# invesalius/invesalius3

Measured on AMD Instinct MI355X. Metric: Mvoxel/s segmentation + Mtriangles/s marching-cubes, 512^3 int16, 1/2/4/8 GPU, higher is better.
Workload: dtype i16; 1 GPU; configs[1]: 512x512x512 int16 per GPU, threshold(226..3071) + 26-neighbour region-grow + marching-cubes(mask@127); global_voxels=134217728, parallelism=z-slab x1, collectives=none, overlap=none

## Files before the change

include/ivx.h:

```cpp
#ifndef IVX_H
#define IVX_H
#include <stddef.h>
#include <stdint.h>

#ifdef __cplusplus
extern "C" {
#endif

#define IVX_OK 0
#define IVX_EINVAL (-1)
#define IVX_ERANGE (-2)
#define IVX_ENOMEM (-3)
#define IVX_EDOM (-4)
#define IVX_EHIP (-5)
#define IVX_ESTALE (-6)
#define IVX_EINTERNAL (-7)

#define IVX_U8 0
#define IVX_I16 1
#define IVX_F64 2
#define IVX_U16 3
#define IVX_F32 4
#define IVX_I32 5
#define IVX_I64 6
// ... 25 lines not shown
int ivx_stream_destroy(void *stream);
int ivx_stream_synchronize(void *stream);
int ivx_event_create(void **event);
int ivx_event_create_sync(void **event);
int ivx_event_destroy(void *event);
int ivx_event_record(void *event, void *stream);
int ivx_stream_wait_event(void *stream, void *event);
int ivx_event_elapsed_ms(void *start, void *stop, float *ms);
int ivx_release_workspace(void);

int ivx_host_register(const void *base, size_t nbytes, uint64_t *handle);
int ivx_host_touch(uint64_t handle);
int ivx_host_touch_range(uint64_t handle, size_t offset, size_t nbytes);
int ivx_host_release(uint64_t handle);
int ivx_host_stats(uint64_t handle, uint64_t out[8]);
int ivx_host_count(uint64_t *count);
int ivx_host_set_check(int on);
int ivx_transfer_stats(uint64_t out[4]);
int ivx_upload_strided(void *dst, const void *src, const int64_t shape[3], const int64_t strides[3], size_t itemsize);
int ivx_download_strided(void *dst, const int64_t shape[3], const int64_t strides[3], const void *src, size_t itemsize);

int ivx_dev_threshold_i16(const int16_t *img, int64_t dz, int64_t dy, int64_t dx, int lo, int hi,
                          int preserve, const uint8_t *skip_flags, uint8_t *mask, void *stream);
int ivx_dev_threshold_i16_bits(const int16_t *img, int64_t dz, int64_t dy, int64_t dx, int lo, int hi, uint8_t *mask,
                               uint64_t *bits, void *stream);
#define IVX_RANGES_BUILD 0
#define IVX_RANGES_USE 1
int ivx_image_ranges_bytes(int64_t dz, int64_t dy, int64_t dx, size_t *nbytes);
int ivx_dev_image_ranges_i16(const int16_t *img, int64_t dz, int64_t dy, int64_t dx, uint32_t *ranges, void *stream);
int ivx_dev_threshold_i16_bits_ranges(const int16_t *img, int64_t dz, int64_t dy, int64_t dx, int lo, int hi,
                                      uint8_t *mask, uint64_t *bits, uint32_t *ranges, int mode, void *stream);
int ivx_dev_threshold_i16_plane(const int16_t *img, int64_t dz, int64_t dy, int64_t dx, int lo, int hi, uint64_t *bits,
                                void *stream);
int ivx_dev_threshold_i16_plane_ranges(const int16_t *img, int64_t dz, int64_t dy, int64_t dx, int lo, int hi, uint64_t *bits,
                                       uint32_t *ranges, int mode, void *stream);
int ivx_threshold_all_slices(const int16_t *img, const int64_t shape[3], const int64_t img_strides[3],
                             int lo, int hi, int preserve, int honour_flags, uint8_t *mask,
                             const int64_t mask_strides[3]);

int ivx_dev_mip_reduce(int dtype, const void *vol, int64_t dz, int64_t dy, int64_t dx, int axis, int op,
                       void *out, void *stream);
int ivx_mip_reduce(int dtype, const void *vol, const int64_t shape[3], const int64_t strides[3], int axis,
                   int op, void *out, const int64_t out_strides[2]);
int ivx_dev_replicate_i16(const int16_t *src, int64_t h, int64_t w, int factor, int16_t *dst, void *stream);

int ivx_dev_minmax_f32(int dtype, const void *vol, int64_t n, float *minmax2, void *stream);
int ivx_dev_mida(int dtype, const void *vol, int64_t dz, int64_t dy, int64_t dx, int axis, float wl, float ww,
                 const float *minmax2 , int out_dtype, void *out,
                 int *status , void *stream);
int ivx_dev_lmip(int dtype, const void *vol, int64_t dz, int64_t dy, int64_t dx, int axis, double tmin,
                 double tmax, void *out, void *stream);
int ivx_dev_rays_z_slab(int kind, int dtype, const void *vol, int64_t dz, int64_t dy, int64_t dx, double p0, double p1,
                        const float *minmax2, const double *state_in, double *state_out, int out_dtype, void *out,
                        int *status, void *stream);
int ivx_powf_variant(void);
int ivx_dev_powf(const float *x, const float *y, float *out, int64_t n, int variant, void *stream);
int ivx_dev_fcm_bounds(const int32_t *d, const uint32_t *other, float n, float *lo, float *hi, int64_t count, void *stream);
int ivx_dev_fcm_volume(int dtype, const void *vol, int64_t dz, int64_t dy, int64_t dx, float n, int axis,
                       void *tmp , int *status, void *stream);
int ivx_dev_fcm_maxip(int dtype, const void *vol, int64_t dz, int64_t dy, int64_t dx, float n, int axis, void *out,
                      int *status, void *stream);
int ivx_mida(int dtype, const void *img, const int64_t shape[3], const int64_t strides[3], int axis,
             double wl, double ww, int out_dtype, void *out, const int64_t out_strides[2]);
int ivx_lmip(int dtype, const void *img, const int64_t shape[3], const int64_t strides[3], int axis,
             double tmin, double tmax, void *out, const int64_t out_strides[2]);
int ivx_fast_countour_mip(int dtype, const void *img, const int64_t shape[3], const int64_t strides[3],
                          float n, int axis, double wl, double ww, int tmip, void *out,
                          const int64_t out_strides[2]);

typedef struct ivx_mc_params {
    int32_t dtype;
    int32_t pad_xy;
    int32_t pad_bottom;
    int32_t pad_top;
    int32_t vtk_pz;
    int32_t niso;
    int64_t nz, ny, nx;
    int64_t roi_start;
    double pad_value;
    double spacing[3];
    double iso[2];
} ivx_mc_params;
int ivx_dev_mc_scratch_bytes(const ivx_mc_params *p, size_t *nbytes);
int ivx_mc_split_word_ids(const ivx_mc_params *p, const uint32_t *wid, size_t n, uint32_t *k, uint32_t *j, uint32_t *w);
int ivx_dev_mc_count(const ivx_mc_params *p, const void *a, void *scratch, int64_t *ntris, void *stream);
int ivx_dev_mc_count_async(const ivx_mc_params *p, const void *a, void *scratch, void *stream);
int ivx_dev_mc_count_bits_async(const ivx_mc_params *p, const uint64_t *inside_bits, void *scratch, void *stream);
int ivx_dev_mc_total(const ivx_mc_params *p, void *scratch, int64_t *ntris, void *stream);
int ivx_dev_mc_total_early(const ivx_mc_params *p, void *scratch, int64_t *ntris, void *stream);
int ivx_dev_mc_count_bits(const ivx_mc_params *p, const uint64_t *inside_bits, void *scratch, int64_t *ntris,
                          void *stream);
int ivx_dev_mc_emit(const ivx_mc_params *p, const void *a, const void *scratch, float *tris, int64_t max_tris,
                    void *stream);
int ivx_dev_mc_emit_levels(const ivx_mc_params *p, const void *scratch, const uint64_t *sel_bits, double v_out, double v_in,
                           double v_sel, float *tris, int64_t max_tris, void *stream);
int ivx_dev_mc_list(const ivx_mc_params *p, const void *scratch, int64_t max_tris, void *stream);
int ivx_marching_cubes_begin(const ivx_mc_params *p, const void *a, const int64_t strides[3], int64_t *ntris);
int ivx_marching_cubes_fetch(float *tris, int64_t ntris);
int ivx_marching_cubes(const ivx_mc_params *p, const void *a, const int64_t strides[3], float *tris,
                       int64_t max_tris, int64_t *ntris);

int ivx_dev_mc_stitch_sig_bytes(const ivx_mc_params *p, size_t *nbytes);
int ivx_dev_mc_stitch_top_sig(const ivx_mc_params *p, const void *scratch, void *sig, void *stream);
int ivx_dev_mc_stitch_match(const ivx_mc_params *p, const void *scratch, const void *nbr_sig, int64_t nverts, uint32_t *vd,
                            void *stream);
int ivx_dev_mc_stitch_apply(const ivx_mc_params *p, const void *scratch, const void *nbr_sig, const uint32_t *vd_all, int rank,
                            const float *verts, int64_t nverts, int32_t *faces, int64_t ntris, float *verts_out, void *stream);
int ivx_dev_mc_indexed_count(const ivx_mc_params *p, const void *a, const void *scratch, int64_t *nverts, void *stream);
int ivx_dev_mc_indexed_emit(const ivx_mc_params *p, const void *a, const void *scratch, float *verts, int64_t max_verts,
                            int32_t *faces, int64_t max_tris, void *stream);
int ivx_dev_mc_indexed_count_levels(const ivx_mc_params *p, const void *scratch, int64_t *nverts, void *stream);
int ivx_dev_mc_indexed_emit_levels(const ivx_mc_params *p, const void *scratch, const uint64_t *sel_bits, double v_out,
                                   double v_in, double v_sel, float *verts, int64_t max_verts, int32_t *faces,
                                   int64_t max_tris, void *stream);
int ivx_marching_cubes_indexed(const ivx_mc_params *p, const void *a, const int64_t strides[3], float *verts,
                               int64_t max_verts, int32_t *faces, int64_t max_tris, int64_t *nverts, int64_t *ntris);

int ivx_dev_mesh_keep_largest(const float *verts, int64_t nverts, const int32_t *faces, int64_t ntris, float *out_verts,
                              int64_t max_verts, int32_t *out_faces, int64_t max_tris, int64_t *out_nverts,
                              int64_t *out_ntris, int64_t *nregions, void *stream);
int ivx_dev_mesh_mass_properties(const float *verts, const int32_t *faces, int64_t ntris, double *out8, void *stream);
int ivx_mesh_keep_largest(const float *verts, int64_t nverts, const int32_t *faces, int64_t ntris, float *out_verts,
                          int32_t *out_faces, int64_t *out_nverts, int64_t *out_ntris, int64_t *nregions);
int ivx_mesh_mass_properties(const float *verts, int64_t nverts, const int32_t *faces, int64_t ntris, double *out8);
int ivx_mesh_fill_holes(const float *verts, int64_t nverts, const int32_t *faces, int64_t ntris, double hole_size,
                        float *new_verts, int32_t *new_faces, int64_t *n_new_verts, int64_t *n_new_tris);
int ivx_mesh_point_normals(const float *verts, int64_t nverts, const int32_t *faces, int64_t ntris, double cos_feature_angle,
                           int splitting, int auto_orient, float *out_verts, int32_t *out_faces, float *point_normals,
                           float *cell_normals , int64_t *out_nverts);
typedef struct ivx_mesh_view {
    double eye[3], right[3], up[3], fwd[3];
    double znear, zfar;
    double tan_half, aspect;
    int32_t width, height;
} ivx_mesh_view;
#define IVX_RASTER_CLEAR 1
#define IVX_RASTER_SMALL 2
#define IVX_RASTER_BIG 4
#define IVX_RASTER_ALL 7
#define IVX_RASTER_SMALL_BOX 64
int ivx_dev_mesh_bounds(const float *verts, int64_t nverts, float *bounds6, void *stream);
int ivx_dev_mesh_depth_raster(const float *verts, int64_t nverts, const int32_t *faces, int64_t ntris,
                              const ivx_mesh_view *view , int stages, float *depth, void *stream);
int ivx_dev_mesh_visible_points(const float *verts, int64_t nverts, const int32_t *faces, int64_t ntris,
                                const ivx_mesh_view *views , int nviews, uint8_t *flags, void *stream);
int ivx_dev_mesh_select_points(const float *verts, int64_t nverts, const int32_t *faces, int64_t ntris, const uint8_t *flags,
                               int invert, float *out_verts, int64_t max_verts, int32_t *out_faces, int64_t max_tris,
                               int64_t *out_nverts, int64_t *out_ntris, void *stream);
int ivx_mesh_bounds(const float *verts, int64_t nverts, float *bounds6);
int ivx_mesh_depth_raster(const float *verts, int64_t nverts, const int32_t *faces, int64_t ntris, const ivx_mesh_view *view,
                          float *depth);
int ivx_mesh_visible_points(const float *verts, int64_t nverts, const int32_t *faces, int64_t ntris,
                            const ivx_mesh_view *views, int nviews, uint8_t *flags);
int ivx_mesh_select_points(const float *verts, int64_t nverts, const int32_t *faces, int64_t ntris, const uint8_t *flags,
                           int invert, float *out_verts, int32_t *out_faces, int64_t *out_nverts, int64_t *out_ntris);
int ivx_mesh_remove_nonvisible(const float *verts, int64_t nverts, const int32_t *faces, int64_t ntris,
                               const ivx_mesh_view *views, int nviews, int remove_visible, float *out_verts,
                               int32_t *out_faces, int64_t *out_nverts, int64_t *out_ntris);

typedef struct ivx_surface_camera {
    double focal[3], right[3], up[3], dir[3];
    double parallel_scale;
    int32_t width, height;
} ivx_surface_camera;
typedef struct ivx_surface_layer {
    const float *verts;
// ... 121 lines not shown
int ivx_dev_mask_snapshot_restore(uint8_t *dst, int64_t n, const void *header, const void *pool, int64_t literal_blocks,
                                  int64_t plane_bytes, uint8_t *plane_flags, void *stream);
int ivx_mask_snapshot(const uint8_t *matrix, size_t nbytes, void **header, void **pool, int64_t *literal_blocks);
int ivx_mask_snapshot_restore(uint8_t *matrix, size_t nbytes, const void *header, const void *pool, int64_t literal_blocks,
                              size_t plane_bytes, int64_t *planes_written);

int ivx_dev_mask_boolean(int op, const uint8_t *m1, const uint8_t *m2, uint8_t *out, int64_t n, void *stream);
int ivx_dev_masked_density_i16(const int16_t *img, const uint8_t *mask, int64_t n, void *acc5, void *stream);
int ivx_mask_boolean(int op, const uint8_t *m1, const int64_t st1[3], const uint8_t *m2, const int64_t st2[3], uint8_t *out,
                     const int64_t sto[3], const int64_t shape[3]);
int ivx_masked_density_i16(const int16_t *img, const int64_t img_strides[3], const uint8_t *mask,
                           const int64_t mask_strides[3], const int64_t shape[3], double *out5);

int ivx_dev_convolve_non_zero(const double *volume, int64_t sz, int64_t sy, int64_t sx, const double *kernel, int64_t skz,
                              int64_t sky, int64_t skx, int cval, double *out, void *stream);
int ivx_mask_area_scratch_bytes(int64_t sz, int64_t sy, int64_t sx, size_t *nbytes);
int ivx_dev_mask_area_u8(const uint8_t *mask, int64_t sz, int64_t sy, int64_t sx, const double *kernel27_dev,
                         double *scratch, double *area_dev, void *stream);
int ivx_convolve_non_zero(const double *volume, const int64_t shape[3], const int64_t vol_strides[3], const double *kernel,
                          const int64_t kshape[3], int cval, double *out);
int ivx_mask_area(const uint8_t *mask, const int64_t shape[3], const int64_t mask_strides[3], const double spacing_xyz[3],
                  double *area);

typedef struct ivx_flood_plan {
    int64_t dz, dy, dx;
    int64_t wx;
    uint32_t strct_bits;
} ivx_flood_plan;
int ivx_flood_bits_bytes(const ivx_flood_plan *p, size_t *nbytes);
int ivx_flood_scratch_bytes(const ivx_flood_plan *p, size_t *nbytes);
int ivx_flood_strct_bits(const uint8_t *strct, const int64_t sshape[3], uint32_t *bits);
int ivx_dev_flood_clear(const ivx_flood_plan *p, uint64_t *reached, void *scratch, void *stream);
int ivx_dev_flood_candidates(const ivx_flood_plan *p, int dtype, const void *data, double t0, double t1,
                             const uint8_t *barrier, int barrier_mode, double fill, uint64_t *cand, void *stream);
int ivx_dev_flood_candidates_ranges(const ivx_flood_plan *p, const int16_t *data, double t0, double t1,
                                    const uint8_t *barrier, int barrier_mode, double fill, const uint32_t *ranges,
                                    uint64_t *cand, void *stream);
int ivx_dev_flood_seed(const ivx_flood_plan *p, int dtype, const void *data, double t0, double t1,
                       const int64_t *seeds_xyz, int64_t nseeds, uint64_t *cand, uint64_t *reached,
                       void *scratch, void *stream);
int ivx_dev_flood_run(const ivx_flood_plan *p, const uint64_t *cand, uint64_t *reached, void *scratch,
                      int *rounds, void *stream);
int ivx_dev_flood_grow(const ivx_flood_plan *p, int dtype, const void *data, double t0, double t1,
                       const int64_t *seeds_xyz, int64_t nseeds, uint64_t *cand, uint64_t *reached, void *scratch,
                       int *rounds, void *stream);
int ivx_dev_flood_visits(const ivx_flood_plan *p, const void *scratch, uint32_t out[2], void *stream);
int ivx_flood_describe(const ivx_flood_plan *p, int64_t nseeds, int32_t out[8]);
int ivx_dev_flood_arm_gate(const void *scratch, uint32_t *word, uint32_t value, uint32_t below_tiles);
int ivx_dev_flood_disarm_gate(const void *scratch);
int ivx_dev_gate_wait(const uint32_t *word, uint32_t value, uint32_t timeout_us, void *stream);
int ivx_dev_gate_open(uint32_t *word, uint32_t value, void *stream);
int ivx_dev_flood_mark_slab(const ivx_flood_plan *p, void *scratch, int64_t z0, int64_t z1, void *stream);
int ivx_dev_bits_combine(uint64_t *dst, const uint64_t *src, int64_t nwords, int op, void *stream);
int ivx_dev_flood_or_plane(const ivx_flood_plan *p, const uint64_t *cand, uint64_t *reached, int64_t z,
                           const uint64_t *plane, void *scratch, int *changed, void *stream);
int ivx_dev_flood_or_planes(const ivx_flood_plan *p, const uint64_t *cand, uint64_t *reached, int64_t z_a,
                            const uint64_t *plane_a, int64_t z_b, const uint64_t *plane_b, void *scratch, int *changed,
                            void *stream);
int ivx_dev_flood_or_planes_dev(const ivx_flood_plan *p, const uint64_t *cand, uint64_t *reached, int64_t z_a,
                                const uint64_t *plane_a, int64_t z_b, const uint64_t *plane_b, void *scratch,
                                uint32_t *changed_dev, void *stream);
int ivx_dev_flood_or_planes_acc(const ivx_flood_plan *p, const uint64_t *cand, uint64_t *reached, int64_t z_a,
                                const uint64_t *plane_a, int64_t z_b, const uint64_t *plane_b, void *scratch,
                                uint32_t *changed_dev, void *stream);
int ivx_dev_flood_apply(const ivx_flood_plan *p, const uint64_t *reached, int dtype, void *target,
                        double fill, void *stream);
int ivx_dev_flood_apply_levels(const ivx_flood_plan *p, const uint64_t *reached, const uint64_t *inside_bits, uint8_t *mask,
                               int v_in, int v_sel, void *stream);
int ivx_dev_mask_from_planes(const ivx_flood_plan *p, const uint64_t *inside_bits, const uint64_t *reached, uint8_t *mask,
                             int v_in, int v_sel, void *stream);
enum { IVX_FLOOD_WRITE_NONE = 0, IVX_FLOOD_WRITE_MASK_FROM_PLANES = 1, IVX_FLOOD_WRITE_APPLY_LEVELS = 2, IVX_FLOOD_WRITE_APPLY_U8 = 3 };
typedef struct ivx_flood_write {
    int32_t kind, v_in, v_sel, reserved;
    const uint64_t *inside_bits;
    uint8_t *mask;
} ivx_flood_write;
int ivx_dev_flood_grow_select(const ivx_flood_plan *p, int dtype, const void *data, double t0, double t1,
                              const int64_t *seeds_xyz, int64_t nseeds, uint64_t *cand, uint64_t *reached, void *scratch,
                              int *rounds, const ivx_flood_write *write, int look_ahead, void *stream);
int ivx_dev_flood_grow_select_count(const ivx_flood_plan *p, int dtype, const void *data, double t0, double t1,
                                    const int64_t *seeds_xyz, int64_t nseeds, uint64_t *cand, uint64_t *reached, void *scratch,
                                    int *rounds, const ivx_flood_write *write, int look_ahead, const ivx_mc_params *mc,
                                    void *mc_scratch, int *counted, void *stream);
int ivx_flood_look_ahead(int64_t n_list, int32_t *look_ahead);
int ivx_dev_flood_apply2(const ivx_flood_plan *p, const uint64_t *reached, uint8_t *out, int fill, uint8_t *mask,
                         int select, void *stream);
int ivx_dev_flood_count(const ivx_flood_plan *p, const uint64_t *reached, int64_t *count, void *stream);
int ivx_flood_edges_bytes(const ivx_flood_plan *p, size_t *nbytes);
int ivx_dev_flood_edges_auto(const ivx_flood_plan *p, const int16_t *data, const uint8_t *out, float pfrac, int fill,
                             uint64_t *edges, void *stream);
int ivx_dev_flood_seed_forced(const ivx_flood_plan *p, const int64_t *seeds_xyz, int64_t nseeds, uint64_t *cand,
                              uint64_t *reached, void *scratch, void *stream);
int ivx_dev_flood_run_edges(const ivx_flood_plan *p, const uint64_t *edges, uint64_t *reached, void *scratch, int *rounds,
                            void *stream);
int ivx_floodfill(int dtype, const void *data, const int64_t shape[3], const int64_t strides[3], int64_t x, int64_t y,
                  int64_t z, double v, int fill, uint8_t *out, const int64_t out_strides[3]);
int ivx_floodfill_auto_threshold(const int16_t *data, const int64_t shape[3], const int64_t strides[3],
                                 const int64_t *seeds_xyz, int64_t nseeds, float pfrac, int fill, uint8_t *out,
                                 const int64_t out_strides[3]);
int ivx_dev_jump_flooding(float *dist, int32_t *owners, const int64_t shape[3], const int32_t *sites_host, int64_t nsites,
                          int normalize, void *stream);
int ivx_jump_flooding(float *dist, const int64_t dist_strides[3], int32_t *owners, const int64_t owner_strides[3],
                      const int64_t shape[3], const int32_t *sites, int64_t nsites, int normalize);
int ivx_floodfill_threshold(int dtype, const void *data, const int64_t shape[3], const int64_t strides[3],
                            const int64_t *seeds_xyz, int64_t nseeds, double t0, double t1, int fill,
                            const uint8_t *strct, const int64_t sshape[3], uint8_t *out,
                            const int64_t out_strides[3]);
int ivx_floodfill_threshold_inplace(int dtype, void *data, const int64_t shape[3], const int64_t strides[3],
                                    const int64_t *seeds_xyz, int64_t nseeds, double t0, double t1,
                                    double fill, const uint8_t *strct, const int64_t sshape[3]);

int ivx_dev_fill_holes(uint8_t *mask, const uint32_t *labels, int64_t n, uint32_t nlabels, uint32_t max_size,
                       uint32_t *sizes , int *status2 ,
                       void *stream);
int ivx_fill_holes_automatically(uint8_t *mask, const int64_t shape[3], const int64_t mask_strides[3],
                                 const uint32_t *labels, const int64_t label_strides[3], uint32_t nlabels,
                                 uint32_t max_size, int *modified);
int ivx_dev_fill_holes_auto(uint8_t *mask, int64_t dz, int64_t dy, int64_t dx, const uint8_t *strct, const int64_t sshape[3],
                            uint32_t max_size, int *modified, void *stream);
int ivx_fill_holes_auto(uint8_t *mask, const int64_t shape[3], const int64_t mask_strides[3], const uint8_t *strct,
                        const int64_t sshape[3], uint32_t max_size, int *modified);

int ivx_dev_lut_u16(const int16_t *img, int64_t n, double window, double level, int top255, uint16_t *out,
                    void *stream);
int ivx_dev_lut_i16(const int16_t *img, int64_t n, double window, double level, int top255, int16_t *out,
                    void *stream);
int ivx_dev_shift_min_u16(const int16_t *img, int64_t n, int imin, uint16_t *out, void *stream);
int ivx_dev_morph_gradient_u16(const uint16_t *in, int64_t dz, int64_t dy, int64_t dx, const int size[3],
                               uint16_t *out, void *stream);
int ivx_dev_watershed_merge(uint8_t *mask, const uint8_t *tmp, int64_t n, int overwrite, void *stream);
int ivx_watershed_prepare(const int16_t *img, const int64_t shape[3], const int64_t strides[3], int use_ww_wl,
                          double window, double level, const int gradient_size[3] , uint16_t *out);
int ivx_watershed_merge(uint8_t *mask, const int64_t shape[3], const int64_t mask_strides[3], const uint8_t *tmp,
                        const int64_t tmp_strides[3], int overwrite);

int ivx_dev_sk_cost_levels(const uint16_t *image, int mdtype, const void *markers, int64_t dz, int64_t dy, int64_t dx,
                           const uint8_t strct[27], uint16_t *C, int max_levels, double stop_frac, int *levels_done,
                           int64_t *reached, int64_t *rounds, void *stream);
int ivx_dev_ws_cost_levels(const uint16_t *cost_image, int mdtype, const void *markers, int64_t dz, int64_t dy, int64_t dx,
                           uint16_t *C, int max_levels, double stop_frac, int *levels_done, int64_t *reached,
                           int64_t *rounds, void *stream);
int ivx_dev_watershed_ift(const uint16_t *cost, int mdtype, const void *markers, int64_t dz, int64_t dy, int64_t dx,
                          const uint8_t strct[27], void *out_labels ,
                          uint8_t *out_u8 , uint16_t *cost_out , int64_t stats[16],
                          void *stream);
int ivx_watershed_ift(int idtype , const void *input, const int64_t shape[3], int mdtype,
                      const void *markers, const uint8_t strct[27], void *output, uint16_t *cost_out, int64_t stats[16]);

int ivx_dev_watershed_sk(const uint16_t *image, int mdtype, const void *markers, int64_t dz, int64_t dy, int64_t dx,
                         const uint8_t strct[27], void *out_labels ,
                         int32_t *out_i32 , uint8_t *out_u8 ,
                         uint16_t *cost_out , int64_t stats[16], void *stream);
int ivx_watershed_sk(int idtype , const void *input, const int64_t shape[3], int mdtype,
                     const void *markers, const uint8_t strct[27], int32_t *output, uint16_t *cost_out, int64_t stats[16]);

int ivx_do_watershed(const int16_t *img, const int64_t shape[3], const int64_t strides[3], int mdtype, const void *markers,
                     const uint8_t strct[27], int algorithm, const int gradient_size[3] ,
                     int use_ww_wl, double window, double level, uint8_t *out_u8, int64_t stats[16]);
int ivx_do_watershed_into(const int16_t *img, const int64_t shape[3], const int64_t strides[3], int mk_src_dtype, const void *markers,
                          const int64_t mk_strides[3], int mdtype, const uint8_t strct[27], int algorithm,
                          const int gradient_size[3] , int use_ww_wl, double window, double level,
                          uint8_t *out_u8, const int64_t out_strides[3], int64_t stats[16]);

int ivx_dev_masked_stats_i16(const int16_t *img, const uint8_t *sel, int64_t n, int64_t out3[3], void *stream);
int ivx_dev_or_equal_u8(uint8_t *dst, const uint8_t *src, int64_t n, int value, void *stream);
int ivx_dev_flood_apply_where(uint8_t *dst, const uint8_t *src, int64_t n, int value, int fill, void *stream);
// ... 209 lines not shown
```

invesalius3_amd/_lib.py:

```python
from __future__ import annotations

import ctypes
import os

import numpy as np

_HERE = os.path.dirname(os.path.abspath(__file__))
LIB_PATH = os.environ.get("IVX_LIB_PATH") or os.path.join(_HERE, "libivx.so")

IVX_OK, IVX_EINVAL, IVX_ERANGE, IVX_ENOMEM, IVX_EDOM, IVX_EHIP, IVX_ESTALE = 0, -1, -2, -3, -4, -5, -6
IVX_EINTERNAL = -7
U8, I16, F64, U16, F32, I32, I64, I8 = 0, 1, 2, 3, 4, 5, 6, 7
DT = {np.dtype(np.uint8): U8, np.dtype(np.int16): I16, np.dtype(np.float64): F64, np.dtype(np.uint16): U16, np.dtype(np.float32): F32, np.dtype(np.int32): I32,
      np.dtype(np.int64): I64}
MIP_MAX, MIP_MIN, MIP_MEAN, MIP_SUM = 0, 1, 2, 3

c_i64 = ctypes.c_int64
c_vp = ctypes.c_void_p


class McParams(ctypes.Structure):
    _fields_ = [
        ("dtype", ctypes.c_int32), ("pad_xy", ctypes.c_int32), ("pad_bottom", ctypes.c_int32),
        ("pad_top", ctypes.c_int32), ("vtk_pz", ctypes.c_int32), ("niso", ctypes.c_int32),
        ("nz", c_i64), ("ny", c_i64), ("nx", c_i64), ("roi_start", c_i64),
        ("pad_value", ctypes.c_double), ("spacing", ctypes.c_double * 3), ("iso", ctypes.c_double * 2),
    ]


class FloodPlan(ctypes.Structure):
    _fields_ = [("dz", c_i64), ("dy", c_i64), ("dx", c_i64), ("wx", c_i64), ("strct_bits", ctypes.c_uint32)]


FLOOD_WRITE_NONE, FLOOD_WRITE_MASK_FROM_PLANES, FLOOD_WRITE_APPLY_LEVELS, FLOOD_WRITE_APPLY_U8 = 0, 1, 2, 3


class FloodWrite(ctypes.Structure):
    _fields_ = [("kind", ctypes.c_int32), ("v_in", ctypes.c_int32), ("v_sel", ctypes.c_int32), ("reserved", ctypes.c_int32),
                ("inside_bits", c_vp), ("mask", c_vp)]


class VolrenParams(ctypes.Structure):
    _fields_ = [
        ("width", ctypes.c_int32), ("height", ctypes.c_int32), ("mip", ctypes.c_int32), ("shade", ctypes.c_int32),
        ("skip", ctypes.c_int32), ("n_table", ctypes.c_int32), ("out_u8", ctypes.c_int32), ("clip", ctypes.c_int32),
        ("origin", ctypes.c_double * 3), ("du", ctypes.c_double * 3), ("dv", ctypes.c_double * 3),
        ("dir", ctypes.c_double * 3), ("spacing", ctypes.c_double * 3), ("dt", ctypes.c_double),
        ("ambient", ctypes.c_double), ("diffuse", ctypes.c_double), ("specular", ctypes.c_double),
        ("specular_power", ctypes.c_double), ("background", ctypes.c_double * 3), ("clip_normal", ctypes.c_double * 3),
        ("clip_origin", ctypes.c_double * 3),
    ]


ROI_ELLIPSE, ROI_POLYGON, ROI_MAX_POINTS, ROI_RECORD_BYTES = 0, 1, 2048, 40
WELD_COUNT_WORDS, WELD_VERTS, WELD_KEPT, WELD_DROPPED, WELD_OVERRUN, WELD_NONFINITE, WELD_MAX_PROBE, WELD_LOG2_SLOTS, WELD_HIST = 32, 0, 1, 2, 3, 4, 5, 6, 8
WELD_MAX_CORNERS = 2 ** 31 - 1


class Roi(ctypes.Structure):
    _fields_ = [
        ("image", c_vp), ("row_stride", c_i64), ("elem_stride", c_i64), ("h", c_i64), ("w", c_i64),
        ("kind", ctypes.c_int32), ("n_points", ctypes.c_int32), ("first_point", c_i64),
        ("sx", ctypes.c_double), ("sy", ctypes.c_double), ("cx", ctypes.c_double), ("cy", ctypes.c_double),
        ("a2", ctypes.c_double), ("b2", ctypes.c_double),
        ("x0", c_i64), ("y0", c_i64), ("x1", c_i64), ("y1", c_i64), ("first_block", c_i64), ("n_blocks", c_i64),
    ]


class StaleError(RuntimeError):
    """IVX_ESTALE: a registered host array (resident.bind) was written without a touch; raised only with the stale check on."""


def _declare(lib):
    u64, sz, u64p = ctypes.c_uint64, ctypes.c_size_t, ctypes.POINTER(ctypes.c_uint64)
    i64p = ctypes.POINTER(c_i64)
    for name, args in (("ivx_host_register", [c_vp, sz, u64p]), ("ivx_host_touch", [u64]), ("ivx_host_touch_range", [u64, sz, sz]),
                       ("ivx_host_release", [u64]), ("ivx_host_stats", [u64, u64p]), ("ivx_host_count", [u64p]),
                       ("ivx_host_set_check", [ctypes.c_int]), ("ivx_transfer_stats", [u64p]),
                       ("ivx_upload_strided", [c_vp, c_vp, i64p, i64p, sz]), ("ivx_download_strided", [c_vp, i64p, i64p, c_vp, sz]),
                       ("ivx_image_ranges_bytes", [c_i64, c_i64, c_i64, ctypes.POINTER(sz)]),
                       ("ivx_dev_image_ranges_i16", [c_vp, c_i64, c_i64, c_i64, c_vp, c_vp]),
                       ("ivx_dev_threshold_i16_bits_ranges", [c_vp, c_i64, c_i64, c_i64, ctypes.c_int, ctypes.c_int, c_vp, c_vp, c_vp,
                                                              ctypes.c_int, c_vp]),
                       ("ivx_dev_threshold_i16_plane", [c_vp, c_i64, c_i64, c_i64, ctypes.c_int, ctypes.c_int, c_vp, c_vp]),
                       ("ivx_dev_threshold_i16_plane_ranges", [c_vp, c_i64, c_i64, c_i64, ctypes.c_int, ctypes.c_int, c_vp, c_vp,
                                                               ctypes.c_int, c_vp]),
                       ("ivx_dev_mask_from_planes", [ctypes.POINTER(FloodPlan), c_vp, c_vp, c_vp, ctypes.c_int, ctypes.c_int, c_vp]),
                       ("ivx_dev_flood_candidates_ranges", [ctypes.POINTER(FloodPlan), c_vp, ctypes.c_double, ctypes.c_double, c_vp,
                                                            ctypes.c_int, ctypes.c_double, c_vp, c_vp, c_vp]),
                       ("ivx_dev_flood_grow_select", [ctypes.POINTER(FloodPlan), ctypes.c_int, c_vp, ctypes.c_double, ctypes.c_double,
                                                      c_vp, c_i64, c_vp, c_vp, c_vp, ctypes.POINTER(ctypes.c_int),
                                                      ctypes.POINTER(FloodWrite), ctypes.c_int, c_vp]),
                       ("ivx_dev_flood_grow_select_count", [ctypes.POINTER(FloodPlan), ctypes.c_int, c_vp, ctypes.c_double, ctypes.c_double,
                                                            c_vp, c_i64, c_vp, c_vp, c_vp, ctypes.POINTER(ctypes.c_int),
                                                            ctypes.POINTER(FloodWrite), ctypes.c_int, ctypes.POINTER(McParams), c_vp,
                                                            ctypes.POINTER(ctypes.c_int), c_vp]),
                       ("ivx_flood_look_ahead", [c_i64, ctypes.POINTER(ctypes.c_int32)]),
                       ("ivx_dev_image_flip", [c_vp, c_i64, c_i64, c_i64, sz, ctypes.c_int, c_vp]),
                       ("ivx_image_flip", [c_vp, i64p, i64p, sz, ctypes.c_int]),
                       ("ivx_dev_image_swap_axes", [c_vp, c_i64, c_i64, c_i64, sz, ctypes.c_int, ctypes.c_int, c_vp, c_vp]),
                       ("ivx_image_swap_axes", [c_vp, i64p, i64p, sz, ctypes.c_int, ctypes.c_int, c_vp, i64p]),
                       ("ivx_image_tilt_scratch_bytes", [c_i64, c_i64, c_i64, ctypes.POINTER(sz)]),
                       ("ivx_dev_image_fix_gantry_tilt", [c_vp, c_i64, c_i64, c_i64, c_vp, c_vp, sz, c_vp, c_vp]),
                       ("ivx_image_fix_gantry_tilt", [c_vp, i64p, i64p, c_vp, c_vp]),
                       ("ivx_host_zero", [c_vp, sz]), ("ivx_host_register_zero", [c_vp, sz, u64p]),
                       ("ivx_slice_show_tables_bytes", [ctypes.c_int, ctypes.POINTER(sz)]),
                       ("ivx_dev_slice_show", [c_vp, c_i64, c_i64] * 3 + [c_i64, c_i64, c_vp, c_vp, c_vp, c_vp]),
                       ("ivx_slice_show", [c_vp, c_i64, c_i64] * 3 + [c_i64, c_i64, c_vp, c_vp, c_vp]),
                       ("ivx_mask_snapshot_header_bytes", [c_i64, ctypes.POINTER(sz)]),
                       ("ivx_dev_mask_snapshot_scan", [c_vp, c_i64, c_vp, i64p, c_vp]),
                       ("ivx_dev_mask_snapshot_pack", [c_vp, c_i64, c_vp, c_vp, c_i64, c_vp]),
                       ("ivx_dev_mask_snapshot_restore", [c_vp, c_i64, c_vp, c_vp, c_i64, c_i64, c_vp, c_vp]),
                       ("ivx_mask_snapshot", [c_vp, sz, ctypes.POINTER(c_vp), ctypes.POINTER(c_vp), i64p]),
                       ("ivx_mask_snapshot_restore", [c_vp, sz, c_vp, c_vp, c_i64, sz, i64p]),
                       ("ivx_dev_surface_raster", [c_vp, c_i64, c_vp, c_i64, c_vp, ctypes.c_int, c_vp, c_vp]),
                       ("ivx_dev_surface_resolve", [c_vp, ctypes.c_int, c_vp, ctypes.c_int, c_vp, ctypes.c_int, c_vp, c_vp, c_vp, c_vp]),
                       ("ivx_surface_render", [c_vp, ctypes.c_int, c_vp, ctypes.c_int, c_vp, ctypes.c_int, c_vp, c_vp, c_vp]),
                       ("ivx_dev_roi_density", [c_vp, c_i64, c_vp, c_vp, c_i64, c_vp, c_vp]),
                       ("ivx_roi_density", [c_vp, c_i64, c_vp, c_i64, c_vp]),
                       ("ivx_dev_m3e_filter", [c_i64, c_i64, c_vp, c_vp, c_i64, ctypes.c_int, c_vp, c_vp]),
                       ("ivx_dev_m3e_cut", [c_vp, i64p, i64p, c_vp, ctypes.c_double, c_vp, c_i64, c_i64, c_vp, c_vp, ctypes.c_int, c_vp, c_vp]),
                       ("ivx_dev_m3e_brush_stroke", [c_vp, c_vp, i64p, i64p, c_vp, c_vp, c_vp, c_i64, ctypes.c_double, ctypes.c_int, c_vp,
                                                     c_vp]),
                       ("ivx_dev_m3e_equal", [c_vp, c_vp, c_i64, ctypes.POINTER(ctypes.c_int), c_vp]),
                       ("ivx_dev_m3e_apply", [c_vp, c_vp, i64p, i64p, c_vp, c_vp]),
                       ("ivx_m3e_filter", [c_i64, c_i64, c_vp, c_vp, c_i64, ctypes.c_int, c_vp]),
                       ("ivx_m3e_cut", [c_vp, i64p, i64p, c_vp, ctypes.c_double, c_vp, c_i64, c_i64, c_vp, c_vp, c_i64, c_vp, c_vp,
                                        ctypes.c_int, i64p]),
                       ("ivx_m3e_brush_stroke", [c_vp, c_vp, i64p, i64p, c_vp, c_vp, c_i64, ctypes.c_double, ctypes.c_int, i64p]),
                       ("ivx_m3e_apply", [c_vp, c_vp, i64p, i64p, i64p]), ("ivx_m3e_flag_planes", [c_vp, i64p, i64p]),
                       ("ivx_mesh_weld_slots", [c_i64, u64p]), ("ivx_mesh_weld_bytes", [c_i64, ctypes.POINTER(sz)]),
                       ("ivx_dev_mesh_weld", [c_vp, c_i64, c_vp, c_vp, c_vp, c_vp, c_vp]),
                       ("ivx_dev_stl_unpack", [c_vp, c_i64, c_vp, c_vp, c_vp]),
                       ("ivx_dev_mesh_transform_points", [c_vp, c_i64, c_vp, c_vp, c_vp]),
                       ("ivx_mesh_weld", [c_vp, c_i64, c_vp, c_vp, c_vp]), ("ivx_mesh_stl_weld", [c_vp, sz, c_vp, c_vp, c_vp]),
                       ("ivx_mesh_transform_points", [c_vp, c_i64, c_vp, c_vp])):
        fn = getattr(lib, name)
        fn.argtypes, fn.restype = args, ctypes.c_int


_lib = None


def lib() -> ctypes.CDLL:
    global _lib
    if _lib is None:
        if not os.path.exists(LIB_PATH):
            raise ImportError(
                "libivx.so not found at %s: build it with `python -m invesalius3_amd.build` "
                "(there is no CPU fallback in this package)" % LIB_PATH)
        _lib = ctypes.CDLL(LIB_PATH)
        _lib.ivx_last_error.restype = ctypes.c_char_p
        _declare(_lib)
    return _lib


def last_error() -> str:
    return (lib().ivx_last_error() or b"").decode("utf-8", "replace")


def check(rc: int, what: str = "ivx") -> int:
    if rc >= 0:
        return rc
    msg = "%s: %s" % (what, last_error())
    if rc == IVX_EINVAL:
        raise TypeError(msg)
    if rc == IVX_ERANGE:
        raise IndexError(msg)
    if rc == IVX_ENOMEM:
        raise MemoryError(msg)
    if rc == IVX_EDOM:
        raise ValueError(msg)
    if rc == IVX_ESTALE:
        raise StaleError(msg)
    raise RuntimeError(msg)


def i64(seq):
    return (c_i64 * len(seq))(*[int(v) for v in seq])


def ptr(a: np.ndarray):
    return ctypes.c_void_p(a.ctypes.data)


def dtype_code(a: np.ndarray, allowed=(U8, I16, F64, U16)) -> int:
    code = DT.get(a.dtype)
    if code is None or code not in allowed:
        raise TypeError("unsupported array dtype %s" % a.dtype)
    return code


class _Pinned:

    def __init__(self, nbytes: int):
        self.ptr = ctypes.c_void_p()
        check(lib().ivx_host_alloc(ctypes.byref(self.ptr), ctypes.c_size_t(int(nbytes))), "ivx_host_alloc")

    def __del__(self):
        try:
            if self.ptr and self.ptr.value:
                lib().ivx_host_free(self.ptr)
        except Exception:
            pass


def pinned_empty(shape, dtype) -> np.ndarray:
    dt = np.dtype(dtype)
    n = int(np.prod(shape)) * dt.itemsize
    own = _Pinned(max(n, 16))
    buf = (ctypes.c_uint8 * max(n, 16)).from_address(own.ptr.value)
    buf._ivx_owner = own
    return np.frombuffer(buf, dtype=dt, count=int(np.prod(shape))).reshape(shape)


def device_count() -> int:
    n = ctypes.c_int(0)
    lib().ivx_device_count(ctypes.byref(n))
    return n.value


def require_device():
    if device_count() < 1:
        raise RuntimeError("invesalius3_amd: no HIP device visible and there is no CPU fallback")


def device_name() -> str:
    buf = ctypes.create_string_buffer(256)
    check(lib().ivx_device_name(buf, ctypes.c_size_t(256)))
    return buf.value.decode()


def set_device(i: int):
    check(lib().ivx_set_device(int(i)))


def synchronize():
    check(lib().ivx_device_synchronize())


def flood_visits(plan: FloodPlan, scratch, stream=None):
    out = (ctypes.c_uint32 * 2)()
    check(lib().ivx_dev_flood_visits(ctypes.byref(plan), scratch, out, stream), "flood_visits")
    return int(out[0]), int(out[1])
```

invesalius3_amd/csrc/ivx_internal.h:

```cpp
#pragma once
#include <hip/hip_runtime.h>
#include <stdint.h>
#include <stdio.h>
#include <string.h>

#include "../../include/ivx.h"

namespace ivx {

void set_error(const char *fmt, ...);

#define IVX_HIP(expr)                                                                      \
    do {                                                                                   \
        hipError_t e__ = (expr);                                                           \
        if (e__ != hipSuccess) {                                                           \
            ivx::set_error("%s:%d %s -> %s", __FILE__, __LINE__, #expr, hipGetErrorString(e__)); \
            return e__ == hipErrorOutOfMemory ? IVX_ENOMEM : IVX_EHIP;                     \
        }                                                                                  \
    } while (0)

bool trace_enabled();
#define IVX_LAUNCH_CHECK()                                                                 \
    do {                                                                                   \
        IVX_HIP(hipGetLastError());                                                        \
        if (ivx::trace_enabled()) {                                                        \
            fprintf(stderr, "ivx trace: launched %s:%d ...", __FILE__, __LINE__);          \
            fflush(stderr);                                                                \
            IVX_HIP(hipDeviceSynchronize());                                               \
            fprintf(stderr, " ok\n");                                                      \
        }                                                                                  \
    } while (0)

#define IVX_REQUIRE(cond, code, ...)                                                       \
    do {                                                                                   \
        if (!(cond)) {                                                                     \
            ivx::set_error(__VA_ARGS__);                                                   \
            return (code);                                                                 \
        }                                                                                  \
    } while (0)

static inline hipStream_t S(void *s) { return (hipStream_t)s; }
static inline int64_t cdiv(int64_t a, int64_t b) { return (a + b - 1) / b; }
static inline size_t dtype_size(int dt) {
    switch (dt) {
    case IVX_U8: return 1;
    case IVX_I16: return 2;
    case IVX_U16: return 2;
    case IVX_F64: return 8;
    default: return 0;
    }
}

enum { WS_IN = 0, WS_OUT, WS_AUX0, WS_AUX1, WS_AUX2, WS_AUX3, WS_SMALL, WS_CCL0, WS_CCL1, WS_MCLIST, WS_MCV, WS_MCST, WS_MESH, WS_MESH2, WS_HOLES, WS_LUT, WS_WSIFT, WS_WSSK, WS_WSA, WS_WSLINK, WS_COUNT };
int ws_get(int slot, size_t nbytes, void **dptr);
int ws_get_s(int slot, hipStream_t stream, size_t nbytes, void **dptr);
uint64_t host_epoch();
int ws_release_s(int slot, hipStream_t stream, size_t keep_below);
struct HostCallGuard {
    HostCallGuard();
    ~HostCallGuard();
};
int hs_get(int slot, size_t nbytes, void **hptr);

int copy_h2d(void *dst_dev, const void *src, size_t n);
int copy_d2h(void *dst, const void *src_dev, size_t n);

int upload_strided(void *dst_dev, const void *src, const int64_t shape[3], const int64_t strides[3], size_t isz,
                   int hslot);
int download_strided(void *dst, const int64_t shape[3], const int64_t strides[3], const void *src_dev, size_t isz,
                     int hslot);
int download_strided2(void *dst, const int64_t shape[2], const int64_t strides[2], const void *src_dev, size_t isz,
                      int hslot);
int mirror_host_view(const void *view, const int64_t shape[3], const int64_t strides[3], size_t isz, void *d_scratch, int hslot);

struct MirrorHold;
int mirror_acquire(const void *p, size_t n, bool reads, MirrorHold **hold, void **mirror);
int mirror_fetch(MirrorHold *hold, void *host, const void *mirror, size_t n);
void mirror_release(MirrorHold *hold, size_t written);

void ccl_forget_stream(void *stream);
void ccl_invalidate(const void *scratch);
int ccl_small_components(const ivx_flood_plan *p, const uint64_t *cand, uint64_t *out, uint32_t max_size, int *any_small,
                         const void *scratch_key, hipStream_t st);
bool ccl_supported(uint32_t strct_bits);
int ccl_run(const ivx_flood_plan *p, const uint64_t *cand, uint64_t *reached, const void *scratch_key, hipStream_t st);
enum FloodMode {
    FLOOD_SYMMETRIC,
    FLOOD_DIRECTED,
    FLOOD_LINEAR,
};
int flood_run(const ivx_flood_plan *p, const uint64_t *planes, FloodMode mode, uint64_t *reached, void *scratch, int *rounds,
              void *stream);

struct ApplyWhen;
bool mc_ride_ok(const ivx_mc_params *p, const void *scratch, int64_t dz, int64_t dy, int64_t dx);
void mc_ride_begin(void *scratch, const uint64_t *inside_bits);
int mc_ride_launch(const ivx_mc_params *p, void *scratch, const uint64_t *reached, const uint64_t *inside, int64_t nchunks, uint8_t *mask,
                   int v_in, int v_sel, bool all, const ApplyWhen &when, hipStream_t st);
int mc_ride_scan(const ivx_mc_params *p, void *scratch, hipStream_t st);

int mailbox_publish(const void *dsrc, int ndwords, hipStream_t st, uint32_t *seq_out);
int mailbox_wait(uint32_t seq, hipStream_t st, uint32_t *out, int ndwords);
int mailbox_reserve(uint32_t **slot_out, uint32_t *seq_out);
int mailbox_wait_reserved(uint32_t seq, hipStream_t st, uint32_t *out, int ndwords, int *got);
int vote_publish(int32_t *votes, hipStream_t st, uint32_t *seq_out);
int progress_line(hipStream_t stream, volatile unsigned long long **line, uint32_t *tag);
void progress_forget_stream(void *stream);

}
```

invesalius3_amd/csrc/k_flood.hip:

```cpp
#include <math.h>
#include <map>
#include <mutex>
#include <stdlib.h>

#include "flood_tiles.h"
#include "levels_write.h"
#include "words_from_records.h"

using ivx::ApplyWhen;

namespace {

constexpr int NT = TY * TZ;
constexpr int HY = TY + 2, HZ = TZ + 2;
constexpr int BATCH = 8;
constexpr int SUB = 1;
constexpr unsigned int CLOSED = 0x40u;

template <typename T> __device__ __forceinline__ double as_double(T v) { return (double)v; }

template <typename T, int BAR>
__global__ __launch_bounds__(256) void k_flood_candidates16(const short8_t *__restrict__ data,
                                                            const uint4 *__restrict__ bar, int64_t nchunks, double t0,
                                                            double t1, double fill, uint16_t *__restrict__ cand) {
    const int64_t stride = (int64_t)gridDim.x * blockDim.x;
    const int lo = (int)ceil(t0 < -70000.0 ? -70000.0 : t0), hi = (int)floor(t1 > 70000.0 ? 70000.0 : t1);
    const unsigned fb = (unsigned)(uint8_t)fill;
    for (int64_t c = (int64_t)blockIdx.x * blockDim.x + threadIdx.x; c < nchunks; c += stride) {
        const short8_t a = __builtin_nontemporal_load(&data[2 * c]);
        const short8_t b = __builtin_nontemporal_load(&data[2 * c + 1]);
        uint4 q = make_uint4(0, 0, 0, 0);
        if (BAR == 1) q = bar[c];
        const unsigned bw[4] = {q.x, q.y, q.z, q.w};
        unsigned m = 0;
#pragma unroll
        for (int e = 0; e < 16; e++) {
            const int v = (int)(T)(e < 8 ? a[e & 7] : b[e & 7]);
            bool ok = v >= lo && v <= hi;
            if (BAR == 1) ok = ok && ((bw[e >> 2] >> (8 * (e & 3))) & 0xffu) != fb;
            if (BAR == 2) ok = ok && (double)v != fill;
            m |= ok ? (1u << e) : 0u;
        }
        cand[c] = (uint16_t)m;
    }
}

__global__ __launch_bounds__(256) void k_flood_candidates_words(const short8_t *__restrict__ data, const unsigned *__restrict__ ranges,
                                                                int64_t nwords, double t0, double t1,
                                                                unsigned long long *__restrict__ cand) {
    const int lo = (int)ceil(t0 < -70000.0 ? -70000.0 : t0), hi = (int)floor(t1 > 70000.0 ? 70000.0 : t1);
    words_from_records(data, ranges, nwords, lo, hi, cand);
}

__global__ __launch_bounds__(256) void k_flood_candidates16_ranges(const short8_t *__restrict__ data,
                                                                   const uint4 *__restrict__ bar,
                                                                   const unsigned *__restrict__ ranges, int64_t nchunks,
                                                                   double t0, double t1, double fill,
                                                                   uint16_t *__restrict__ cand) {
    const int64_t stride = (int64_t)gridDim.x * blockDim.x;
    const int lo = (int)ceil(t0 < -70000.0 ? -70000.0 : t0), hi = (int)floor(t1 > 70000.0 ? 70000.0 : t1);
    const unsigned fb = (unsigned)(uint8_t)fill;
    int64_t c = (int64_t)blockIdx.x * blockDim.x + threadIdx.x;
    if (c >= nchunks) return;
    unsigned rec = ranges[c >> 2];
    for (;;) {
        const int64_t cn = c + stride;
        unsigned rec_next = 0;
        if (cn < nchunks) rec_next = ranges[cn >> 2];
        const int mn = (int)(short)(rec & 0xffffu), mx = (int)(short)(rec >> 16);
        unsigned m = 0;
        if (!(mx < lo || mn > hi)) {
            const bool inside = mn >= lo && mx <= hi;
            if (inside) {
                m = 0xffffu;
            } else {
                const short8_t a = __builtin_nontemporal_load(&data[2 * c]);
                const short8_t b = __builtin_nontemporal_load(&data[2 * c + 1]);
#pragma unroll
                for (int e = 0; e < 16; e++) {
                    const int v = (int)(e < 8 ? a[e & 7] : b[e & 7]);
                    m |= (v >= lo && v <= hi) ? (1u << e) : 0u;
                }
            }
            if (m) {
                const uint4 q = bar[c];
                const unsigned bw[4] = {q.x, q.y, q.z, q.w};
#pragma unroll
                for (int e = 0; e < 16; e++)
                    if (((bw[e >> 2] >> (8 * (e & 3))) & 0xffu) == fb) m &= ~(1u << e);
            }
        }
        cand[c] = (uint16_t)m;
        if (cn >= nchunks) break;
        c = cn;
        rec = rec_next;
    }
}

template <typename T, int BAR>
__global__ __launch_bounds__(256) void k_flood_candidates(const T *__restrict__ data, const uint8_t *__restrict__ bar,
                                                          Tiles t, double t0, double t1, double fill,
                                                          uint8_t *__restrict__ cand) {
    const int64_t bpr = t.wx * 8;
    const int64_t total = t.dz * t.dy * bpr;
    const int64_t stride = (int64_t)gridDim.x * blockDim.x;
    const bool vec = (sizeof(T) == 2) && (t.dx % 8 == 0) && (((uintptr_t)data & 15) == 0) &&
                     (BAR != 1 || ((uintptr_t)bar & 7) == 0);
    for (int64_t i = (int64_t)blockIdx.x * blockDim.x + threadIdx.x; i < total; i += stride) {
        const int64_t row = i / bpr, q = i - row * bpr;
        const int64_t x0 = q * 8;
        unsigned m = 0;
        if (x0 < t.dx) {
            const int64_t base = row * t.dx + x0;
            if (vec) {
                const short8_t v = *reinterpret_cast<const short8_t *>(data + base);
                unsigned long long b8 = 0;
                if (BAR == 1) b8 = *reinterpret_cast<const unsigned long long *>(bar + base);
#pragma unroll
                for (int e = 0; e < 8; e++) {
                    const double d = (double)(T)v[e];
                    bool ok = d >= t0 && d <= t1;
                    if (BAR == 1) ok = ok && (((b8 >> (8 * e)) & 0xff) != (unsigned long long)(uint8_t)fill);
                    if (BAR == 2) ok = ok && d != fill;
                    m |= ok ? (1u << e) : 0u;
                }
            } else {
#pragma unroll
                for (int e = 0; e < 8; e++) {
                    if (x0 + e < t.dx) {
                        const double d = as_double(data[base + e]);
                        bool ok = d >= t0 && d <= t1;
                        if (BAR == 1) ok = ok && bar[base + e] != (uint8_t)fill;
                        if (BAR == 2) ok = ok && d != fill;
                        m |= ok ? (1u << e) : 0u;
                    }
                }
            }
        }
        cand[i] = (uint8_t)m;
    }
}

template <typename T>
__global__ void k_flood_seed(const T *__restrict__ data, Tiles t, double t0, double t1, const int64_t *__restrict__ seeds,
                             int64_t nseeds, unsigned long long *__restrict__ cand,
                             unsigned long long *__restrict__ reached, uint8_t *__restrict__ dirty) {
    const int64_t n = (int64_t)blockIdx.x * blockDim.x + threadIdx.x;
    if (n >= nseeds) return;
    const int64_t x = seeds[3 * n], y = seeds[3 * n + 1], z = seeds[3 * n + 2];
    const double v = as_double(data[(z * t.dy + y) * t.dx + x]);
    if (!(v >= t0 && v <= t1)) return;
    const int64_t w = (z * t.dy + y) * t.wx + (x >> 6);
    const unsigned long long bit = 1ull << (x & 63);
    atomicOr(&cand[w], bit);
    atomicOr(&reached[w], bit);
    mark_tile_nbhd(t, dirty, z / TZ, y / TY, x >> 6);
}

struct SeedPack {
    int64_t xyz[16][3];
    int n;
};
template <typename T>
__global__ void k_flood_seed_args(const T *__restrict__ data, Tiles t, double t0, double t1, SeedPack sp,
                                  unsigned long long *__restrict__ cand, unsigned long long *__restrict__ reached,
                                  uint8_t *__restrict__ dirty) {
    const int n = threadIdx.x;
    if (n >= sp.n) return;
    const int64_t x = sp.xyz[n][0], y = sp.xyz[n][1], z = sp.xyz[n][2];
    const double v = as_double(data[(z * t.dy + y) * t.dx + x]);
    if (!(v >= t0 && v <= t1)) return;
    const int64_t w = (z * t.dy + y) * t.wx + (x >> 6);
    const unsigned long long bit = 1ull << (x & 63);
    atomicOr(&cand[w], bit);
    atomicOr(&reached[w], bit);
    mark_tile_nbhd(t, dirty, z / TZ, y / TY, x >> 6);
}

__device__ __forceinline__ unsigned long long fill_up(unsigned long long seed, unsigned long long m) {
    return (((m + seed) ^ m) & m) | seed;
}
__device__ __forceinline__ unsigned long long fill_runs(unsigned long long seed, unsigned long long m) {
    unsigned long long f = fill_up(seed, m);
    return __brevll(fill_up(__brevll(f), __brevll(m)));
}

__device__ __forceinline__ void lds_barrier() {
    __builtin_amdgcn_s_waitcnt(0xC07F);
    __builtin_amdgcn_s_barrier();
}
struct TileOpen {
    unsigned long long sO[HZ * HY];
};
struct TileLds {
    unsigned long long sN[HZ * HY];
    unsigned long long sD[HZ * HY];
    unsigned char sCL[HZ * HY], sCR[HZ * HY];
    unsigned int dirs;
    unsigned int open;
    unsigned int vote[2];
};
__device__ __forceinline__ void post_dirs(TileLds &L, unsigned dirs) {
#pragma unroll
    for (int o = 32; o > 0; o >>= 1) dirs |= __shfl_xor(dirs, o, 64);
    if ((threadIdx.x & 63) == 0 && dirs) atomicOr(&L.dirs, dirs);
}

template <int CONN>
__device__ __forceinline__ void tile_update(const Tiles &t, const unsigned long long *__restrict__ cand,
                                            unsigned long long *reached, int64_t tile, TileLds &L, TileOpen &O) {
    const int64_t txi = tile % t.wx, r1 = tile / t.wx;
    const int64_t tyi = r1 % t.nty, tzi = r1 / t.nty;
    const int64_t z0 = tzi * TZ, y0 = tyi * TY;
    unsigned long long w3[2][3] = {{0ull, 0ull, 0ull}, {0ull, 0ull, 0ull}};
    unsigned long long hc[2] = {0ull, 0ull};
    unsigned int hx[2] = {0u, 0u};
#pragma unroll
    for (int pass = 0; pass < 2; pass++) {
        const int idx = threadIdx.x + pass * NT;
        if (idx < HZ * HY) {
            const int yy = idx % HY, zz = idx / HY;
            const int64_t z = z0 + zz - 1, y = y0 + yy - 1;
            if (z >= 0 && z < t.dz && y >= 0 && y < t.dy) {
                unsigned long long *row = reached + (z * t.dy + y) * t.wx;
#pragma unroll
                for (int xx = 0; xx < 3; xx++) {
                    const int64_t w = txi + xx - 1;
                    if (w >= 0 && w < t.wx) w3[pass][xx] = row[w];
                }
                if (zz == 0 || zz == HZ - 1 || yy == 0 || yy == HY - 1) hc[pass] = cand[(z * t.dy + y) * t.wx + txi];
                hx[pass] = 1u;
            }
        }
    }
#pragma unroll
    for (int pass = 0; pass < 2; pass++) {
        const int idx = threadIdx.x + pass * NT;
        if (idx < HZ * HY) {
            const unsigned long long cl = w3[pass][0] >> 63, cr = w3[pass][2] & 1ull, n = w3[pass][1];
            L.sN[idx] = n;
            L.sD[idx] = n | (n << 1) | (n >> 1) | cl | (cr << 63);
            const unsigned int ul = hx[pass] & ~(unsigned int)cl, ur = hx[pass] & ~(unsigned int)cr;
            L.sCL[idx] = (unsigned char)(cl | (ul << 1) | (ur << 2));
            L.sCR[idx] = (unsigned char)cr;
            O.sO[idx] = hc[pass] & ~n;
        }
    }
    const int ty = threadIdx.x & (TY - 1), tz = threadIdx.x >> TY_LOG;
    const int64_t z = z0 + tz, y = y0 + ty;
    const bool inside = z < t.dz && y < t.dy;
    const unsigned long long c = inside ? cand[(z * t.dy + y) * t.wx + txi] : 0ull;
    if (threadIdx.x == 0) L.vote[0] = 0u;
    __syncthreads();
    const int me = (tz + 1) * HY + (ty + 1);
    const unsigned long long r_in = L.sN[me];
    const unsigned long long mycl = L.sCL[me] & 1u, mycr = L.sCR[me];
    unsigned long long r = r_in;
    const uint32_t st = t.strct;
    const bool xrun = (st >> 12 & 1) && (st >> 14 & 1);
    bool exhausted = true;
    for (int it = 0; it < t.itcap; it++) {
      bool changed = false;
#pragma unroll
      for (int sub = 0; sub < SUB; sub++) {
        unsigned long long nb = 0;
        if (CONN != 0) {
            unsigned long long v[9];
#pragma unroll
// ... 255 lines not shown
        if (zlo) dirs |= 1u << 4;
        if (zhi) dirs |= 1u << 22;
        if (ylo) {
            if (y0 > 0) dirs |= 1u << 10;
            else if (me_w - t.wx >= 0 && lin_enlist(t, me_w - t.wx, tile, dirty_next, list_next, n_next)) dirs |= 1u << 13;
        }
        if (yhi) {
            if (y0 + TY < t.dy) dirs |= 1u << 16;
            else if (me_w + t.wx < nwords && lin_enlist(t, me_w + t.wx, tile, dirty_next, list_next, n_next)) dirs |= 1u << 13;
        }
        if (xlo) {
            if (txi > 0) dirs |= 1u << 12;
            else if (me_w > 0 && lin_enlist(t, me_w - 1, tile, dirty_next, list_next, n_next)) dirs |= 1u << 13;
        }
        if (xhi) {
            if (txi + 1 < t.wx) dirs |= 1u << 14;
            else if (me_w + 1 < nwords && lin_enlist(t, me_w + 1, tile, dirty_next, list_next, n_next)) dirs |= 1u << 13;
        }
        if (exhausted) dirs |= 1u << 13;
    }
    post_dirs(L, dirs);
    if (threadIdx.x == 0) L.open = 1u;
}

__global__ void k_flood_build_list(Tiles t, const uint8_t *__restrict__ dirty, unsigned int *__restrict__ list,
                                   unsigned int *__restrict__ count) {
    const int64_t i = (int64_t)blockIdx.x * blockDim.x + threadIdx.x;
    if (i < t.ntiles && (dirty[i] & 1u)) list[atomicAdd(count, 1u)] = (unsigned int)i;
}

constexpr int STATS_AT = 36, HIST_AT = 64, HIST = 64, CNT_CLEARED = HIST_AT + HIST;
static_assert(CNT_CLEARED == FLOOD_CNT_DWORDS, "the counter block of flood_tiles.h");
__device__ __forceinline__ void count_visits(unsigned int *cnt, unsigned int round, unsigned int n) {
    if (!n) return;
    if (round <= (unsigned int)HIST) cnt[HIST_AT + round - 1u] = n;
    else cnt[STATS_AT] += n;
}
template <int MODE>
__global__ __launch_bounds__(NT, 6) void k_flood_round_list(Tiles t, const unsigned long long *__restrict__ cand,
                                                             unsigned long long *reached, const unsigned int *__restrict__ list_cur,
                                                             const unsigned int *__restrict__ n_cur, uint8_t *dirty_cur,
                                                             uint8_t *dirty_next, unsigned int *list_next,
                                                             unsigned int *n_next, unsigned int *n_clear,
                                                             unsigned int *cnt_all, unsigned long long *line,
                                                             unsigned int tag_round, unsigned int *gate,
                                                             unsigned int gate_val, unsigned int gate_below) {
    __shared__ TileLds L;
    const unsigned int n = *n_cur;
    if (blockIdx.x == 0 && threadIdx.x == 0) {
        if (gate && n < gate_below) __hip_atomic_store(gate, gate_val, __ATOMIC_RELAXED, __HIP_MEMORY_SCOPE_AGENT);
        *n_clear = 0u;
        count_visits(cnt_all, tag_round & 0xffffffu, n);
        const unsigned long long hi = (unsigned long long)tag_round << 32;
        __hip_atomic_store(&line[0], hi | n, __ATOMIC_RELAXED, __HIP_MEMORY_SCOPE_SYSTEM);
        if (n) __hip_atomic_store(&line[1], hi, __ATOMIC_RELAXED, __HIP_MEMORY_SCOPE_SYSTEM);
    }
    for (unsigned int li = blockIdx.x; li < n; li += gridDim.x) {
        const int64_t tile = list_cur[li];
        if (threadIdx.x == 0) {
            dirty_cur[tile] = 0;
            L.dirs = 0;
            L.open = 0;
        }
        __syncthreads();
        if constexpr (MODE == 2) tile_update_lin(t, cand, reached, tile, L, dirty_next, list_next, n_next);
        else if constexpr (MODE == 1) tile_update_dir(t, cand, reached, tile, L);
        else {
            __shared__ TileOpen O;
            tile_update_conn(t, cand, reached, tile, L, O);
        }
        lds_barrier();
        publish_tile(t, tile, L, dirty_cur, dirty_next, list_next, n_next);
        __syncthreads();
    }
}

__global__ void k_flood_mark(Tiles t, int64_t tz0, int64_t tz1, uint8_t *dirty) {
    const int64_t per = t.nty * t.wx;
    const int64_t n = (tz1 - tz0) * per;
    const int64_t i = (int64_t)blockIdx.x * blockDim.x + threadIdx.x;
    if (i < n) dirty[tz0 * per + i] = 1;
}

constexpr int CT = 1024, CRP = 8, CROWS_MAX = 7680;
constexpr unsigned int ENLISTED = 0x80u;

struct Blocks {
    int q;
    int bxs;
};
__device__ __forceinline__ unsigned long long block_mask(const Blocks &b, unsigned long long qbits) {
    const unsigned long long one = b.bxs == 64 ? ~0ull : ((1ull << b.bxs) - 1ull);
    unsigned long long m = 0;
    for (int q = 0; q < b.q; q++)
        if (qbits >> q & 1ull) m |= one << (b.bxs * q);
    return m;
}
__device__ __forceinline__ unsigned int block_exist(const Tiles &t, const Blocks &b, int64_t txi) {
    unsigned int m = 0;
    for (int q = 0; q < b.q; q++)
        if (txi * 64 + (int64_t)b.bxs * q < t.dx) m |= 1u << q;
    return m;
}

__device__ __forceinline__ double load_as_double(const void *data, int dtype, int64_t i) {
    switch (dtype) {
    case IVX_I16: return (double)((const int16_t *)data)[i];
    case IVX_U8: return (double)((const uint8_t *)data)[i];
    case IVX_U16: return (double)((const uint16_t *)data)[i];
    default: return ((const double *)data)[i];
    }
}

template <bool FRESH>
__global__ __launch_bounds__(256) void k_flood_block_flags(Tiles t, Blocks bk, unsigned long long *cand,
                                                           const unsigned long long *__restrict__ reached,
                                                           uint8_t *dirty, uint8_t *dirty1,
                                                           unsigned long long *__restrict__ rowF,
                                                           unsigned long long *__restrict__ rowW,
                                                           unsigned int *__restrict__ cnt, int ncnt, SeedPack sp, int dtype,
                                                           const void *__restrict__ data, double t0, double t1,
                                                           unsigned int *__restrict__ seed_ok) {
    __shared__ unsigned int s_bad[64], s_has[64];
    const int64_t tyi = blockIdx.x % t.nty, tzi = blockIdx.x / t.nty;
    if (threadIdx.x < 64) {
        s_bad[threadIdx.x] = 0u;
        s_has[threadIdx.x] = 0u;
    }
    if (blockIdx.x == 0 && (int)threadIdx.x < ncnt) cnt[threadIdx.x] = 0u;
    const int wx = (int)t.wx, per_z = TY * wx, nw = TZ * per_z;
    const int64_t tile0 = (int64_t)blockIdx.x * t.wx;
    if (FRESH) {
        if ((int)threadIdx.x < wx) {
            dirty[tile0 + threadIdx.x] = 0;
            dirty1[tile0 + threadIdx.x] = 0;
        }
        if (blockIdx.x == 0) {
            __shared__ unsigned int s_ok;
            if (threadIdx.x == 0) s_ok = 0u;
            __syncthreads();
            if ((int)threadIdx.x < sp.n) {
                const int64_t x = sp.xyz[threadIdx.x][0], y = sp.xyz[threadIdx.x][1], z = sp.xyz[threadIdx.x][2];
                const double v = load_as_double(data, dtype, (z * t.dy + y) * t.dx + x);
                if (v >= t0 && v <= t1) {
                    atomicOr(&cand[(z * t.dy + y) * t.wx + (x >> 6)], 1ull << (x & 63));
                    atomicOr(&s_ok, 1u << threadIdx.x);
                }
            }
            __syncthreads();
            if (threadIdx.x == 0) *seed_ok = s_ok;
        }
    }
    __syncthreads();
    const unsigned long long last = (t.dx & 63) ? (1ull << (t.dx & 63)) - 1ull : ~0ull;
    const unsigned long long one = bk.bxs == 64 ? ~0ull : ((1ull << bk.bxs) - 1ull);
    for (int i0 = threadIdx.x; i0 < nw; i0 += 4 * 256) {
        unsigned long long cv[4], rv[4];
        int64_t wi[4];
        int tx[4];
#pragma unroll
        for (int u = 0; u < 4; u++) {
            const int i = i0 + u * 256;
            const int tz = i / per_z, rem = i - tz * per_z, ty = rem / wx;
            tx[u] = rem - ty * wx;
            const int64_t z = tzi * TZ + tz, y = tyi * TY + ty;
            wi[u] = (i < nw && z < t.dz && y < t.dy) ? (z * t.dy + y) * t.wx + tx[u] : -1;
            cv[u] = wi[u] >= 0 ? cand[wi[u]] : 0ull;
            rv[u] = 0ull;
            if (!FRESH && wi[u] >= 0 && (dirty[tile0 + tx[u]] & 1u)) rv[u] = reached[wi[u]];
        }
#pragma unroll
        for (int u = 0; u < 4; u++) {
            if (wi[u] < 0) continue;
            const unsigned long long miss = ~cv[u] & (tx[u] == wx - 1 ? last : ~0ull);
            for (int q = 0; q < bk.q; q++) {
                if ((miss >> (bk.bxs * q)) & one) s_bad[tx[u] * bk.q + q] = 1u;
                else if (!FRESH && ((rv[u] >> (bk.bxs * q)) & one)) s_has[tx[u] * bk.q + q] = 1u;
            }
        }
    }
    __syncthreads();
    if (threadIdx.x < 64) {
        const int b = threadIdx.x, btx = b / bk.q;
        const bool in = btx < wx && (int64_t)btx * 64 + (int64_t)bk.bxs * (b % bk.q) < t.dx;
        const unsigned long long f = __ballot(in && !s_bad[b]);
        const unsigned long long h = __ballot(in && s_has[b]);
        if (threadIdx.x == 0) {
            rowF[blockIdx.x] = f;
            rowW[blockIdx.x] = FRESH ? 0ull : (f & h);
        }
    }
}

template <int CONN, bool SEEDED>
__global__ __launch_bounds__(CT) void k_flood_coarse(Tiles t, Blocks bk, const unsigned long long *__restrict__ rowF,
                                                     unsigned long long *__restrict__ rowW, SeedPack sp,
                                                     const unsigned int *__restrict__ seed_ok) {
    __shared__ unsigned long long sR[CROWS_MAX];
    __shared__ unsigned int vote[2];
    const int nty = (int)t.nty, ntz = (int)t.ntz, hy = nty + 2;
    const int nrows = nty * ntz, nh = hy * (ntz + 2);
    unsigned long long F[CRP], R[CRP];
    int me[CRP];
#pragma unroll
    for (int k = 0; k < CRP; k++) {
        const int j = threadIdx.x + k * (int)blockDim.x;
        F[k] = j < nrows ? rowF[j] : 0ull;
        R[k] = (j < nrows && !SEEDED) ? rowW[j] : 0ull;
        me[k] = j < nrows ? (j / nty + 1) * hy + (j % nty) + 1 : 0;
    }
    for (int i = threadIdx.x; i < nh; i += blockDim.x) sR[i] = 0ull;
    if (threadIdx.x == 0) vote[0] = 0u;
    __syncthreads();
    if (SEEDED) {
        if ((int)threadIdx.x < sp.n && (*seed_ok >> threadIdx.x & 1u)) {
            const int64_t x = sp.xyz[threadIdx.x][0], y = sp.xyz[threadIdx.x][1], z = sp.xyz[threadIdx.x][2];
            const int j = (int)((z / TZ) * nty + y / TY);
            const unsigned long long bit = 1ull << (x / bk.bxs);
            if (rowF[j] & bit) atomicOr(&sR[(j / nty + 1) * hy + (j % nty) + 1], bit);
        }
        __syncthreads();
#pragma unroll
        for (int k = 0; k < CRP; k++) R[k] = sR[me[k]];
        __syncthreads();
    }
#pragma unroll
    for (int k = 0; k < CRP; k++)
        if (R[k]) {
            R[k] = fill_runs(R[k], F[k]);
            sR[me[k]] = R[k];
        }
    __syncthreads();
    for (int it = 0; it < 65536; it++) {
        bool changed = false;
#pragma unroll
        for (int k = 0; k < CRP; k++) {
            if (!(F[k] & ~R[k])) continue;
            unsigned long long nb = 0;
#pragma unroll
            for (int kk = -1; kk <= 1; kk++)
#pragma unroll
                for (int jj = -1; jj <= 1; jj++) {
                    const int nz = (kk != 0) + (jj != 0);
                    const bool wide = CONN == 26 || (CONN == 18 && nz <= 1) || (CONN == 6 && nz == 0);
                    const bool mid = (CONN == 18 && nz == 2) || (CONN == 6 && nz == 1);
                    if (!wide && !mid) continue;
                    const unsigned long long n = sR[me[k] + kk * hy + jj];
                    nb |= wide ? (n | (n << 1) | (n >> 1)) : n;
                }
            const unsigned long long nr = fill_runs(R[k] | (nb & F[k]), F[k]);
            if (nr != R[k]) {
                R[k] = nr;
                sR[me[k]] = nr;
                changed = true;
            }
        }
        if (__any(changed) && (threadIdx.x & 63) == 0) vote[it & 1] = 1u;
        if (threadIdx.x == 0) vote[(it + 1) & 1] = 0u;
        __syncthreads();
        if (!vote[it & 1]) break;
    }
#pragma unroll
    for (int k = 0; k < CRP; k++) {
        const int j = threadIdx.x + k * (int)blockDim.x;
        if (j < nrows) rowW[j] = R[k];
    }
}

template <bool FRESH>
__global__ __launch_bounds__(256) void k_flood_block_apply(Tiles t, Blocks bk, const unsigned long long *__restrict__ cand,
                                                           unsigned long long *__restrict__ reached,
                                                           const unsigned long long *__restrict__ rowW, uint8_t *dirty,
                                                           unsigned int *__restrict__ list, unsigned int *count, SeedPack sp,
                                                           const unsigned int *__restrict__ seed_ok) {
    __shared__ unsigned int s_chg[64];
    __shared__ unsigned int s_all[64];
// ... 411 lines not shown
    const uint4 z = make_uint4(0u, 0u, 0u, 0u);
    for (int64_t i = (int64_t)blockIdx.x * blockDim.x + threadIdx.x; i < n16 + h16; i += stride) {
        if (i < n16) reached[i] = z;
        else head[i - n16] = z;
    }
}

extern "C" int ivx_dev_flood_clear(const ivx_flood_plan *p, uint64_t *reached, void *scratch, void *stream) {
    Tiles t;
    int rc = make_tiles(p, &t);
    if (rc) return rc;
    const FScratch s = make_fscratch(t);
    const size_t nb = (size_t)(t.dz * t.dy * t.wx) * 8;
    if ((nb | s.off_seeds | (uintptr_t)reached | (uintptr_t)scratch) & 15) {
        IVX_HIP(hipMemsetAsync(reached, 0, nb, ivx::S(stream)));
        IVX_HIP(hipMemsetAsync(scratch, 0, s.off_seeds, ivx::S(stream)));
    } else {
        const int64_t total = (int64_t)((nb + s.off_seeds) / 16);
        const int64_t blocks = ivx::cdiv(total, 256);
        hipLaunchKernelGGL(k_flood_clear, dim3((unsigned)(blocks < 8192 ? blocks : 8192)), dim3(256), 0, ivx::S(stream),
                           (uint4 *)reached, (int64_t)(nb / 16), (uint4 *)scratch, (int64_t)(s.off_seeds / 16));
        IVX_LAUNCH_CHECK();
    }
    ivx::ccl_invalidate(scratch);
    return IVX_OK;
}

struct GateArm {
    unsigned int *word;
    unsigned int value, below;
};
static std::map<const void *, GateArm> g_gates;
static std::mutex g_gates_mu;

__global__ void k_gate_wait(const unsigned int *word, unsigned int value, unsigned long long timeout_ticks) {
    if (threadIdx.x) return;
    const unsigned long long t0 = wall_clock64();
    while (__hip_atomic_load(word, __ATOMIC_RELAXED, __HIP_MEMORY_SCOPE_AGENT) != value) {
        if (wall_clock64() - t0 > timeout_ticks) break;
        __builtin_amdgcn_s_sleep(32);
    }
}
__global__ void k_gate_set(unsigned int *word, unsigned int value) {
    if (threadIdx.x == 0) __hip_atomic_store(word, value, __ATOMIC_RELAXED, __HIP_MEMORY_SCOPE_AGENT);
}

struct Fresh {
    int dtype;
    const void *data;
    double t0, t1;
    SeedPack sp;
};
static bool flood_mode_ccl() {
    static const bool ccl = [] {
        const char *e = getenv("IVX_FLOOD_MODE");
        return e && !strcmp(e, "ccl");
    }();
    return ccl;
}
static bool coarse_ok(const Tiles &t, ivx::FloodMode mode) {
    static const bool coarse_on = [] {
        const char *e = getenv("IVX_FLOOD_COARSE");
        return !(e && e[0] == '0');
    }();
    return coarse_on && mode == ivx::FLOOD_SYMMETRIC && t.conn != 0 && t.wx <= 64 && (t.nty + 2) * (t.ntz + 2) <= CROWS_MAX &&
           t.nty * t.ntz <= (int64_t)CT * CRP;
}
static Blocks coarse_blocks(const Tiles &t) {
    static const int bxs_env = [] {
        const char *e = getenv("IVX_FLOOD_BLOCK");
        return e ? atoi(e) : 0;
    }();
    Blocks bk;
    bk.bxs = 16;
    while (bk.bxs < 64 && ((64 / bk.bxs) * t.wx > 64 || bk.bxs < bxs_env)) bk.bxs *= 2;
    bk.q = 64 / bk.bxs;
    return bk;
}
static int coarse_lanes(const Tiles &t) {
    int ct = 64;
    while (ct < CT && ct < t.nty * t.ntz) ct *= 2;
    return ct;
}
template <bool FRESH>
static int coarse_pass(const Tiles &t, const FScratch &s, char *scr, const uint64_t *cand, uint64_t *reached, const Fresh &f,
                       int ncnt, hipStream_t st) {
    const Blocks bk = coarse_blocks(t);
    uint8_t *dirty0 = (uint8_t *)(scr + s.off_dirty0), *dirty1 = (uint8_t *)(scr + s.off_dirty1);
    unsigned int *cnt = (unsigned int *)(scr + s.off_cnt), *list0 = (unsigned int *)(scr + s.off_list0);
    unsigned long long *rowF = (unsigned long long *)(scr + s.off_full), *rowW = (unsigned long long *)(scr + s.off_whole);
    unsigned int *seed_ok = (unsigned int *)(scr + s.off_status) + 8;
    const unsigned groups = (unsigned)(t.nty * t.ntz);
    const int ct = coarse_lanes(t);
    hipLaunchKernelGGL(k_flood_block_flags<FRESH>, dim3(groups), dim3(256), 0, st, t, bk, (unsigned long long *)cand,
                       (const unsigned long long *)reached, dirty0, dirty1, rowF, rowW, cnt, ncnt, f.sp, f.dtype, f.data, f.t0,
                       f.t1, seed_ok);
    IVX_LAUNCH_CHECK();
    auto coarse = t.conn == 26 ? k_flood_coarse<26, FRESH> : t.conn == 18 ? k_flood_coarse<18, FRESH> : k_flood_coarse<6, FRESH>;
    hipLaunchKernelGGL(coarse, dim3(1), dim3(ct), 0, st, t, bk, (const unsigned long long *)rowF, rowW, f.sp,
                       (const unsigned int *)seed_ok);
    IVX_LAUNCH_CHECK();
    hipLaunchKernelGGL(k_flood_block_apply<FRESH>, dim3(groups), dim3(256), 0, st, t, bk, (const unsigned long long *)cand,
                       (unsigned long long *)reached, (const unsigned long long *)rowW, dirty0, list0, cnt, f.sp,
                       (const unsigned int *)seed_ok);
    IVX_LAUNCH_CHECK();
    return IVX_OK;
}
static unsigned round_grid_cap(const Tiles &t) { return (unsigned)(t.ntiles < 1536 ? t.ntiles : 1536); }
template <typename Done>
static int poll_line(volatile unsigned long long *line, long spins, hipStream_t st, Done done, const char *never,
                     unsigned long long *word) {
    for (long n = 0; n < spins; n++) {
        *word = __atomic_load_n((const unsigned long long *)line, __ATOMIC_ACQUIRE);
        if (done(*word)) return IVX_OK;
#if defined(__x86_64__)
        __builtin_ia32_pause();
#endif
    }
    IVX_HIP(hipStreamSynchronize(st));
    *word = __atomic_load_n((const unsigned long long *)line, __ATOMIC_ACQUIRE);
    IVX_REQUIRE(done(*word), IVX_EHIP, "%s", never);
    return IVX_OK;
}
static int levels_check(const Tiles &t, const uint64_t *reached, const uint64_t *inside_bits, const uint8_t *mask, int v_in, int v_sel,
                        bool all) {
    if (all) {
        IVX_REQUIRE(inside_bits && mask, IVX_EINVAL, "mask_from_planes: null plane or mask");
        IVX_REQUIRE(t.dx % 64 == 0 && ((uintptr_t)mask & 15) == 0 && (((uintptr_t)inside_bits | (uintptr_t)reached) & 7) == 0, IVX_EINVAL,
                    "mask_from_planes: rows of whole 64-voxel words, a 16-byte aligned mask and 8-byte aligned planes only");
        IVX_REQUIRE(v_in >= 0 && v_in <= 255 && v_sel >= 0 && v_sel <= 255, IVX_EINVAL, "mask_from_planes: levels are bytes");
    } else {
        IVX_REQUIRE(reached && inside_bits && mask, IVX_EINVAL, "flood_apply_levels: null plane or mask");
        IVX_REQUIRE(t.dx % 64 == 0 && ((uintptr_t)mask & 15) == 0, IVX_EINVAL,
                    "flood_apply_levels: rows of whole 64-voxel words and a 16-byte aligned mask only");
        IVX_REQUIRE(v_in >= 0 && v_in <= 255 && v_sel >= 0 && v_sel <= 255, IVX_EINVAL, "flood_apply_levels: levels are bytes");
    }
    return IVX_OK;
}
struct McRide {
    const ivx_mc_params *p;
    void *scratch;
};
static int launch_levels(const Tiles &t, const uint64_t *reached, const uint64_t *inside, uint8_t *mask, int v_in, int v_sel, bool all,
                         const ApplyWhen &when, hipStream_t st, const McRide *ride = nullptr) {
    const int64_t nchunks = t.dz * t.dy * t.dx / 16;
    if (!nchunks) return IVX_OK;
    if (ride) return ivx::mc_ride_launch(ride->p, ride->scratch, reached, inside, nchunks, mask, v_in, v_sel, all, when, st);
    const int64_t blocks = ivx::cdiv(nchunks, 1024);
    auto k = all ? k_flood_apply_levels16<true> : k_flood_apply_levels16<false>;
    hipLaunchKernelGGL(k, dim3((unsigned)(blocks < 16384 ? blocks : 16384)), dim3(256), 0, st, (const uint16_t *)reached,
                       (const uint16_t *)inside, nchunks, (uint4 *)mask, (uint8_t)v_in, (uint8_t)v_sel, when);
    IVX_LAUNCH_CHECK();
    return IVX_OK;
}
constexpr unsigned AHEAD_LONG_LIST = 384u;
static int default_look_ahead(unsigned n_list) { return n_list >= AHEAD_LONG_LIST ? 0 : 1; }
struct EarlyWrite {
    const ivx_flood_write *w;
    bool written;
    const McRide *ride = nullptr;
    bool plain = false;
};
constexpr unsigned EARLY_BELOW = 96u;
constexpr int EARLY_TRIES = 2;
static int flood_run_impl(const ivx_flood_plan *p, const uint64_t *cand, ivx::FloodMode mode, uint64_t *reached, void *scratch_,
                          int *rounds, void *stream, const Fresh *fresh = nullptr, int look_ahead = -1, EarlyWrite *early = nullptr) {
    const bool sym = mode == ivx::FLOOD_SYMMETRIC;
    Tiles t;
    int rc = make_tiles(p, &t);
    if (rc) return rc;
    if (rounds) *rounds = 0;
    hipStream_t st = ivx::S(stream);
    GateArm arm = {nullptr, 0u, 0u};
    {
        std::lock_guard<std::mutex> lk(g_gates_mu);
        auto it = g_gates.find(scratch_);
        if (it != g_gates.end()) {
            arm = it->second;
            g_gates.erase(it);
        }
    }
    struct GateGuard {
        GateArm &a;
        hipStream_t st;
        ~GateGuard() {
            if (a.word) hipLaunchKernelGGL(k_gate_set, dim3(1), dim3(64), 0, st, a.word, a.value);
        }
    } gate_guard = {arm, st};
    if (t.ntiles == 0) return IVX_OK;
    const FScratch s = make_fscratch(t);
    char *scr = (char *)scratch_;
    uint8_t *dirty[2] = {(uint8_t *)(scr + s.off_dirty0), (uint8_t *)(scr + s.off_dirty1)};
    unsigned int *cnt = (unsigned int *)(scr + s.off_cnt);
    constexpr int CCL_ESCAPE_ROUNDS = 48;
    if (sym && flood_mode_ccl() && ivx::ccl_supported(p->strct_bits)) {
        if (rounds) *rounds = 1;
        IVX_HIP(hipMemsetAsync(dirty[0], 0, (size_t)t.ntiles, st));
        if (early) early->plain = true;
        return ivx::ccl_run(p, cand, reached, scratch_, st);
    }
    int total_rounds = 0;
    unsigned int *list[2] = {(unsigned int *)(scr + s.off_list0), (unsigned int *)(scr + s.off_list1)};
    constexpr int RING = 2 * BATCH;
    static const int env_ahead = [] {
        const char *e = getenv("IVX_FLOOD_BATCH");
        if (!e || !*e) return -1;
        const int v = atoi(e);
        return v < 0 ? 0 : (v > BATCH ? BATCH : v);
    }();
    const int fixed_ahead = env_ahead >= 0 ? env_ahead : (look_ahead > BATCH ? BATCH : look_ahead);
    int ahead = fixed_ahead >= 0 ? fixed_ahead : 1;
    if (coarse_ok(t, mode)) {
        static const Fresh no_seeds = {0, nullptr, 0.0, 0.0, {{}, 0}};
        rc = fresh ? coarse_pass<true>(t, s, scr, cand, reached, *fresh, CNT_CLEARED, st)
                   : coarse_pass<false>(t, s, scr, cand, reached, no_seeds, CNT_CLEARED, st);
        if (rc) return rc;
    } else {
        IVX_REQUIRE(!fresh, IVX_EINVAL, "flood: the fused start needs the coarse pass");
        IVX_HIP(hipMemsetAsync(cnt, 0, CNT_CLEARED * 4, st));
        hipLaunchKernelGGL(k_flood_build_list, dim3((unsigned)ivx::cdiv(t.ntiles, 256)), dim3(256), 0, st, t, dirty[0], list[0], cnt);
        IVX_LAUNCH_CHECK();
    }
    volatile unsigned long long *line = nullptr;
    uint32_t tag = 0;
    if ((rc = ivx::progress_line(st, &line, &tag))) return rc;
    const unsigned grid_max = round_grid_cap(t);
    unsigned grid = grid_max;
    int64_t queued = 0;
    auto round_kernel = mode == ivx::FLOOD_LINEAR ? k_flood_round_list<2> : mode == ivx::FLOOD_DIRECTED ? k_flood_round_list<1> : k_flood_round_list<0>;
    auto queue_round = [&]() -> int {
        const int r = (int)(queued % RING), cur = (int)(queued & 1);
        const unsigned int tr = (unsigned int)(tag << 24) | (unsigned int)((queued + 1) & 0xffffff);
        hipLaunchKernelGGL(round_kernel, dim3(grid), dim3(NT), 0, st, t, (const unsigned long long *)cand,
                           (unsigned long long *)reached, (const unsigned int *)list[cur], (const unsigned int *)(cnt + r), dirty[cur],
                           dirty[cur ^ 1], list[cur ^ 1], cnt + (r + 1) % RING, cnt + (r + 2) % RING, cnt,
                           (unsigned long long *)line, tr,
                           arm.word, arm.value, arm.below);
        IVX_LAUNCH_CHECK();
        queued++;
        return IVX_OK;
    };
    static const bool trace = getenv("IVX_FLOOD_TRACE") != nullptr;
    static const bool early_on = [] {
        const char *e = getenv("IVX_FLOOD_EARLY");
        return !(e && e[0] == '0');
    }();
    const bool early_all = early && early->w->kind == IVX_FLOOD_WRITE_MASK_FROM_PLANES;
    int early_left = 0;
    if (early_on && early && (early_all || early->w->kind == IVX_FLOOD_WRITE_APPLY_LEVELS) &&
        levels_check(t, reached, early->w->inside_bits, early->w->mask, early->w->v_in, early->w->v_sel, early_all) == IVX_OK)
        early_left = EARLY_TRIES;
    if (early_left) __atomic_store_n((unsigned long long *)line + 2, 0ull, __ATOMIC_RELEASE);
    int64_t early_at = -1;
    unsigned long long early_report = 0;
    bool early_seen = false;
    unsigned int prev_list = 0xffffffffu;
    int64_t seen = 0;
    for (;;) {
        while (queued < seen + 1 + ahead)
            if ((rc = queue_round())) return rc;
        unsigned long long v = 0;
        rc = poll_line(line, 20000000L, st,
                       [&](unsigned long long w) {
                           if (early_at >= 0 && __atomic_load_n((const unsigned long long *)line + 2, __ATOMIC_ACQUIRE) == early_report)
                               return early_seen = true;
                           return (uint32_t)(w >> 56) == tag && (int64_t)((w >> 32) & 0xffffffull) > seen;
                       },
                       "flood: the queued rounds never reported", &v);
        if (rc) return rc;
        if (early_seen) {
            const unsigned long long u = __atomic_load_n((const unsigned long long *)line + 1, __ATOMIC_ACQUIRE);
            total_rounds = (uint32_t)(u >> 56) == tag ? (int)((u >> 32) & 0xffffffull) : 0;
            early->written = true;
            if (trace) fprintf(stderr, "ivx flood: the write behind round %lld went ahead (%d rounds with work)\n", (long long)early_at, total_rounds);
            break;
        }
        seen = (int64_t)((v >> 32) & 0xffffffull);
        const unsigned int n_list = (unsigned int)(v & 0xffffffffull);
        if (trace) fprintf(stderr, "ivx flood: round %lld starts with %u of %lld tiles (%lld queued)\n", (long long)seen, n_list,
                           (long long)t.ntiles, (long long)queued);
        if (n_list < arm.below) arm.word = nullptr;
        grid = n_list >= 384u ? grid_max : (n_list >= 96u ? (grid_max < 512u ? grid_max : 512u) : (grid_max < 128u ? grid_max : 128u));
        if (fixed_ahead < 0) ahead = default_look_ahead(n_list);
        if (n_list == 0) {
            const unsigned long long u = __atomic_load_n((const unsigned long long *)line + 1, __ATOMIC_ACQUIRE);
            total_rounds = (uint32_t)(u >> 56) == tag ? (int)((u >> 32) & 0xffffffull) : 0;
            if (early_at >= 0 && total_rounds <= early_at) early->written = true;
            break;
        }
        if (early_at >= 0 && seen > early_at) early_at = -1;
        if (early_left > 0 && early_at < 0 && n_list < EARLY_BELOW && n_list <= prev_list / 2u) {
            early_at = queued;
            early_left--;
            early_report = ((unsigned long long)tag << 56) | ((unsigned long long)(queued & 0xffffff) << 32) | 1ull;
            if (trace) fprintf(stderr, "ivx flood: write queued behind round %lld\n", (long long)queued);
            rc = launch_levels(t, reached, early->w->inside_bits, early->w->mask, early->w->v_in, early->w->v_sel, early_all,
                               ApplyWhen{cnt + queued % RING, (unsigned long long *)line, early_report}, st, early->ride);
            if (rc) return rc;
        }
        prev_list = n_list;
        total_rounds = (int)seen;
        if (sym && total_rounds >= CCL_ESCAPE_ROUNDS && ivx::ccl_supported(p->strct_bits)) {
            IVX_HIP(hipMemsetAsync(dirty[0], 0, (size_t)t.ntiles, st));
            IVX_HIP(hipMemsetAsync(dirty[1], 0, (size_t)t.ntiles, st));
            if ((rc = ivx::ccl_run(p, cand, reached, scratch_, st))) return rc;
            total_rounds += 1;
            if (early) early->plain = true;
            break;
        }
        IVX_REQUIRE(total_rounds < (1 << 24) - 64, IVX_EHIP, "flood: did not converge");
    }
    if (rounds) *rounds = total_rounds;
    return IVX_OK;
}

constexpr int AHEAD_CHAINED = 3;
int ivx::flood_run(const ivx_flood_plan *p, const uint64_t *planes, ivx::FloodMode mode, uint64_t *reached, void *scratch,
                   int *rounds, void *stream) {
    return flood_run_impl(p, planes, mode, reached, scratch, rounds, stream, nullptr, AHEAD_CHAINED);
}

extern "C" int ivx_dev_flood_run(const ivx_flood_plan *p, const uint64_t *cand, uint64_t *reached, void *scratch_,
                                 int *rounds, void *stream) {
    return flood_run_impl(p, cand, ivx::FLOOD_SYMMETRIC, reached, scratch_, rounds, stream, nullptr, AHEAD_CHAINED);
}
static bool fused_start(const Tiles &t, int64_t nseeds) {
    static const bool fused_on = [] {
        const char *e = getenv("IVX_FLOOD_FUSED");
        return !(e && e[0] == '0');
    }();
    return fused_on && nseeds >= 1 && nseeds <= 16 && t.ntiles > 0 && !flood_mode_ccl() && coarse_ok(t, ivx::FLOOD_SYMMETRIC);
}
static int flood_grow_impl(const ivx_flood_plan *p, int dtype, const void *data, double t0, double t1, const int64_t *seeds_xyz,
                           int64_t nseeds, uint64_t *cand, uint64_t *reached, void *scratch_, int *rounds, void *stream,
                           int look_ahead, EarlyWrite *early = nullptr) {
    Tiles t;
    int rc = make_tiles(p, &t);
    if (rc) return rc;
    IVX_REQUIRE(ivx::dtype_size(dtype), IVX_EINVAL, "flood: unsupported dtype %d", dtype);
    for (int64_t n = 0; n < nseeds; n++) {
        const int64_t x = seeds_xyz[3 * n], y = seeds_xyz[3 * n + 1], z = seeds_xyz[3 * n + 2];
        IVX_REQUIRE(x >= 0 && y >= 0 && z >= 0 && x < t.dx && y < t.dy && z < t.dz, IVX_ERANGE,
                    "flood: seed (%lld,%lld,%lld) outside volume (%lld,%lld,%lld) [x,y,z]", (long long)x, (long long)y,
                    (long long)z, (long long)t.dx, (long long)t.dy, (long long)t.dz);
    }
    if (!fused_start(t, nseeds)) {
        if ((rc = ivx_dev_flood_clear(p, reached, scratch_, stream))) return rc;
        if ((rc = ivx_dev_flood_seed(p, dtype, data, t0, t1, seeds_xyz, nseeds, cand, reached, scratch_, stream))) return rc;
        return flood_run_impl(p, cand, ivx::FLOOD_SYMMETRIC, reached, scratch_, rounds, stream, nullptr, look_ahead, early);
    }
    ivx::ccl_invalidate(scratch_);
    Fresh f;
    f.dtype = dtype;
    f.data = data;
    f.t0 = t0;
    f.t1 = t1;
    f.sp.n = (int)nseeds;
    for (int64_t n = 0; n < nseeds; n++)
        for (int q = 0; q < 3; q++) f.sp.xyz[n][q] = seeds_xyz[3 * n + q];
    return flood_run_impl(p, cand, ivx::FLOOD_SYMMETRIC, reached, scratch_, rounds, stream, &f, look_ahead, early);
}
extern "C" int ivx_dev_flood_grow(const ivx_flood_plan *p, int dtype, const void *data, double t0, double t1,
                                  const int64_t *seeds_xyz, int64_t nseeds, uint64_t *cand, uint64_t *reached, void *scratch_,
                                  int *rounds, void *stream) {
    return flood_grow_impl(p, dtype, data, t0, t1, seeds_xyz, nseeds, cand, reached, scratch_, rounds, stream, AHEAD_CHAINED);
}
extern "C" int ivx_flood_look_ahead(int64_t n_list, int32_t *look_ahead) {
    IVX_REQUIRE(look_ahead && n_list >= 0, IVX_EINVAL, "flood_look_ahead: NULL or negative argument");
    *look_ahead = default_look_ahead(n_list > 0xffffffffll ? 0xffffffffu : (unsigned)n_list);
    return IVX_OK;
}
extern "C" int ivx_dev_flood_visits(const ivx_flood_plan *p, const void *scratch_, uint32_t out[2], void *stream) {
    IVX_REQUIRE(scratch_ && out, IVX_EINVAL, "flood_visits: NULL argument");
    Tiles t;
    int rc = make_tiles(p, &t);
    if (rc) return rc;
    out[0] = out[1] = 0u;
    if (t.ntiles == 0) return IVX_OK;
    const FScratch s = make_fscratch(t);
    hipStream_t st = ivx::S(stream);
    unsigned int w[CNT_CLEARED - STATS_AT];
    IVX_HIP(hipMemcpyAsync(w, (const char *)scratch_ + s.off_cnt + STATS_AT * 4, sizeof w, hipMemcpyDeviceToHost, st));
    IVX_HIP(hipStreamSynchronize(st));
    out[0] = w[0];
    for (int k = 0; k < HIST; k++) out[0] += w[HIST_AT - STATS_AT + k];
    out[1] = w[HIST_AT - STATS_AT];
    return IVX_OK;
}
extern "C" int ivx_flood_describe(const ivx_flood_plan *p, int64_t nseeds, int32_t out[8]) {
    IVX_REQUIRE(out, IVX_EINVAL, "flood_describe: NULL argument");
    Tiles t;
    int rc = make_tiles(p, &t);
    if (rc) return rc;
    for (int i = 0; i < 8; i++) out[i] = 0;
    if (coarse_ok(t, ivx::FLOOD_SYMMETRIC)) {
        const Blocks bk = coarse_blocks(t);
        const int ct = coarse_lanes(t);
        out[0] = 1;
        out[1] = bk.bxs;
        out[2] = bk.q;
        out[3] = ct;
        out[4] = (int32_t)ivx::cdiv(t.nty * t.ntz, (int64_t)ct);
    }
    out[5] = fused_start(t, nseeds) ? 1 : 0;
    out[6] = (int32_t)round_grid_cap(t);
    out[7] = (int32_t)t.ntiles;
    return IVX_OK;
}

extern "C" int ivx_dev_flood_run_edges(const ivx_flood_plan *p, const uint64_t *edges, uint64_t *reached, void *scratch_,
                                       int *rounds, void *stream) {
    return flood_run_impl(p, edges, ivx::FLOOD_DIRECTED, reached, scratch_, rounds, stream, nullptr, AHEAD_CHAINED);
}

extern "C" int ivx_flood_edges_bytes(const ivx_flood_plan *p, size_t *nbytes) {
// ... 55 lines not shown
extern "C" int ivx_dev_flood_disarm_gate(const void *scratch) {
    std::lock_guard<std::mutex> lk(g_gates_mu);
    g_gates.erase(scratch);
    return IVX_OK;
}
extern "C" int ivx_dev_gate_open(uint32_t *word, uint32_t value, void *stream) {
    IVX_REQUIRE(word, IVX_EINVAL, "gate_open: NULL argument");
    hipLaunchKernelGGL(k_gate_set, dim3(1), dim3(64), 0, ivx::S(stream), word, value);
    IVX_LAUNCH_CHECK();
    return IVX_OK;
}
extern "C" int ivx_dev_gate_wait(const uint32_t *word, uint32_t value, uint32_t timeout_us, void *stream) {
    IVX_REQUIRE(word, IVX_EINVAL, "gate_wait: NULL argument");
    hipLaunchKernelGGL(k_gate_wait, dim3(1), dim3(64), 0, ivx::S(stream), word, value, (unsigned long long)timeout_us * 100ull);
    IVX_LAUNCH_CHECK();
    return IVX_OK;
}

extern "C" int ivx_dev_flood_mark_slab(const ivx_flood_plan *p, void *scratch_, int64_t z0, int64_t z1, void *stream) {
    Tiles t;
    int rc = make_tiles(p, &t);
    if (rc) return rc;
    if (z0 < 0) z0 = 0;
    if (z1 > t.dz) z1 = t.dz;
    if (z1 <= z0 || t.ntiles == 0) return IVX_OK;
    const FScratch s = make_fscratch(t);
    const int64_t tz0 = z0 / TZ, tz1 = ivx::cdiv(z1, TZ);
    const int64_t n = (tz1 - tz0) * t.nty * t.wx;
    hipLaunchKernelGGL(k_flood_mark, dim3((unsigned)ivx::cdiv(n, 256)), dim3(256), 0, ivx::S(stream), t, tz0, tz1,
                       (uint8_t *)((char *)scratch_ + s.off_dirty0));
    IVX_LAUNCH_CHECK();
    return IVX_OK;
}

extern "C" int ivx_dev_flood_apply(const ivx_flood_plan *p, const uint64_t *reached, int dtype, void *target,
                                   double fill, void *stream) {
    Tiles t;
    int rc = make_tiles(p, &t);
    if (rc) return rc;
    const int64_t total = t.dz * t.dy * t.wx * 8;
    if (!total) return IVX_OK;
    const int g = grid_for(total);
    hipStream_t st = ivx::S(stream);
    const uint8_t *r = (const uint8_t *)reached;
    if (dtype == IVX_U8 && t.dx % 64 == 0 && ((uintptr_t)target & 15) == 0) {
        const int64_t nchunks = t.dz * t.dy * t.dx / 16;
        const int64_t blocks = ivx::cdiv(nchunks, 1024);
        hipLaunchKernelGGL(k_flood_apply16, dim3((unsigned)(blocks < 16384 ? blocks : 16384)), dim3(256), 0, st,
                           (const uint16_t *)reached, nchunks, (uint4 *)target, (uint8_t)fill);
        IVX_LAUNCH_CHECK();
        return IVX_OK;
    }
    switch (dtype) {
    case IVX_U8: hipLaunchKernelGGL(k_flood_apply<uint8_t>, dim3(g), dim3(256), 0, st, t, r, (uint8_t *)target, (uint8_t)fill); break;
    case IVX_I16: hipLaunchKernelGGL(k_flood_apply<int16_t>, dim3(g), dim3(256), 0, st, t, r, (int16_t *)target, (int16_t)fill); break;
    case IVX_U16: hipLaunchKernelGGL(k_flood_apply<uint16_t>, dim3(g), dim3(256), 0, st, t, r, (uint16_t *)target, (uint16_t)fill); break;
    case IVX_F64: hipLaunchKernelGGL(k_flood_apply<double>, dim3(g), dim3(256), 0, st, t, r, (double *)target, fill); break;
    default: ivx::set_error("flood: unsupported dtype %d", dtype); return IVX_EINVAL;
    }
    IVX_LAUNCH_CHECK();
    return IVX_OK;
}

extern "C" int ivx_dev_flood_apply_levels(const ivx_flood_plan *p, const uint64_t *reached, const uint64_t *inside_bits, uint8_t *mask,
                                          int v_in, int v_sel, void *stream) {
    Tiles t;
    int rc = make_tiles(p, &t);
    if (rc) return rc;
    if ((rc = levels_check(t, reached, inside_bits, mask, v_in, v_sel, false))) return rc;
    return launch_levels(t, reached, inside_bits, mask, v_in, v_sel, false, ApplyWhen{nullptr, nullptr, 0ull}, ivx::S(stream));
}

extern "C" int ivx_dev_mask_from_planes(const ivx_flood_plan *p, const uint64_t *inside_bits, const uint64_t *reached, uint8_t *mask,
                                        int v_in, int v_sel, void *stream) {
    Tiles t;
    int rc = make_tiles(p, &t);
    if (rc) return rc;
    if ((rc = levels_check(t, reached, inside_bits, mask, v_in, v_sel, true))) return rc;
    return launch_levels(t, reached, inside_bits, mask, v_in, v_sel, true, ApplyWhen{nullptr, nullptr, 0ull}, ivx::S(stream));
}

static int grow_select_impl(const ivx_flood_plan *p, int dtype, const void *data, double t0, double t1, const int64_t *seeds_xyz,
                            int64_t nseeds, uint64_t *cand, uint64_t *reached, void *scratch_, int *rounds, const ivx_flood_write *write,
                            int look_ahead, const ivx_mc_params *mc, void *mc_scratch, int *counted, void *stream) {
    IVX_REQUIRE(write && write->kind >= IVX_FLOOD_WRITE_NONE && write->kind <= IVX_FLOOD_WRITE_APPLY_U8, IVX_EINVAL,
                "flood_grow_select: no write description, or one of an unknown kind");
    IVX_REQUIRE(write->kind == IVX_FLOOD_WRITE_NONE || write->mask, IVX_EINVAL, "flood_grow_select: the write has no mask");
    if (counted) *counted = 0;
    EarlyWrite early = {write, false};
    const bool all = write->kind == IVX_FLOOD_WRITE_MASK_FROM_PLANES;
    const McRide ride = {mc, mc_scratch};
    Tiles t;
    int rc = make_tiles(p, &t);
    if (rc) return rc;
    if (mc && counted && (all || write->kind == IVX_FLOOD_WRITE_APPLY_LEVELS) &&
        levels_check(t, reached, write->inside_bits, write->mask, write->v_in, write->v_sel, all) == IVX_OK &&
        ivx::mc_ride_ok(mc, mc_scratch, t.dz, t.dy, t.dx)) {
        early.ride = &ride;
        ivx::mc_ride_begin(mc_scratch, write->inside_bits);
    }
    rc = flood_grow_impl(p, dtype, data, t0, t1, seeds_xyz, nseeds, cand, reached, scratch_, rounds, stream, look_ahead, &early);
    if (rc) return rc;
    const bool fused = early.ride && !early.plain;
    if (!early.written) {
        switch (write->kind) {
        case IVX_FLOOD_WRITE_MASK_FROM_PLANES:
        case IVX_FLOOD_WRITE_APPLY_LEVELS:
            if (fused)
                rc = launch_levels(t, reached, write->inside_bits, write->mask, write->v_in, write->v_sel, all, ApplyWhen{nullptr, nullptr, 0ull},
                                   ivx::S(stream), &ride);
            else if (all)
                rc = ivx_dev_mask_from_planes(p, write->inside_bits, reached, write->mask, write->v_in, write->v_sel, stream);
            else
                rc = ivx_dev_flood_apply_levels(p, reached, write->inside_bits, write->mask, write->v_in, write->v_sel, stream);
            break;
        case IVX_FLOOD_WRITE_APPLY_U8: rc = ivx_dev_flood_apply(p, reached, IVX_U8, write->mask, (double)write->v_sel, stream); break;
        default: break;
        }
        if (rc) return rc;
    }
    if (fused) {
        if ((rc = ivx::mc_ride_scan(mc, mc_scratch, ivx::S(stream)))) return rc;
        *counted = 1;
    }
    return IVX_OK;
}
extern "C" int ivx_dev_flood_grow_select(const ivx_flood_plan *p, int dtype, const void *data, double t0, double t1,
                                         const int64_t *seeds_xyz, int64_t nseeds, uint64_t *cand, uint64_t *reached,
                                         void *scratch_, int *rounds, const ivx_flood_write *write, int look_ahead, void *stream) {
    return grow_select_impl(p, dtype, data, t0, t1, seeds_xyz, nseeds, cand, reached, scratch_, rounds, write, look_ahead, nullptr, nullptr,
                            nullptr, stream);
}
extern "C" int ivx_dev_flood_grow_select_count(const ivx_flood_plan *p, int dtype, const void *data, double t0, double t1,
                                               const int64_t *seeds_xyz, int64_t nseeds, uint64_t *cand, uint64_t *reached,
                                               void *scratch_, int *rounds, const ivx_flood_write *write, int look_ahead,
                                               const ivx_mc_params *mc, void *mc_scratch, int *counted, void *stream) {
    IVX_REQUIRE(mc && mc_scratch && counted, IVX_EINVAL, "flood_grow_select_count: null piece, scratch or result");
    return grow_select_impl(p, dtype, data, t0, t1, seeds_xyz, nseeds, cand, reached, scratch_, rounds, write, look_ahead, mc, mc_scratch,
                            counted, stream);
}

extern "C" int ivx_dev_flood_apply2(const ivx_flood_plan *p, const uint64_t *reached, uint8_t *out, int fill,
                                    uint8_t *mask, int select, void *stream) {
    Tiles t;
    int rc = make_tiles(p, &t);
    if (rc) return rc;
    const int64_t total = t.dz * t.dy * t.wx * 8;
    if (!total) return IVX_OK;
    hipLaunchKernelGGL(k_flood_apply2, dim3(grid_for(total)), dim3(256), 0, ivx::S(stream), t, (const uint8_t *)reached, out,
                       (uint8_t)fill, mask, (uint8_t)select);
    IVX_LAUNCH_CHECK();
    return IVX_OK;
}

extern "C" int ivx_dev_flood_count(const ivx_flood_plan *p, const uint64_t *reached, int64_t *count, void *stream) {
    Tiles t;
    int rc = make_tiles(p, &t);
    if (rc) return rc;
    *count = 0;
    const int64_t nw = t.dz * t.dy * t.wx;
    if (!nw) return IVX_OK;
    void *d_tot;
    if ((rc = ivx::ws_get_s(ivx::WS_SMALL, ivx::S(stream), 64, &d_tot))) return rc;
    hipStream_t st = ivx::S(stream);
    IVX_HIP(hipMemsetAsync(d_tot, 0, 8, st));
    hipLaunchKernelGGL(k_flood_count, dim3(grid_for(nw)), dim3(256), 0, st, (const unsigned long long *)reached, nw,
                       (unsigned long long *)d_tot);
    IVX_LAUNCH_CHECK();
    unsigned long long h = 0;
    IVX_HIP(hipMemcpyAsync(&h, d_tot, 8, hipMemcpyDeviceToHost, st));
    IVX_HIP(hipStreamSynchronize(st));
    *count = (int64_t)h;
    return IVX_OK;
}

template <bool MARK>
__global__ __launch_bounds__(256) void k_flood_or_plane(unsigned long long *__restrict__ dst,
                                                        const unsigned long long *__restrict__ src,
                                                        const unsigned long long *__restrict__ cand, int64_t nwords,
                                                        unsigned int *__restrict__ changed, Tiles t, int64_t z,
                                                        uint8_t *__restrict__ dirty) {
    const int64_t i = (int64_t)blockIdx.x * blockDim.x + threadIdx.x;
    if (i >= nwords) return;
    const unsigned long long add = src[i] & cand[i] & ~dst[i];
    if (add) {
        dst[i] |= add;
        atomicAdd(changed, 1u);
        if (MARK) {
            const int64_t y = i / t.wx, txi = i - y * t.wx;
            mark_tile_nbhd(t, dirty, z / TZ, y / TY, txi);
        }
    }
}

__global__ __launch_bounds__(256) void k_bits_combine(unsigned long long *__restrict__ dst,
                                                      const unsigned long long *__restrict__ src, int64_t n, int op) {
    const int64_t stride = (int64_t)gridDim.x * blockDim.x;
    for (int64_t i = (int64_t)blockIdx.x * blockDim.x + threadIdx.x; i < n; i += stride)
        dst[i] = op == 0 ? (dst[i] | src[i]) : (dst[i] & ~src[i]);
}
extern "C" int ivx_dev_bits_combine(uint64_t *dst, const uint64_t *src, int64_t nwords, int op, void *stream) {
    IVX_REQUIRE(nwords >= 0 && (op == 0 || op == 1), IVX_EINVAL, "bits_combine: bad arguments");
    if (nwords == 0) return IVX_OK;
    const int64_t blocks = ivx::cdiv(nwords, 256);
    hipLaunchKernelGGL(k_bits_combine, dim3((unsigned)(blocks < 8192 ? blocks : 8192)), dim3(256), 0, ivx::S(stream),
                       (unsigned long long *)dst, (const unsigned long long *)src, nwords, op);
    IVX_LAUNCH_CHECK();
    return IVX_OK;
}

extern "C" int ivx_dev_flood_or_plane(const ivx_flood_plan *p, const uint64_t *cand, uint64_t *reached, int64_t z,
                                      const uint64_t *plane, void *scratch_, int *changed, void *stream) {
    Tiles t;
    int rc = make_tiles(p, &t);
    if (rc) return rc;
    IVX_REQUIRE(z >= 0 && z < t.dz, IVX_ERANGE, "flood: plane %lld outside slab", (long long)z);
    const FScratch s = make_fscratch(t);
    const int64_t nw = t.dy * t.wx;
    *changed = 0;
    if (!nw) return IVX_OK;
    hipStream_t st = ivx::S(stream);
    unsigned int *d_chg = (unsigned int *)((char *)scratch_ + s.off_status);
// ... 223 lines not shown
```

invesalius3_amd/csrc/k_mc.hip:

```cpp
#include <algorithm>

#include "levels_write.h"
#include "mc_common.h"

#define MC_TABLE_QUAL static __device__ __attribute__((aligned(16))) const
#include "../../include/ivx_mc_tables.h"

typedef short short8_t __attribute__((ext_vector_type(8)));
typedef unsigned char uchar16_t __attribute__((ext_vector_type(16)));

using namespace ivx;

namespace {

template <typename T, int NISO>
__global__ __launch_bounds__(256) void k_mc_bits(const T *__restrict__ a, int64_t nrows_src, int64_t nx, int64_t ws,
                                                 double iso0, double iso1, uint8_t *__restrict__ bits0,
                                                 uint8_t *__restrict__ bits1) {
    constexpr int V = 16 / sizeof(T);
    constexpr int OB = V / 8;
    const int64_t cpr = ws * 64 / V;
    const int64_t total = nrows_src * cpr;
    const int64_t stride = (int64_t)gridDim.x * blockDim.x;
    const bool vec = (nx % V == 0) && (((uintptr_t)a & 15) == 0);
    if (vec && ws * 64 == nx) {
        const int64_t nchunk = nrows_src * (nx / V);
        typedef T vec_t __attribute__((ext_vector_type(V)));
        const vec_t *src = reinterpret_cast<const vec_t *>(a);
        for (int64_t t0 = ((int64_t)blockIdx.x * blockDim.x) * 4 + threadIdx.x; t0 < nchunk; t0 += stride * 4) {
            vec_t x[4];
#pragma unroll
            for (int u = 0; u < 4; u++) {
                const int64_t t = t0 + (int64_t)u * blockDim.x;
                if (t < nchunk) x[u] = __builtin_nontemporal_load(&src[t]);
            }
#pragma unroll
            for (int u = 0; u < 4; u++) {
                const int64_t t = t0 + (int64_t)u * blockDim.x;
                if (t >= nchunk) continue;
                unsigned m0 = 0, m1 = 0;
#pragma unroll
                for (int e = 0; e < V; e++) {
                    const double d = (double)(T)x[u][e];
                    m0 |= d >= iso0 ? (1u << e) : 0u;
                    if (NISO == 2) m1 |= d >= iso1 ? (1u << e) : 0u;
                }
                if (OB == 1) {
                    bits0[t] = (uint8_t)m0;
                    if (NISO == 2) bits1[t] = (uint8_t)m1;
                } else {
                    reinterpret_cast<uint16_t *>(bits0)[t] = (uint16_t)m0;
                    if (NISO == 2) reinterpret_cast<uint16_t *>(bits1)[t] = (uint16_t)m1;
                }
            }
        }
        return;
    }
    for (int64_t t = (int64_t)blockIdx.x * blockDim.x + threadIdx.x; t < total; t += stride) {
        const int64_t row = t / cpr, q = t - row * cpr;
        const int64_t x0 = q * V;
        unsigned m0 = 0, m1 = 0;
        if (x0 < nx) {
            const T *r = a + row * nx + x0;
            T v[V];
            if (vec) {
                if (sizeof(T) == 2) {
                    const short8_t c = *reinterpret_cast<const short8_t *>(r);
#pragma unroll
                    for (int e = 0; e < V; e++) v[e] = (T)c[e % 8];
                } else {
                    const uchar16_t c = *reinterpret_cast<const uchar16_t *>(r);
#pragma unroll
                    for (int e = 0; e < V; e++) v[e] = (T)c[e % 16];
                }
            } else {
#pragma unroll
                for (int e = 0; e < V; e++) v[e] = (x0 + e < nx) ? r[e] : (T)0;
            }
#pragma unroll
            for (int e = 0; e < V; e++) {
                const bool valid = vec || (x0 + e < nx);
                const double d = (double)v[e];
                m0 |= (valid && d >= iso0) ? (1u << e) : 0u;
                if (NISO == 2) m1 |= (valid && d >= iso1) ? (1u << e) : 0u;
// ... 39 lines not shown
    const bool src1 = x1 - g.pxy < nx32;
    const int32_t wc = w32 >= ws32 ? (ws32 > 0 ? ws32 - 1 : 0) : w32;
    const int32_t wm = w32 - 1 >= ws32 ? (ws32 > 0 ? ws32 - 1 : 0) : (w32 - 1 < 0 ? 0 : w32 - 1);
    const int32_t wp = w32 + 1 >= ws32 ? (ws32 > 0 ? ws32 - 1 : 0) : w32 + 1;
    const int32_t ja0 = ((int32_t)g.NY - 1 - (int32_t)j) - g.pxy, ka0 = (int32_t)k - g.pb;
    const bool inner = ja0 - 1 >= 0 && ja0 < (int32_t)g.ny && ka0 >= 0 && ka0 + 1 < (int32_t)g.nz;
    if (__all(inner)) {
        const uint64_t padlo = pbits & exist & ~srcm;
        const bool use1 = exist1 && src1;
        const uint32_t nbpad = exist1 ? (uint32_t)pbits & 1u : 0u;
        const uint64_t *row = bits + (uint64_t)((uint32_t)ka0 * (uint32_t)g.ny + (uint32_t)ja0) * (uint64_t)(uint32_t)ws32;
        const uint64_t *pc = row + wc, *pa = row + (g.pxy ? wm : wp);
        const int64_t dj = -g.ws, dk = g.ny * g.ws;
        uint64_t a0[4], a1[4];
#pragma unroll
        for (int q = 0; q < 4; q++) {
            const int64_t d = ((q & 1) ? dj : 0) + ((q >> 1) ? dk : 0);
            a0[q] = pc[d];
            a1[q] = pa[d];
        }
#pragma unroll
        for (int q = 0; q < 4; q++) {
            uint64_t v0;
            uint32_t raw1;
            if (g.pxy) {
                v0 = mc_shl1(a0[q], (uint32_t)(a1[q] >> 32));
                raw1 = (uint32_t)(a0[q] >> 63);
            } else {
                v0 = a0[q];
                raw1 = (uint32_t)a1[q] & 1u;
            }
            const uint64_t lo = (v0 & srcm) | padlo;
            r.c[2 * q] = lo;
            r.c[2 * q + 1] = mc_shr1(lo, use1 ? raw1 : nbpad);
        }
    } else {
        const bool has_m = w32 - 1 >= 0 && w32 - 1 < ws32, has_c = w32 < ws32, has_p = w32 + 1 < ws32;
        uint64_t a0[4], a1[4];
        bool rin[4];
#pragma unroll
        for (int q = 0; q < 4; q++) {
            const int64_t ja = (g.NY - 1 - (j + (q & 1))) - g.pxy, ka = k + (q >> 1) - g.pb;
            rin[q] = ja >= 0 && ja < g.ny && ka >= 0 && ka < g.nz;
            const uint64_t *row = bits + (clampi(ka, g.nz) * g.ny + clampi(ja, g.ny)) * g.ws;
            a0[q] = row[wc];
            a1[q] = g.pxy ? row[wm] : row[wp];
        }
#pragma unroll
        for (int q = 0; q < 4; q++) {
            const uint64_t sc = (rin[q] && has_c) ? a0[q] : 0ull;
            uint64_t v0, raw1;
            if (g.pxy) {
                const uint64_t sm = (rin[q] && has_m) ? a1[q] : 0ull;
                v0 = (sc << 1) | (sm >> 63);
                raw1 = sc >> 63;
            } else {
                const uint64_t sp = (rin[q] && has_p) ? a1[q] : 0ull;
                v0 = sc;
                raw1 = sp & 1ull;
            }
            const uint64_t src = rin[q] ? srcm : 0ull;
            const uint64_t lo = (v0 & src) | (pbits & exist & ~src);
            const uint64_t nb = exist1 ? ((rin[q] && src1) ? raw1 : (pbits & 1ull)) : 0ull;
            r.c[2 * q] = lo;
            r.c[2 * q + 1] = (lo >> 1) | (nb << 63);
        }
    }
    uint64_t any = 0, all = ~0ull;
#pragma unroll
    for (int c = 0; c < 8; c++) {
        any |= r.c[c];
        all &= r.c[c];
    }
    r.active = any & ~all & mc_lowbits(NX32 - 1 - w32 * 64);
    return r;
}

struct McRideArgs {
    const uint16_t *reached, *inside;
    int64_t nchunks;
    uint4 *out;
    unsigned int in4, sel4;
};
template <bool RIDE, bool ALL>
__device__ __forceinline__ void mc_count_body(const uint64_t *__restrict__ bits, const Geom &g, size_t nwords, uint64_t pbits,
                                              uint16_t *__restrict__ counts, uint32_t *__restrict__ bsum, const McRideArgs &ride) {
    __shared__ uint32_t s_part[4], s_wcnt[4];
    __shared__ uint8_t s_ntri[256];
    __shared__ uint64_t s_c[256][5];
    __shared__ uint8_t s_hi[256];
    __shared__ uint16_t s_slot[256];
    const int tid = threadIdx.x, lane = tid & 63, wv = tid >> 6;
    const uint8_t ntri = MC_NTRI[tid];
    const int64_t ride_i0 = (int64_t)blockIdx.x * 1024 + tid;
    LevelsWords lw;
    if (RIDE) levels_load<ALL>(ride.reached, ride.inside, ride.nchunks, ride_i0, lw);
    auto ride_rest = [&]() {
        if (!RIDE) return;
        const int64_t stride = (int64_t)gridDim.x * 1024;
        for (int64_t i0 = ride_i0 + stride; i0 < ride.nchunks; i0 += stride) {
            LevelsWords w2;
            levels_load<ALL>(ride.reached, ride.inside, ride.nchunks, i0, w2);
            levels_store<ALL>(w2, ride.nchunks, i0, ride.out, ride.in4, ride.sel4);
        }
    };
    auto ride_store = [&]() {
#if !defined(IVX_RIDE_NO_STORES)
        if (RIDE) levels_store<ALL>(lw, ride.nchunks, ride_i0, ride.out, ride.in4, ride.sel4);
#endif
    };
    const size_t wid = (size_t)blockIdx.x * 256 + tid;
    uint64_t act = 0;
    Corner8 r;
    if (wid < nwords) {
        uint32_t k, j, w;
        mc_split_wid(g, (uint32_t)wid, k, j, w);
        r = load_corners(bits, g, (int64_t)k, (int64_t)j, (int64_t)w, pbits);
        act = r.active;
        if (!act) counts[wid] = 0;
    }
#if defined(IVX_RIDE_STORES_EARLY)
    ride_store();
#endif
    const unsigned long long am = __ballot(act != 0);
    if (lane == 0) s_wcnt[wv] = (uint32_t)__popcll(am);
    s_ntri[tid] = ntri;
    __syncthreads();
    uint32_t before = 0;
    for (int q = 0; q < wv; q++) before += s_wcnt[q];
    const uint32_t nact = s_wcnt[0] + s_wcnt[1] + s_wcnt[2] + s_wcnt[3];
#if !defined(IVX_RIDE_STORES_EARLY)
    ride_store();
#endif
#if defined(IVX_RIDE_NO_WALK)
    if (RIDE) {
        if (tid == 0) bsum[blockIdx.x] = 0;
        ride_rest();
        return;
    }
#endif
    if (!nact) {
        if (tid == 0) bsum[blockIdx.x] = 0;
        ride_rest();
        return;
    }
    if (act) {
        const uint32_t slot = before + (uint32_t)__popcll(am & ((1ull << lane) - 1ull));
        s_slot[slot] = (uint16_t)tid;
        uint32_t hi = 0;
#pragma unroll
        for (int q = 0; q < 4; q++) {
            s_c[slot][q] = r.c[2 * q];
            hi |= (uint32_t)(r.c[2 * q + 1] >> 63) << q;
        }
        s_c[slot][4] = act;
        s_hi[slot] = (uint8_t)hi;
    }
    __syncthreads();
    uint32_t n = 0;
    if ((uint32_t)tid < nact) {
        const uint64_t c0 = s_c[tid][0], c1 = s_c[tid][1], c2 = s_c[tid][2], c3 = s_c[tid][3];
        uint64_t a2 = s_c[tid][4];
        const uint32_t hi = s_hi[tid];
        while (a2) {
            const int b = __builtin_ctzll(a2);
            a2 &= a2 - 1;
            int idx;
            if (b != 63)
                idx = (int)((c0 >> b) & 3ull) | ((int)((c1 >> b) & 3ull) << 2) | ((int)((c2 >> b) & 3ull) << 4) | ((int)((c3 >> b) & 3ull) << 6);
            else
                idx = (int)(c0 >> 63) | ((int)(hi & 1u) << 1) | ((int)(c1 >> 63) << 2) | ((int)(hi >> 1 & 1u) << 3) | ((int)(c2 >> 63) << 4) |
                      ((int)(hi >> 2 & 1u) << 5) | ((int)(c3 >> 63) << 6) | ((int)(hi >> 3 & 1u) << 7);
            n += s_ntri[idx];
        }
        counts[(size_t)blockIdx.x * 256 + s_slot[tid]] = (uint16_t)n;
    }
    uint32_t s = n;
#pragma unroll
    for (int o = 32; o > 0; o >>= 1) s += __shfl_xor(s, o, 64);
    if (lane == 0) s_part[wv] = s;
    __syncthreads();
    if (tid == 0) bsum[blockIdx.x] = s_part[0] + s_part[1] + s_part[2] + s_part[3];
    ride_rest();
}
__global__ __launch_bounds__(256) void k_mc_count(const uint64_t *__restrict__ bits, Geom g, size_t nwords,
                                                  uint64_t pbits, uint16_t *__restrict__ counts,
                                                  uint32_t *__restrict__ bsum) {
    mc_count_body<false, false>(bits, g, nwords, pbits, counts, bsum, McRideArgs{});
}
template <bool ALL>
__global__ __launch_bounds__(256) void k_mc_count_write(const uint64_t *__restrict__ bits, Geom g, size_t nwords, uint64_t pbits,
                                                        uint16_t *__restrict__ counts, uint32_t *__restrict__ bsum, McRideArgs ride,
                                                        ApplyWhen when) {
    if (apply_when_skips(when)) return;
    mc_count_body<true, ALL>(bits, g, nwords, pbits, counts, bsum, ride);
}

__global__ __launch_bounds__(1024) void k_mc_scan(const uint32_t *__restrict__ bsum, size_t n,
                                                  uint64_t *__restrict__ boff, uint32_t *mb, uint32_t seq) {
    __shared__ uint64_t s_wave[16];
    __shared__ uint64_t s_carry;
    __shared__ uint32_t s_tot[64], s_exc[64];
    constexpr int RND = 4;
    const int lane = threadIdx.x & 63, wv = threadIdx.x >> 6;
    const size_t base = (size_t)blockIdx.x * (1024 * 4 * RND);
    uint64_t pre = 0;
    {
        const uint4 *b4 = reinterpret_cast<const uint4 *>(bsum);
        const size_t n4 = base / 4;
        uint64_t p0 = 0, p1 = 0, p2 = 0, p3 = 0;
        size_t i = threadIdx.x;
        for (; i + 3 * 1024 < n4; i += 4 * 1024) {
            const uint4 a = b4[i], b = b4[i + 1024], c = b4[i + 2048], d = b4[i + 3072];
            p0 += (uint64_t)a.x + a.y + a.z + a.w;
            p1 += (uint64_t)b.x + b.y + b.z + b.w;
            p2 += (uint64_t)c.x + c.y + c.z + c.w;
            p3 += (uint64_t)d.x + d.y + d.z + d.w;
        }
        for (; i < n4; i += 1024) {
            const uint4 a = b4[i];
            p0 += (uint64_t)a.x + a.y + a.z + a.w;
        }
        pre = p0 + p1 + p2 + p3;
    }
#pragma unroll
    for (int o = 32; o > 0; o >>= 1) pre += __shfl_xor(pre, o, 64);
    if (lane == 0) s_wave[wv] = pre;
    const bool al16 = ((uintptr_t)bsum & 15) == 0 && ((uintptr_t)boff & 15) == 0;
    uint32_t v[RND][4], inc[RND];
#pragma unroll
    for (int r = 0; r < RND; r++) {
        const size_t i0 = base + (size_t)r * 4096 + (size_t)threadIdx.x * 4;
        if (al16 && i0 + 3 < n) {
            const uint4 a = *reinterpret_cast<const uint4 *>(bsum + i0);
            v[r][0] = a.x; v[r][1] = a.y; v[r][2] = a.z; v[r][3] = a.w;
        } else {
#pragma unroll
            for (int q = 0; q < 4; q++) v[r][q] = i0 + q < n ? bsum[i0 + q] : 0u;
        }
    }
#pragma unroll
    for (int r = 0; r < RND; r++) {
        inc[r] = v[r][0] + v[r][1] + v[r][2] + v[r][3];
#pragma unroll
        for (int o = 1; o < 64; o <<= 1) {
            const uint32_t t = __shfl_up(inc[r], o, 64);
            if (lane >= o) inc[r] += t;
        }
        if (lane == 63) s_tot[r * 16 + wv] = inc[r];
    }
    __syncthreads();
    if (wv == 0) {
        const uint32_t t = s_tot[lane];
        uint32_t e = t;
#pragma unroll
        for (int o = 1; o < 64; o <<= 1) {
            const uint32_t u = __shfl_up(e, o, 64);
            if (lane >= o) e += u;
        }
        s_exc[lane] = e - t;
        uint64_t c = 0;
        for (int q = 0; q < 16; q++) c += s_wave[q];
        if (lane == 0) s_carry = c;
        if (lane == 63 && base + 1024 * 4 * RND >= n) {
            const uint64_t total = c + e;
            boff[n] = total;
            if (mb) {
                mb[0] = (uint32_t)total;
                mb[1] = (uint32_t)(total >> 32);
                __threadfence_system();
                __hip_atomic_store(&mb[63], seq, __ATOMIC_RELEASE, __HIP_MEMORY_SCOPE_SYSTEM);
            }
        }
    }
    __syncthreads();
    const uint64_t carry = s_carry;
#pragma unroll
    for (int r = 0; r < RND; r++) {
        const size_t i0 = base + (size_t)r * 4096 + (size_t)threadIdx.x * 4;
        const uint32_t lanesum = v[r][0] + v[r][1] + v[r][2] + v[r][3];
        const uint64_t o0 = carry + (uint64_t)(s_exc[r * 16 + wv] + inc[r] - lanesum);
        const uint64_t o1 = o0 + v[r][0], o2 = o1 + v[r][1], o3 = o2 + v[r][2];
        if (al16 && i0 + 3 < n) {
            typedef unsigned long long u64x2_t __attribute__((ext_vector_type(2)));
            u64x2_t *d = reinterpret_cast<u64x2_t *>(boff + i0);
            d[0] = u64x2_t{o0, o1};
            d[1] = u64x2_t{o2, o3};
        } else {
            if (i0 < n) boff[i0] = o0;
            if (i0 + 1 < n) boff[i0 + 1] = o1;
            if (i0 + 2 < n) boff[i0 + 2] = o2;
            if (i0 + 3 < n) boff[i0 + 3] = o3;
        }
    }
}

constexpr int MCL_CHUNK = 256;
constexpr int MCL_CELLS = 2048;
__device__ __forceinline__ uint32_t mcl_wave_scan(uint32_t v) {
    v += (uint32_t)__builtin_amdgcn_update_dpp(0, (int)v, 0x111, 0xf, 0xf, false);
    v += (uint32_t)__builtin_amdgcn_update_dpp(0, (int)v, 0x112, 0xf, 0xf, false);
    v += (uint32_t)__builtin_amdgcn_update_dpp(0, (int)v, 0x114, 0xf, 0xf, false);
    v += (uint32_t)__builtin_amdgcn_update_dpp(0, (int)v, 0x118, 0xf, 0xf, false);
    v += (uint32_t)__builtin_amdgcn_update_dpp(0, (int)v, 0x142, 0xa, 0xf, false);
    v += (uint32_t)__builtin_amdgcn_update_dpp(0, (int)v, 0x143, 0xc, 0xf, false);
    return v;
}
__global__ __launch_bounds__(256) void k_mc_list(const uint64_t *__restrict__ bits, Geom g, size_t nwords, uint64_t pbits,
                                                 const uint16_t *__restrict__ counts, const uint64_t *__restrict__ boff,
                                                 uint64_t *__restrict__ list, uint64_t max_tris) {
    __shared__ uint32_t s_wave[4], s_part[2][4];
    __shared__ uint8_t s_ntri[256];
    __shared__ uint64_t s_c[4][256];
    __shared__ uint8_t s_hi[256];
    __shared__ uint64_t s_pre[256];
    __shared__ uint16_t s_cell[MCL_CELLS];
    const int tid = threadIdx.x, lane = tid & 63, wv = tid >> 6;
    const uint8_t ntri = MC_NTRI[tid];
    const size_t wid0 = (size_t)blockIdx.x * 256;
    const uint32_t n = wid0 + tid < nwords ? (uint32_t)counts[wid0 + tid] : 0u;
    const uint64_t pos0 = boff[blockIdx.x];
    if (boff[blockIdx.x + 1] == pos0 || pos0 >= max_tris) return;
    uint64_t a2 = 0;
    if (n) {
        uint32_t k, j, w;
        mc_split_wid(g, (uint32_t)(wid0 + tid), k, j, w);
        const Corner8 r = load_corners(bits, g, (int64_t)k, (int64_t)j, (int64_t)w, pbits);
        a2 = r.active;
        uint32_t hi = 0;
#pragma unroll
        for (int q = 0; q < 4; q++) {
            s_c[q][tid] = r.c[2 * q];
            hi |= (uint32_t)(r.c[2 * q + 1] >> 63) << q;
        }
        s_hi[tid] = (uint8_t)hi;
        s_pre[tid] = ((uint64_t)k << 48) | ((uint64_t)j << 32) | ((uint64_t)w << 17);
    }
    const uint32_t pc = (uint32_t)__popcll(a2);
    const uint32_t inc = mcl_wave_scan(pc);
    if (lane == 63) s_wave[wv] = inc;
    s_ntri[tid] = ntri;
    __syncthreads();
    uint32_t ci = inc - pc;
    for (int q = 0; q < wv; q++) ci += s_wave[q];
    const uint32_t ncell = s_wave[0] + s_wave[1] + s_wave[2] + s_wave[3];
    uint64_t P = pos0;
    int par = 0;
    for (uint32_t sb = 0; sb < ncell; sb += MCL_CELLS) {
        const uint32_t se = sb + MCL_CELLS < ncell ? sb + MCL_CELLS : ncell;
        while (a2 && ci < se) {
            const int b = __builtin_ctzll(a2);
            a2 &= a2 - 1;
            s_cell[ci - sb] = (uint16_t)((tid << 6) | b);
            ci++;
        }
        __syncthreads();
        for (uint32_t cb = sb; cb < se; cb += MCL_CHUNK) {
            const uint32_t c = cb + tid;
            uint32_t nt = 0;
            uint64_t d0 = 0;
            if (c < se) {
                const uint32_t rec = s_cell[c - sb], sl = rec >> 6;
                const int b = (int)(rec & 63u);
                const uint64_t c0 = s_c[0][sl], c1 = s_c[1][sl], c2 = s_c[2][sl], c3 = s_c[3][sl];
                int idx;
                if (b != 63) {
                    idx = (int)((c0 >> b) & 3ull) | ((int)((c1 >> b) & 3ull) << 2) | ((int)((c2 >> b) & 3ull) << 4) | ((int)((c3 >> b) & 3ull) << 6);
                } else {
                    const uint32_t hi = s_hi[sl];
                    idx = (int)(c0 >> 63) | ((int)(hi & 1u) << 1) | ((int)(c1 >> 63) << 2) | ((int)(hi >> 1 & 1u) << 3) | ((int)(c2 >> 63) << 4) |
                          ((int)(hi >> 2 & 1u) << 5) | ((int)(c3 >> 63) << 6) | ((int)(hi >> 3 & 1u) << 7);
                }
                nt = s_ntri[idx];
                d0 = s_pre[sl] | ((uint64_t)b << 11) | ((uint64_t)idx << 3);
            }
            const uint32_t ti = mcl_wave_scan(nt);
            if (lane == 63) s_part[par][wv] = ti;
            __syncthreads();
            uint32_t off = ti - nt;
            for (int q = 0; q < wv; q++) off += s_part[par][q];
            const uint32_t tot = s_part[par][0] + s_part[par][1] + s_part[par][2] + s_part[par][3];
            const uint64_t p0 = P + off;
#pragma unroll
            for (uint32_t t = 0; t < MC_MAX_TRI; t++)
                if (t < nt && p0 + t < max_tris) list[p0 + t] = d0 | t;
            P += tot;
            if (P >= max_tris) return;
            par ^= 1;
        }
    }
}

template <typename T, bool LEVELS>
__device__ __forceinline__ void mc_triangle(const T *__restrict__ a, const Geom &g, const McLevels &lv, double iso,
                                            const uint8_t *s_tri, const int *s_e0, const int *s_e1, const int *s_ec, int32_t k,
                                            int32_t j, int32_t i, int idx, int rel, float *o) {
    const int32_t ka = k - (int32_t)g.pb, ja = ((int32_t)g.NY - 1 - j) - (int32_t)g.pxy;
    const int32_t ia = i - (int32_t)g.pxy;
    const bool fast = ka >= 0 && ka + 1 < (int32_t)g.nz && ja - 1 >= 0 && ja < (int32_t)g.ny && ia >= 0 &&
                      ia + 1 < (int32_t)g.nx;
    double s0[3], s1[3];
    int ec[3];
#pragma unroll
    for (int v = 0; v < 3; v++) ec[v] = s_tri[idx * 15 + 3 * rel + v];
    double ttl[3];
    if (LEVELS) {
#pragma unroll
        for (int v = 0; v < 3; v++) {
            const int c = s_ec[ec[v]];
            const int ax = c & 3, bx = (c >> 2) & 1, by = (c >> 3) & 1, bz = (c >> 4) & 1;
            const int lo = bx + 2 * by + 4 * bz;
            const bool in0 = (idx >> lo) & 1, in1 = (idx >> (lo + (1 << ax))) & 1;
            const int32_t kk = k + bz + (in1 && ax == 2), jj = j + by + (in1 && ax == 1), ii = i + bx + (in1 && ax == 0);
            const int64_t sk = kk - (int32_t)g.pb, sj = ((int32_t)g.NY - 1 - jj) - (int32_t)g.pxy, si = ii - (int32_t)g.pxy;
            const uint64_t wsel = lv.sel[(sk * g.ny + sj) * g.ws + (si >> 6)];
            ttl[v] = lv.tt[(in0 ? 2 : 0) + (int)((wsel >> (si & 63)) & 1ull)];
            ec[v] = c;
        }
    } else if (fast) {
        const T *cell = a + ((int64_t)ka * g.ny + ja) * g.nx + ia;
#pragma unroll
        for (int v = 0; v < 3; v++) {
            s0[v] = (double)cell[s_e0[ec[v]]];
            s1[v] = (double)cell[s_e1[ec[v]]];
        }
#pragma unroll
        for (int v = 0; v < 3; v++) ec[v] = s_ec[ec[v]];
    } else {
#pragma unroll
        for (int v = 0; v < 3; v++) {
            const int c = s_ec[ec[v]];
            const int ax = c & 3, bx = (c >> 2) & 1, by = (c >> 3) & 1, bz = (c >> 4) & 1;
            s0[v] = mc_at(a, g, k + bz, j + by, i + bx);
            s1[v] = mc_at(a, g, k + bz + (ax == 2), j + by + (ax == 1), i + bx + (ax == 0));
            ec[v] = c;
        }
    }
#pragma unroll
    for (int v = 0; v < 3; v++) {
        const int ax = ec[v] & 3, bx = (ec[v] >> 2) & 1, by = (ec[v] >> 3) & 1, bz = (ec[v] >> 4) & 1;
        const double tt = LEVELS ? ttl[v] : (iso - s0[v]) / (s1[v] - s0[v]);
        double p0 = (double)(i + bx - (int32_t)g.pxy);
        double p1 = (double)(j + by - (int32_t)g.yoff);
        double p2 = (double)(k + bz + g.zoff);
        if (ax == 0) p0 += tt;
        else if (ax == 1) p1 += tt;
        else p2 += tt;
        o[3 * v + 0] = (float)(g.sx * p0);
        o[3 * v + 1] = (float)(g.sy * p1);
        o[3 * v + 2] = (float)(g.sz * p2);
    }
}

template <typename T, bool LEVELS>
__global__ __launch_bounds__(256) void k_mc_emit(const T *__restrict__ a, Geom g, double iso0, double iso1,
                                                 const uint64_t *__restrict__ split_dev,
                                                 const uint64_t *__restrict__ total_dev,
                                                 const uint64_t *__restrict__ list, uint64_t cap,
                                                 float *__restrict__ tris, McLevels lv) {
    __shared__ __attribute__((aligned(16))) uint8_t s_tri[256 * 15];
    __shared__ __attribute__((aligned(16))) float s_out[256 * 9];
    const int tid = threadIdx.x;
    const uint64_t total = *total_dev, split = *split_dev;
    const uint64_t ntris = total < cap ? total : cap;
    const uint64_t T0 = (uint64_t)blockIdx.x * 256;
    if (T0 >= ntris) return;
#pragma unroll
    for (int q = 0; q < 4; q++)
        if (q * 256 + tid < 960) ((uint32_t *)s_tri)[q * 256 + tid] = ((const uint32_t *)&MC_TRI[0][0])[q * 256 + tid];
    const uint64_t T_ = T0 + tid;
    const double iso = T_ < split ? iso0 : iso1;
    __shared__ int s_e0[12], s_e1[12], s_ec[12];
    const int plane32 = (int)(g.ny * g.nx), nx32 = (int)g.nx;
// ... 46 lines not shown
        hipLaunchKernelGGL((k_mc_bits<T, 1>), dim3(grid), dim3(256), 0, st, (const T *)a, nrows_src, g.nx, g.ws,
                           iso0, 0.0, b0, b0);
    IVX_LAUNCH_CHECK();
    return IVX_OK;
}

template <typename T>
static int run_emit(const ivx_mc_params *p, const Geom &g, const Scratch &s, const void *a, const char *scratch,
                    float *tris, int64_t max_tris, hipStream_t st, const McLevels *lv) {
    const uint64_t *boff = (const uint64_t *)(scratch + s.off_boff);
    void *d_list;
    int rc = ws_get_s(WS_MCLIST, st, (size_t)max_tris * 8 + 64, &d_list);
    if (rc) return rc;
    const size_t nb = s.nblocks * (size_t)p->niso;
    if (!mc_pieces().list_ready(scratch, d_list, max_tris))
        if ((rc = mc_queue_list(p, g, s, scratch, d_list, max_tris, st))) return rc;
    if (lv)
        hipLaunchKernelGGL((k_mc_emit<T, true>), dim3((unsigned)ivx::cdiv(max_tris, (int64_t)256)), dim3(256), 0, st, (const T *)a, g,
                           p->iso[0], p->iso[1], boff + (p->niso == 2 ? s.nblocks : nb), boff + nb, (const uint64_t *)d_list,
                           (uint64_t)max_tris, tris, *lv);
    else
        hipLaunchKernelGGL((k_mc_emit<T, false>), dim3((unsigned)ivx::cdiv(max_tris, (int64_t)256)), dim3(256), 0, st, (const T *)a, g,
                           p->iso[0], p->iso[1], boff + (p->niso == 2 ? s.nblocks : nb), boff + nb, (const uint64_t *)d_list,
                           (uint64_t)max_tris, tris, McLevels{nullptr, 0.0, 0.0, 0.0, {0.0, 0.0, 0.0, 0.0}});
    IVX_LAUNCH_CHECK();
    return IVX_OK;
}

}

namespace ivx {

int mc_piece_layout(const ivx_mc_params *p, Geom *g, Scratch *s, bool *empty) {
    int rc = make_geom(p, g);
    if (rc) return rc;
    *s = make_scratch(*g, p->niso);
    *empty = s->nwords == 0;
    if (*empty) return IVX_OK;
    IVX_REQUIRE(s->nblocks * (size_t)p->niso < 0x7fffffffull, IVX_EINVAL, "mc: piece too large for one launch");
    IVX_REQUIRE(s->nwords < 0xffffffffull, IVX_EINVAL, "mc: piece too large for 32-bit cell-word ids");
    return IVX_OK;
}

int mc_inside_planes(const ivx_mc_params *p, const Geom &g, const Scratch &s, const void *a, void *dst, double iso0, double iso1,
                     hipStream_t st) {
    return MC_BY_DTYPE(p->dtype, run_bits, p, g, s, a, (uint8_t *)dst, iso0, iso1, st);
}

int mc_queue_list(const ivx_mc_params *p, const Geom &g, const Scratch &s, const void *scratch_, void *d_list, int64_t max_tris,
                  hipStream_t st) {
    const char *scratch = (const char *)scratch_;
    const uint64_t *boff = (const uint64_t *)(scratch + s.off_boff);
    for (int q = 0; q < p->niso; q++) {
        const uint64_t *bits = mc_bits_ptr(scratch, s, q);
        const uint16_t *counts = (const uint16_t *)(scratch + s.off_counts) + (size_t)q * s.nwords;
        hipLaunchKernelGGL(k_mc_list, dim3((unsigned)s.nblocks), dim3(256), 0, st, bits, g, s.nwords, pad_bits(p, q), counts,
                           boff + (size_t)q * s.nblocks, (uint64_t *)d_list, (uint64_t)max_tris);
        IVX_LAUNCH_CHECK();
    }
    return IVX_OK;
}

int mc_upload_piece(const ivx_mc_params *p, const void *a, const int64_t strides[3], void **d_a, void **d_scr) {
    size_t sb;
    int rc = ivx_dev_mc_scratch_bytes(p, &sb);
    if (rc) return rc;
    const size_t isz = dtype_size(p->dtype);
    const int64_t shape[3] = {p->nz, p->ny, p->nx};
    if ((rc = ws_get(WS_IN, (size_t)p->nz * p->ny * p->nx * isz, d_a))) return rc;
    if ((rc = ws_get(WS_AUX0, sb, d_scr))) return rc;
    return upload_strided(*d_a, a, shape, strides, isz, WS_IN);
}

}

extern "C" int ivx_mc_split_word_ids(const ivx_mc_params *p, const uint32_t *wid, size_t n, uint32_t *k, uint32_t *j, uint32_t *w) {
    Geom g;
    int rc = make_geom(p, &g);
    if (rc) return rc;
    for (size_t i = 0; i < n; i++) mc_split_wid(g, wid[i], k[i], j[i], w[i]);
    return IVX_OK;
}

extern "C" int ivx_dev_mc_scratch_bytes(const ivx_mc_params *p, size_t *nbytes) {
    Geom g;
    int rc = make_geom(p, &g);
    if (rc) return rc;
    *nbytes = make_scratch(g, p->niso).total;
    return IVX_OK;
}

static int mc_read_total(const ivx_mc_params *p, const Scratch &s, void *scratch_, int64_t *ntris, hipStream_t st) {
    char *scratch = (char *)scratch_;
    int rc;
    uint64_t *boff = (uint64_t *)(scratch + s.off_boff);
    const size_t nb = s.nblocks * (size_t)p->niso;
    uint32_t seq, tw[2];
    if (p->niso == 2) {
        uint32_t seq0, t0[2];
        if ((rc = ivx::mailbox_publish(boff + s.nblocks, 2, st, &seq0))) return rc;
        if ((rc = ivx::mailbox_wait(seq0, st, t0, 2))) return rc;
        mc_pieces().set_split(scratch_, ((uint64_t)t0[1] << 32) | t0[0]);
    }
    if ((rc = ivx::mailbox_publish(boff + nb, 2, st, &seq))) return rc;
    if ((rc = ivx::mailbox_wait(seq, st, tw, 2))) return rc;
    *ntris = (int64_t)(((uint64_t)tw[1] << 32) | tw[0]);
    return IVX_OK;
}

static int mc_read_total_early(const ivx_mc_params *p, const Scratch &s, void *scratch_, int64_t *ntris, hipStream_t st) {
    const uint32_t seq = p->niso == 1 ? mc_pieces().total_seq(scratch_) : 0u;
    if (seq) {
        uint32_t tw[2];
        int got = 0;
        const int rc = ivx::mailbox_wait_reserved(seq, st, tw, 2, &got);
        if (rc) return rc;
        if (got) {
            *ntris = (int64_t)(((uint64_t)tw[1] << 32) | tw[0]);
            return IVX_OK;
        }
    }
    return mc_read_total(p, s, scratch_, ntris, st);
}

static void mc_count_record(void *scratch_, const uint64_t *inside_bits) { mc_pieces().begin_count(scratch_, inside_bits); }
static int mc_count_launch(const ivx_mc_params *p, const Geom &g, const Scratch &s, void *scratch_, hipStream_t st) {
    char *scratch = (char *)scratch_;
    uint32_t *bsum = (uint32_t *)(scratch + s.off_bsum);
    for (int q = 0; q < p->niso; q++) {
        const uint64_t *bits = mc_bits_ptr(scratch, s, q);
        uint16_t *counts = (uint16_t *)(scratch + s.off_counts) + (size_t)q * s.nwords;
        hipLaunchKernelGGL(k_mc_count, dim3((unsigned)s.nblocks), dim3(256), 0, st, bits, g, s.nwords, pad_bits(p, q),
                           counts, bsum + (size_t)q * s.nblocks);
        IVX_LAUNCH_CHECK();
    }
    return IVX_OK;
}
static int mc_count_scan(const ivx_mc_params *p, const Scratch &s, void *scratch_, hipStream_t st) {
    char *scratch = (char *)scratch_;
    uint32_t *bsum = (uint32_t *)(scratch + s.off_bsum);
    uint64_t *boff = (uint64_t *)(scratch + s.off_boff);
    const size_t nb = s.nblocks * (size_t)p->niso;
    uint32_t *mb = nullptr, seq = 0;
    if (p->niso == 1) {
        int rc = ivx::mailbox_reserve(&mb, &seq);
        if (rc) return rc;
        mc_pieces().set_total_seq(scratch_, seq);
    }
    hipLaunchKernelGGL(k_mc_scan, dim3((unsigned)std::max<size_t>(1, (nb + 16383) / 16384)), dim3(1024), 0, st, bsum, nb, boff, mb,
                       seq);
    IVX_LAUNCH_CHECK();
    return IVX_OK;
}

static int mc_count_impl(const ivx_mc_params *p, const void *a, const uint64_t *inside_bits, void *scratch_, int64_t *ntris,
                         void *stream) {
    Geom g;
    Scratch s;
    bool empty;
    int rc = mc_piece_layout(p, &g, &s, &empty);
    if (rc) return rc;
    IVX_REQUIRE(!inside_bits || p->niso == 1, IVX_EINVAL, "mc_count_bits: one iso-value only");
    if (ntris) *ntris = 0;
    if (empty) return IVX_OK;
    IVX_REQUIRE(a || inside_bits, IVX_EINVAL, "mc_count: neither voxels nor an inside plane");
    char *scratch = (char *)scratch_;
    hipStream_t st = S(stream);
    mc_count_record(scratch_, inside_bits);
    if (!inside_bits && (rc = mc_inside_planes(p, g, s, a, scratch + s.off_bits, p->iso[0], p->iso[1], st))) return rc;
    if ((rc = mc_count_launch(p, g, s, scratch_, st))) return rc;
    if ((rc = mc_count_scan(p, s, scratch_, st))) return rc;
    return ntris ? mc_read_total_early(p, s, scratch_, ntris, st) : IVX_OK;
}

bool ivx::mc_ride_ok(const ivx_mc_params *p, const void *scratch, int64_t dz, int64_t dy, int64_t dx) {
    Geom g;
    Scratch s;
    bool empty;
    if (!p || !scratch || mc_piece_layout(p, &g, &s, &empty) != IVX_OK || empty) return false;
    return p->niso == 1 && p->ny == dy && p->nx == dx && p->nz <= dz;
}
void ivx::mc_ride_begin(void *scratch, const uint64_t *inside_bits) { mc_count_record(scratch, inside_bits); }
int ivx::mc_ride_launch(const ivx_mc_params *p, void *scratch_, const uint64_t *reached, const uint64_t *inside, int64_t nchunks,
                        uint8_t *mask, int v_in, int v_sel, bool all, const ApplyWhen &when, hipStream_t st) {
    Geom g;
    Scratch s;
    bool empty;
    int rc = mc_piece_layout(p, &g, &s, &empty);
    if (rc) return rc;
    IVX_REQUIRE(!empty && p->niso == 1 && nchunks > 0, IVX_EINVAL, "mc_ride: an empty piece or volume, or two iso-values");
    char *scratch = (char *)scratch_;
    const McRideArgs ride = {(const uint16_t *)reached, (const uint16_t *)inside, nchunks, (uint4 *)mask, 0x01010101u * (uint8_t)v_in,
                             0x01010101u * (uint8_t)v_sel};
    auto k = all ? k_mc_count_write<true> : k_mc_count_write<false>;
    hipLaunchKernelGGL(k, dim3((unsigned)s.nblocks), dim3(256), 0, st, mc_bits_ptr(scratch, s, 0), g, s.nwords, pad_bits(p, 0),
                       (uint16_t *)(scratch + s.off_counts), (uint32_t *)(scratch + s.off_bsum), ride, when);
    IVX_LAUNCH_CHECK();
    return IVX_OK;
}
int ivx::mc_ride_scan(const ivx_mc_params *p, void *scratch, hipStream_t st) {
    Geom g;
    Scratch s;
    bool empty;
    int rc = mc_piece_layout(p, &g, &s, &empty);
    if (rc) return rc;
    return mc_count_scan(p, s, scratch, st);
}

extern "C" int ivx_dev_mc_count(const ivx_mc_params *p, const void *a, void *scratch_, int64_t *ntris, void *stream) {
    return mc_count_impl(p, a, nullptr, scratch_, ntris, stream);
}
extern "C" int ivx_dev_mc_count_async(const ivx_mc_params *p, const void *a, void *scratch_, void *stream) {
    return mc_count_impl(p, a, nullptr, scratch_, nullptr, stream);
}
extern "C" int ivx_dev_mc_total(const ivx_mc_params *p, void *scratch_, int64_t *ntris, void *stream) {
    Geom g;
    Scratch s;
    bool empty;
    int rc = mc_piece_layout(p, &g, &s, &empty);
    if (rc) return rc;
    *ntris = 0;
    return empty ? IVX_OK : mc_read_total(p, s, scratch_, ntris, S(stream));
}
extern "C" int ivx_dev_mc_total_early(const ivx_mc_params *p, void *scratch_, int64_t *ntris, void *stream) {
    Geom g;
    Scratch s;
    bool empty;
    int rc = mc_piece_layout(p, &g, &s, &empty);
    if (rc) return rc;
    *ntris = 0;
    return empty ? IVX_OK : mc_read_total_early(p, s, scratch_, ntris, S(stream));
}

extern "C" int ivx_dev_mc_count_bits(const ivx_mc_params *p, const uint64_t *inside_bits, void *scratch_, int64_t *ntris,
                                     void *stream) {
    return mc_count_impl(p, nullptr, inside_bits, scratch_, ntris, stream);
}
extern "C" int ivx_dev_mc_count_bits_async(const ivx_mc_params *p, const uint64_t *inside_bits, void *scratch_, void *stream) {
    return mc_count_impl(p, nullptr, inside_bits, scratch_, nullptr, stream);
}

extern "C" int ivx_dev_mc_emit(const ivx_mc_params *p, const void *a, const void *scratch, float *tris,
                               int64_t max_tris, void *stream) {
    Geom g;
    Scratch s;
    bool empty;
    int rc = mc_piece_layout(p, &g, &s, &empty);
    if (rc) return rc;
    if (empty || max_tris <= 0) return IVX_OK;
    return MC_BY_DTYPE(p->dtype, run_emit, p, g, s, a, (const char *)scratch, tris, max_tris, S(stream), nullptr);
}

extern "C" int ivx_dev_mc_emit_levels(const ivx_mc_params *p, const void *scratch, const uint64_t *sel_bits, double v_out,
                                      double v_in, double v_sel, float *tris, int64_t max_tris, void *stream) {
    Geom g;
    Scratch s;
    bool empty;
    int rc = mc_piece_layout(p, &g, &s, &empty);
    if (rc) return rc;
    IVX_REQUIRE(p->dtype == IVX_U8 && p->niso == 1 && sel_bits, IVX_EINVAL, "mc_emit_levels: uint8 mask, one iso-value");
    IVX_REQUIRE(v_out < p->iso[0] && v_in >= p->iso[0] && v_sel >= p->iso[0] && (double)p->pad_value == v_out, IVX_EINVAL,
                "mc_emit_levels: v_out must lie below the iso-value and equal the padding value, v_in and v_sel at or above it");
    if (empty || max_tris <= 0) return IVX_OK;
    const McLevels lv = make_levels(sel_bits, p->iso[0], v_out, v_in, v_sel);
    return run_emit<uint8_t>(p, g, s, nullptr, (const char *)scratch, tris, max_tris, S(stream), &lv);
}

extern "C" int ivx_dev_mc_list(const ivx_mc_params *p, const void *scratch, int64_t max_tris, void *stream) {
    Geom g;
    Scratch s;
    bool empty;
    int rc = mc_piece_layout(p, &g, &s, &empty);
    if (rc) return rc;
    if (empty || max_tris <= 0) return IVX_OK;
    hipStream_t st = S(stream);
    void *d_list;
    if ((rc = ws_get_s(WS_MCLIST, st, (size_t)max_tris * 8 + 64, &d_list))) return rc;
    if ((rc = mc_queue_list(p, g, s, scratch, d_list, max_tris, st))) return rc;
    mc_pieces().list_built(scratch, d_list, max_tris);
    return IVX_OK;
}

// ... 53 lines not shown
```

invesalius3_amd/device.py:

```python
from __future__ import annotations

import ctypes
import os
from typing import NamedTuple, Optional

import numpy as np

from . import _lib as L
from .mc_ride import RideBook


class _MaskLevels(NamedTuple):
    v_in: float
    sel: Optional[ctypes.c_void_p]
    v_sel: float

    @property
    def has_second(self):
        return self.sel is not None


class DeviceBuffer:

    def __init__(self, nbytes: int):
# ... 109 lines not shown
        def __exit__(self, *a):
            return False

    _OFF = _Off()

    def _ev(self):
        if self._pool:
            return self._pool.pop()
        e = ctypes.c_void_p()
        L.check(L.lib().ivx_event_create(ctypes.byref(e)))
        return e

    class _Span:
        def __init__(self, t, name):
            self.t, self.name = t, name

        def __enter__(self):
            self.e0 = self.t._ev()
            L.check(L.lib().ivx_event_record(self.e0, self.t.stream))

        def __exit__(self, *a):
            e1 = self.t._ev()
            L.check(L.lib().ivx_event_record(e1, self.t.stream))
            self.t.spans.append((self.name, self.e0, e1))

    def records(self, name) -> bool:
        return self.only is None or name in self.only

    def span(self, name):
        if not self.records(name):
            return Timer._OFF
        return Timer._Span(self, name)

    def collect(self) -> dict:
        out = {}
        for name, e0, e1 in self.spans:
            ms = ctypes.c_float(0)
            L.check(L.lib().ivx_event_elapsed_ms(e0, e1, ctypes.byref(ms)))
            out.setdefault(name, []).append(ms.value)
            self._pool += [e0, e1]
        self.spans = []
        return out


class DeviceVolume:

    def __init__(self, image: np.ndarray | None = None, shape=None, spacing=(1.0, 1.0, 1.0), device: int | None = None):
        L.require_device()
        if device is not None:
            L.set_device(device)
        if image is not None:
            if image.dtype != np.int16 or image.ndim != 3:
                raise TypeError("image must be a 3-D int16 array")
            shape = image.shape
        self.shape = tuple(int(s) for s in shape)
        self.dz, self.dy, self.dx = self.shape
        self.n = self.dz * self.dy * self.dx
        self.spacing = tuple(float(s) for s in spacing)
        s = ctypes.c_void_p()
        L.check(L.lib().ivx_stream_create(ctypes.byref(s)))
        self.stream = s
        self.timer = Timer(self.stream)
        self._mbits_valid = False
        self._mbits_range = None
        self._mask_levels = None
        self._out_bytes_zero = False
        self._mc_params_cache = {}
        self._stream2 = None
        self._sync_events = []
        self._prefetch = None
        self._gate = None
        self._gate_epoch = 0
        self._gate_armed = False
        self._mbits_version = 0
        self._out_pending = None
        self._mask_pending = False
        self._defer_pays = True
        self._fuse = os.environ.get("IVX_NO_FUSE", "") == ""
        self._apply_levels = os.environ.get("IVX_APPLY_LEVELS", "1") != "0"
        self._use_ranges = os.environ.get("IVX_RANGES", "1") != "0"
        self._mask_defer = os.environ.get("IVX_MASK_DEFER", "1") != "0"
        self._select = os.environ.get("IVX_FLOOD_SELECT", "1") != "0"
        self._ride = RideBook(os.environ.get("IVX_MC_RIDE", "1") != "0")
        self._look_ahead = -1
        self._ranges = None
        self._ranges_valid = False
        self.image = TrackedBuffer(self.n * 2, self._image_touched)
        self.mask = TrackedBuffer(self.n, self._mask_touched, self._mask_read)
        self.out_mask = TrackedBuffer(self.n, self._out_touched)
        if image is not None:
            self.image.upload_view(image)
        self.mask.zero(self.stream)
        self.zero_out_mask()
        self.plan = L.FloodPlan(self.dz, self.dy, self.dx, (self.dx + 63) // 64, 0)
        nb, ns = ctypes.c_size_t(0), ctypes.c_size_t(0)
        L.check(L.lib().ivx_flood_bits_bytes(ctypes.byref(self.plan), ctypes.byref(nb)))
        L.check(L.lib().ivx_flood_scratch_bytes(ctypes.byref(self.plan), ctypes.byref(ns)))
        self.cand = DeviceBuffer(nb.value)
        self.reached = DeviceBuffer(nb.value)
        self._mbits = DeviceBuffer(nb.value)
        self._plane_words = nb.value // 8
        self.flood_scratch = DeviceBuffer(ns.value)
        self._mc_scratch = None
        self._tris = None
        self._verts = None
        self._faces = None
        self._range_buf = None
        self._range_valid = False
        self.sync()

    def _image_touched(self):
        self._mbits_range = None
        self._range_valid = False
        self._ranges_valid = False
        self._drop_volren()

    def _mask_touched(self):
        self._mask_read()
        self._mp_cells_valid = False
        self._mbits_valid = False
        self._mbits_range = None
        self._mask_levels = None
        self._mbits_version += 1

    def _materialize_mask(self):
        if self._mask_pending:
            self._defer_pays = False
            lv = self._mask_levels
            sel = self.reached.ptr if lv[1] is not None else None
            with self.timer.span("mask_bytes"):
                L.check(L.lib().ivx_dev_mask_from_planes(ctypes.byref(self.plan), self._mbits.ptr, sel, self.mask.raw, int(lv[0]),
                                                         int(lv[0] if lv[1] is None else lv[1]), self.stream), "mask_from_planes")
            self._mask_pending = False

    def _mask_read(self):
        if self._mask_pending:
            self._materialize_mask()
            self.sync()

    def mask_bytes(self) -> ctypes.c_void_p:
        self._materialize_mask()
        return self.mask.raw

    def _out_logically_zero(self) -> bool:
        return self._out_bytes_zero and self._out_pending is None

    def _materialize_out(self):
        if self._out_pending is not None:
            L.check(L.lib().ivx_dev_flood_apply(ctypes.byref(self.plan), self.reached.ptr, L.U8, self.out_mask.raw,
                                                ctypes.c_double(self._out_pending), self.stream))
            self._out_pending = None
            self._out_bytes_zero = False

    def _out_touched(self):
        self._materialize_out()
        self._out_bytes_zero = False

    def zero_out_mask(self):
        self._materialize_mask()
        if not self._out_bytes_zero:
            L.check(L.lib().ivx_memset(self.out_mask.raw, 0, ctypes.c_size_t(self.n), self.stream))
        self._out_bytes_zero, self._out_pending = True, None

    def sync(self):
        self._materialize_mask()
        L.check(L.lib().ivx_stream_synchronize(self.stream))
# ... 51 lines not shown
        return history.snapshot_device(self.mask_bytes(), self.n, self.shape, self.stream)

    def restore_mask(self, snapshot):
        if snapshot.closed:
            raise ValueError("restore_mask: the snapshot has been closed")
        if snapshot.n != self.n or tuple(snapshot.shape) != self.shape:
            raise ValueError("restore_mask: the snapshot holds shape %r, the volume has %r" % (tuple(snapshot.shape), self.shape))
        self._materialize_mask()
        L.check(L.lib().ivx_dev_mask_snapshot_restore(self.mask.raw, self.n, snapshot.header.ptr, snapshot.pool.ptr,
                                                      snapshot.literal_blocks, 1, None, self.stream), "restore_mask")
        self._mask_touched()

    def download_out_mask(self) -> np.ndarray:
        self._materialize_mask()
        self._materialize_out()
        self.sync()
        return self.out_mask.download(self.shape, np.uint8)

    def threshold(self, lo: int, hi: int, preserve: bool = False):
        lib = L.lib()
        self._join_prefetch()
        if self._fuse and not preserve and self.dx % 64 == 0:
            self._mbits_version += 1
            self._mp_cells_valid = False
            dims = (c64(self.dz), c64(self.dy), c64(self.dx), int(lo), int(hi))
            defer = self._mask_defer and self._defer_pays
            if self._use_ranges:
                mode = 1 if self._ranges_valid else 0
                if defer:
                    L.check(lib.ivx_dev_threshold_i16_plane_ranges(self.image.raw, *dims, self._mbits.ptr, self._ranges_buffer().ptr,
                                                                   mode, self.stream), "threshold")
                else:
                    L.check(lib.ivx_dev_threshold_i16_bits_ranges(self.image.raw, *dims, self.mask.raw, self._mbits.ptr,
                                                                  self._ranges_buffer().ptr, mode, self.stream), "threshold")
                self._ranges_valid = True
            elif defer:
                L.check(lib.ivx_dev_threshold_i16_plane(self.image.raw, *dims, self._mbits.ptr, self.stream), "threshold")
            else:
                L.check(lib.ivx_dev_threshold_i16_bits(self.image.raw, *dims, self.mask.raw, self._mbits.ptr, self.stream), "threshold")
            self._mask_pending = defer
            self._mbits_valid, self._mbits_range = True, (int(lo), int(hi))
            self._mask_levels = (255, None)
            return
        if preserve:
            self._materialize_mask()
        self._mask_pending = False
        L.check(lib.ivx_dev_threshold_i16(self.image.raw, c64(self.dz), c64(self.dy), c64(self.dx), int(lo), int(hi),
                                          int(bool(preserve)), None, self.mask.raw, self.stream), "threshold")
        self._mask_touched()

    def _ranges_buffer(self) -> DeviceBuffer:
        if self._ranges is None:
            nb = ctypes.c_size_t(0)
            L.check(L.lib().ivx_image_ranges_bytes(c64(self.dz), c64(self.dy), c64(self.dx), ctypes.byref(nb)), "image_ranges_bytes")
            self._ranges = DeviceBuffer(max(nb.value, 4))
            self._ranges_valid = False
        return self._ranges

    def lut_image_255(self, ww, wl) -> DeviceBuffer:
        self._materialize_mask()
        buf = DeviceBuffer(self.n * 2)
        L.check(L.lib().ivx_dev_lut_i16(self.image.raw, c64(self.n), ctypes.c_double(float(ww)), ctypes.c_double(float(wl)),
                                        1, buf.ptr, self.stream), "lut_image_255")
        return buf

    def region_grow(self, seeds_xyz, t0, t1, strct, fill: int = 1, select_value: int | None = 254,
                    image: DeviceBuffer | None = None) -> int:
        lib = L.lib()
        img_ptr = image.ptr if image is not None else self.image.raw
        s3 = np.ascontiguousarray(strct, dtype=np.uint8)
        bits = ctypes.c_uint32(0)
        L.check(lib.ivx_flood_strct_bits(L.ptr(s3), L.i64(s3.shape), ctypes.byref(bits)))
        self.plan.strct_bits = bits.value
        seeds = np.ascontiguousarray(np.array([tuple(s) for s in seeds_xyz], dtype=np.int64).reshape(-1, 3))
        p = ctypes.byref(self.plan)
        st = self.stream
        t0, t1 = float(int(t0)), float(int(t1))
        self._before_flood()
        cand, shared = self._candidate_plane(image, t0, t1, fill)
        rounds = ctypes.c_int(0)
        write = self._flood_write(fill, select_value) if self._select else None
        piece = self._piece_to_ride(write, shared, select_value)
        if piece is not None:
            counted = ctypes.c_int(0)
            L.check(lib.ivx_dev_flood_grow_select_count(p, L.I16, img_ptr, ctypes.c_double(t0), ctypes.c_double(t1), L.ptr(seeds),
                                                        c64(len(seeds)), cand.ptr, self.reached.ptr, self.flood_scratch.ptr,
                                                        ctypes.byref(rounds), ctypes.byref(write), int(self._look_ahead),
                                                        ctypes.byref(piece[0]), self._mc_scratch.ptr, ctypes.byref(counted), st),
                    "region_grow")
            if counted.value:
                self._ride.rode(self._mbits_version)
            else:
                self._ride.drop()
        elif write is not None:
            L.check(lib.ivx_dev_flood_grow_select(p, L.I16, img_ptr, ctypes.c_double(t0), ctypes.c_double(t1), L.ptr(seeds),
                                                  c64(len(seeds)), cand.ptr, self.reached.ptr, self.flood_scratch.ptr,
                                                  ctypes.byref(rounds), ctypes.byref(write), int(self._look_ahead), st), "region_grow")
        else:
            L.check(lib.ivx_dev_flood_grow(p, L.I16, img_ptr, ctypes.c_double(t0), ctypes.c_double(t1), L.ptr(seeds),
                                           c64(len(seeds)), cand.ptr, self.reached.ptr, self.flood_scratch.ptr,
                                           ctypes.byref(rounds), st), "region_grow")
        self._gate_armed = False
        self._apply_reached(fill, select_value, shared, queued=write is not None)
        return rounds.value

    def _piece_to_ride(self, write, shared, select_value):
        if (write is None or write.kind not in (L.FLOOD_WRITE_MASK_FROM_PLANES, L.FLOOD_WRITE_APPLY_LEVELS) or not shared
                or select_value is None or int(select_value) < 127 or not self._fuse or self._prefetch is not None
                or self._mc_scratch is None or self._tris is None or self.timer.records("mc_count")
                or self.timer.records("mask_bytes")):
            return None
        piece = self._ride.piece_to_ride()
        if piece is None or piece[1] != 0 or piece[0].ny != self.dy or piece[0].nx != self.dx or piece[0].nz > self.dz:
            return None
        return piece

    def flood_visits(self):
        self._materialize_mask()
        return L.flood_visits(self.plan, self.flood_scratch.ptr, self.stream)

    def _before_flood(self):
        self._materialize_out()
        if self._mask_levels is not None and self._mask_levels[1] is not None:
            self._materialize_mask()
            self._mask_levels = None

    def _candidate_plane(self, image, t0, t1, fill):
        shared = (image is None and self._mbits_valid and self._out_logically_zero() and int(fill) != 0
                  and self._mbits_range == (int(t0), int(t1)))
        if shared:
            return self._mbits, True
        bar, bar_mode = (None, 0) if (self._out_logically_zero() and (int(fill) & 0xff) != 0) else (self.out_mask.raw, 1)
        if image is None and self._use_ranges and self._ranges_valid:
            L.check(L.lib().ivx_dev_flood_candidates_ranges(ctypes.byref(self.plan), self.image.raw, ctypes.c_double(t0),
                                                            ctypes.c_double(t1), bar, bar_mode, ctypes.c_double(fill),
                                                            self._ranges.ptr, self.cand.ptr, self.stream), "flood_candidates_ranges")
            return self.cand, False
        img_ptr = image.ptr if image is not None else self.image.raw
        L.check(L.lib().ivx_dev_flood_candidates(ctypes.byref(self.plan), L.I16, img_ptr, ctypes.c_double(t0),
                                                 ctypes.c_double(t1), bar, bar_mode, ctypes.c_double(fill),
                                                 self.cand.ptr, self.stream))
        return self.cand, False

    def _write_kind(self, fill, select_value):
        if not (self._out_logically_zero() and int(fill) != 0):
            return None
        if select_value is not None and self._mask_levels == (255, None) and self._mbits_valid and self._apply_levels:
            return L.FLOOD_WRITE_MASK_FROM_PLANES if self._mask_pending else L.FLOOD_WRITE_APPLY_LEVELS
        return L.FLOOD_WRITE_APPLY_U8 if select_value is not None else L.FLOOD_WRITE_NONE

    def _flood_write(self, fill, select_value):
        kind = self._write_kind(fill, select_value)
        if kind is None or (kind == L.FLOOD_WRITE_MASK_FROM_PLANES and self.timer.records("mask_bytes")):
            return None
        if kind == L.FLOOD_WRITE_APPLY_U8:
            self._materialize_mask()
        return L.FloodWrite(kind=kind, v_in=255, v_sel=int(select_value) if select_value is not None else 0,
                            inside_bits=self._mbits.ptr.value, mask=self.mask.raw.value)

    def _apply_reached(self, fill, select_value, shared, queued=False):
        lib, p, st = L.lib(), ctypes.byref(self.plan), self.stream
        if select_value is not None:
            self._mp_cells_valid = False
        kind = self._write_kind(fill, select_value)
        assert kind is not None or not queued
        if kind not in (L.FLOOD_WRITE_MASK_FROM_PLANES, L.FLOOD_WRITE_APPLY_LEVELS):
            self._materialize_mask()
        else:
            self._defer_pays = True
        if kind is not None:
            self._out_pending = int(fill)
            if kind == L.FLOOD_WRITE_MASK_FROM_PLANES:
                if not queued:
                    with self.timer.span("mask_bytes"):
                        L.check(lib.ivx_dev_mask_from_planes(p, self._mbits.ptr, self.reached.ptr, self.mask.raw, 255,
                                                             int(select_value), st), "mask_from_planes")
                self._mask_pending = False
            elif kind == L.FLOOD_WRITE_APPLY_LEVELS and not queued:
                L.check(lib.ivx_dev_flood_apply_levels(p, self.reached.ptr, self._mbits.ptr, self.mask.raw, 255, int(select_value), st),
                        "flood_apply_levels")
            elif kind == L.FLOOD_WRITE_APPLY_U8 and not queued:
                L.check(lib.ivx_dev_flood_apply(p, self.reached.ptr, L.U8, self.mask.raw, ctypes.c_double(int(select_value)), st))
        elif select_value is not None:
            L.check(lib.ivx_dev_flood_apply2(p, self.reached.ptr, self.out_mask.raw, int(fill), self.mask.raw,
                                             int(select_value), st))
            self._out_bytes_zero = False
        else:
            L.check(lib.ivx_dev_flood_apply(p, self.reached.ptr, L.U8, self.out_mask.raw, ctypes.c_double(fill), st))
            self._out_bytes_zero = False
        if select_value is not None:
            lv = self._mask_levels
            self._mask_levels = (lv[0], int(select_value)) if (lv is not None and lv[1] is None and int(select_value) >= 127
                                                                and self._mbits_valid) else None
# ... 872 lines not shown
```

invesalius3_amd/mc_ride.py:

```python
from __future__ import annotations


class RideBook:
    def __init__(self, enabled: bool = True):
        self.enabled = bool(enabled)
        self.armed = None
        self.note = None
        self.rides = 0
        self.taken = 0

    def piece_to_ride(self):
        return self.armed if self.enabled else None

    def rode(self, version: int):
        self.note = (self.armed[0], self.armed[1], int(version))
        self.armed = None
        self.rides += 1

    def take(self, params, z0: int, version: int) -> bool:
        n, self.note = self.note, None
        ok = n is not None and n[0] is params and n[1] == z0 and n[2] == int(version)
        self.taken += int(ok)
        return ok

    def drop(self):
        self.note = None

    def surface_counted(self, params, z0: int, from_plane: bool):
        self.armed = (params, z0) if (self.enabled and from_plane) else None
```

Before: 446,900 Mvoxel/s.

## Fuse marching-cubes count into coarse flood pass and build triangle list during level write

New measurement: 473,500 Mvoxel/s, median of 5. 1.06x the previous value.

```diff
diff --git a/include/ivx.h b/include/ivx.h
--- a/include/ivx.h
+++ b/include/ivx.h
@@ -131,6 +131,7 @@
     double iso[2];
 } ivx_mc_params;
 int ivx_dev_mc_scratch_bytes(const ivx_mc_params *p, size_t *nbytes);
+int ivx_mc_scratch_layout(const ivx_mc_params *p, size_t out[4]);
 int ivx_mc_split_word_ids(const ivx_mc_params *p, const uint32_t *wid, size_t n, uint32_t *k, uint32_t *j, uint32_t *w);
 int ivx_dev_mc_count(const ivx_mc_params *p, const void *a, void *scratch, int64_t *ntris, void *stream);
 int ivx_dev_mc_count_async(const ivx_mc_params *p, const void *a, void *scratch, void *stream);
@@ -418,6 +419,12 @@
                                     const int64_t *seeds_xyz, int64_t nseeds, uint64_t *cand, uint64_t *reached, void *scratch,
                                     int *rounds, const ivx_flood_write *write, int look_ahead, const ivx_mc_params *mc,
                                     void *mc_scratch, int *counted, void *stream);
+enum { IVX_FLOOD_FRONT_COUNT = 1, IVX_FLOOD_WRITE_LIST = 2 };
+int ivx_dev_flood_grow_select_list(const ivx_flood_plan *p, int dtype, const void *data, double t0, double t1,
+                                   const int64_t *seeds_xyz, int64_t nseeds, uint64_t *cand, uint64_t *reached, void *scratch,
+                                   int *rounds, const ivx_flood_write *write, int look_ahead, const ivx_mc_params *mc,
+                                   void *mc_scratch, int flags, int64_t max_tris, int64_t did[3], void *stream);
+int ivx_flood_front_describe(const ivx_flood_plan *p, int64_t nseeds, int32_t out[4]);
 int ivx_flood_look_ahead(int64_t n_list, int32_t *look_ahead);
 int ivx_dev_flood_apply2(const ivx_flood_plan *p, const uint64_t *reached, uint8_t *out, int fill, uint8_t *mask,
                          int select, void *stream);
diff --git a/invesalius3_amd/_lib.py b/invesalius3_amd/_lib.py
--- a/invesalius3_amd/_lib.py
+++ b/invesalius3_amd/_lib.py
@@ -33,6 +33,7 @@
 
 
 FLOOD_WRITE_NONE, FLOOD_WRITE_MASK_FROM_PLANES, FLOOD_WRITE_APPLY_LEVELS, FLOOD_WRITE_APPLY_U8 = 0, 1, 2, 3
+FLOOD_FRONT_COUNT, FLOOD_WRITE_LIST = 1, 2
 
 
 class FloodWrite(ctypes.Structure):
@@ -95,6 +96,11 @@
                                                             c_vp, c_i64, c_vp, c_vp, c_vp, ctypes.POINTER(ctypes.c_int),
                                                             ctypes.POINTER(FloodWrite), ctypes.c_int, ctypes.POINTER(McParams), c_vp,
                                                             ctypes.POINTER(ctypes.c_int), c_vp]),
+                       ("ivx_dev_flood_grow_select_list", [ctypes.POINTER(FloodPlan), ctypes.c_int, c_vp, ctypes.c_double, ctypes.c_double,
+                                                           c_vp, c_i64, c_vp, c_vp, c_vp, ctypes.POINTER(ctypes.c_int),
+                                                           ctypes.POINTER(FloodWrite), ctypes.c_int, ctypes.POINTER(McParams), c_vp,
+                                                           ctypes.c_int, c_i64, i64p, c_vp]),
+                       ("ivx_flood_front_describe", [ctypes.POINTER(FloodPlan), c_i64, ctypes.POINTER(ctypes.c_int32)]),
                        ("ivx_flood_look_ahead", [c_i64, ctypes.POINTER(ctypes.c_int32)]),
                        ("ivx_dev_image_flip", [c_vp, c_i64, c_i64, c_i64, sz, ctypes.c_int, c_vp]),
                        ("ivx_image_flip", [c_vp, i64p, i64p, sz, ctypes.c_int]),
@@ -243,3 +249,9 @@
     out = (ctypes.c_uint32 * 2)()
     check(lib().ivx_dev_flood_visits(ctypes.byref(plan), scratch, out, stream), "flood_visits")
     return int(out[0]), int(out[1])
+
+
+def flood_front_describe(plan: FloodPlan, nseeds: int):
+    out = (ctypes.c_int32 * 4)()
+    check(lib().ivx_flood_front_describe(ctypes.byref(plan), int(nseeds), out), "flood_front_describe")
+    return bool(out[0]), int(out[1]), int(out[2]), int(out[3])
diff --git a/invesalius3_amd/csrc/flood_coarse.h b/invesalius3_amd/csrc/flood_coarse.h
--- /dev/null
+++ b/invesalius3_amd/csrc/flood_coarse.h
@@ -0,0 +1,106 @@
+#pragma once
+#include <hip/hip_runtime.h>
+#include <stdint.h>
+
+namespace ivx {
+
+constexpr int COARSE_CRP = 8;
+
+struct SeedPack {
+    int64_t xyz[16][3];
+    int n;
+};
+
+struct CoarseArgs {
+    int nty, ntz;
+    int bxs;
+    int ty, tz;
+    const unsigned long long *rowF;
+    unsigned long long *rowW;
+    const unsigned int *seed_ok;
+};
+
+__device__ __forceinline__ unsigned long long fill_up(unsigned long long seed, unsigned long long m) {
+    return (((m + seed) ^ m) & m) | seed;
+}
+__device__ __forceinline__ unsigned long long fill_runs(unsigned long long seed, unsigned long long m) {
+    unsigned long long f = fill_up(seed, m);
+    return __brevll(fill_up(__brevll(f), __brevll(m)));
+}
+
+template <int CONN>
+__device__ __forceinline__ void coarse_body_lean(const CoarseArgs &a, const SeedPack &sp, unsigned long long *sR, unsigned int *vote) {
+    constexpr int CRP = COARSE_CRP;
+    const int nty = a.nty, ntz = a.ntz, hy = nty + 2;
+    const int nrows = nty * ntz, nh = hy * (ntz + 2);
+    const unsigned long long *__restrict__ rowF = a.rowF;
+    unsigned long long *__restrict__ rowW = a.rowW;
+    unsigned long long F[CRP];
+    int me[CRP];
+#pragma unroll
+    for (int k = 0; k < CRP; k++) {
+        const int j = threadIdx.x + k * (int)blockDim.x;
+        F[k] = j < nrows ? rowF[j] : 0ull;
+        me[k] = j < nrows ? (j / nty + 1) * hy + (j % nty) + 1 : 0;
+    }
+    for (int i = threadIdx.x; i < nh; i += blockDim.x) sR[i] = 0ull;
+    if (threadIdx.x == 0) vote[0] = 0u;
+    __syncthreads();
+    if ((int)threadIdx.x < sp.n && (*a.seed_ok >> threadIdx.x & 1u)) {
+        const int64_t x = sp.xyz[threadIdx.x][0], y = sp.xyz[threadIdx.x][1], z = sp.xyz[threadIdx.x][2];
+        const int j = (int)((z / a.tz) * nty + y / a.ty);
+        const unsigned long long bit = 1ull << (x / a.bxs);
+        if (rowF[j] & bit) atomicOr(&sR[(j / nty + 1) * hy + (j % nty) + 1], bit);
+    }
+    __syncthreads();
+#pragma unroll
+    for (int k = 0; k < CRP; k++) {
+        const unsigned long long r = sR[me[k]];
+        if (r && me[k]) sR[me[k]] = fill_runs(r, F[k]);
+    }
+    __syncthreads();
+    for (int it = 0; it < 65536; it++) {
+        bool changed = false;
+        int hyl = hy;
+        asm volatile("" : "+s"(hyl));
+#pragma unroll
+        for (int k = 0; k < CRP; k++) {
+            unsigned long long Fk = F[k];
+            asm volatile("" : "+v"(Fk));
+            const unsigned long long r = sR[me[k]];
+            if (!(Fk & ~r)) continue;
+            unsigned long long nw = 0, nm = 0;
+#pragma unroll
+            for (int kk = -1; kk <= 1; kk++)
+#pragma unroll
+                for (int jj = -1; jj <= 1; jj++) {
+                    const int nz = (kk != 0) + (jj != 0);
+                    const bool wide = CONN == 26 || (CONN == 18 && nz <= 1) || (CONN == 6 && nz == 0);
+                    const bool mid = (CONN == 18 && nz == 2) || (CONN == 6 && nz == 1);
+                    if (!wide && !mid) continue;
+                    const unsigned long long n = sR[me[k] + kk * hyl + jj];
+                    if (wide) nw |= n;
+                    else nm |= n;
+                }
+            const unsigned long long nb = nw | (nw << 1) | (nw >> 1) | nm;
+            const unsigned long long nr = fill_runs(r | (nb & Fk), Fk);
+            if (nr != r) {
+                sR[me[k]] = nr;
+                changed = true;
+            }
+        }
+        if (__any(changed) && (threadIdx.x & 63) == 0) vote[it & 1] = 1u;
+        if (threadIdx.x == 0) vote[(it + 1) & 1] = 0u;
+        __syncthreads();
+        const bool more = vote[it & 1] != 0u;
+        __syncthreads();
+        if (!more) break;
+    }
+    int tid = threadIdx.x;
+    asm volatile("" : "+v"(tid));
+#pragma unroll
+    for (int k = 0; k < CRP; k++)
+        if (me[k] != 0) rowW[tid + k * (int)blockDim.x] = sR[me[k]];
+}
+
+}
diff --git a/invesalius3_amd/csrc/ivx_internal.h b/invesalius3_amd/csrc/ivx_internal.h
--- a/invesalius3_amd/csrc/ivx_internal.h
+++ b/invesalius3_amd/csrc/ivx_internal.h
@@ -98,6 +98,16 @@
 int mc_ride_launch(const ivx_mc_params *p, void *scratch, const uint64_t *reached, const uint64_t *inside, int64_t nchunks, uint8_t *mask,
                    int v_in, int v_sel, bool all, const ApplyWhen &when, hipStream_t st);
 int mc_ride_scan(const ivx_mc_params *p, void *scratch, hipStream_t st);
+struct CoarseArgs;
+struct SeedPack;
+bool mc_front_fits(int64_t nty, int64_t ntz);
+int mc_front_lanes();
+int mc_front_launch(const ivx_mc_params *p, void *scratch, const CoarseArgs &ca, const SeedPack &sp, int conn, hipStream_t st);
+int mc_ride_list_buffer(int64_t max_tris, hipStream_t st, void **list);
+int mc_ride_list_launch(const ivx_mc_params *p, void *scratch, void *list, int64_t max_tris, const uint64_t *reached,
+                        const uint64_t *inside, int64_t nchunks, uint8_t *mask, int v_in, int v_sel, bool all, const ApplyWhen &when,
+                        hipStream_t st);
+void mc_ride_list_built(const void *scratch, const void *list, int64_t max_tris);
 
 int mailbox_publish(const void *dsrc, int ndwords, hipStream_t st, uint32_t *seq_out);
 int mailbox_wait(uint32_t seq, hipStream_t st, uint32_t *out, int ndwords);
diff --git a/invesalius3_amd/csrc/k_flood.hip b/invesalius3_amd/csrc/k_flood.hip
--- a/invesalius3_amd/csrc/k_flood.hip
+++ b/invesalius3_amd/csrc/k_flood.hip
@@ -1,13 +1,18 @@
 #include <math.h>
 #include <map>
+#include <algorithm>
 #include <mutex>
 #include <stdlib.h>
 
+#include "flood_coarse.h"
 #include "flood_tiles.h"
 #include "levels_write.h"
 #include "words_from_records.h"
 
 using ivx::ApplyWhen;
+using ivx::fill_runs;
+using ivx::fill_up;
+using ivx::SeedPack;
 
 namespace {
 
@@ -157,10 +162,6 @@
     mark_tile_nbhd(t, dirty, z / TZ, y / TY, x >> 6);
 }
 
-struct SeedPack {
-    int64_t xyz[16][3];
-    int n;
-};
 template <typename T>
 __global__ void k_flood_seed_args(const T *__restrict__ data, Tiles t, double t0, double t1, SeedPack sp,
                                   unsigned long long *__restrict__ cand, unsigned long long *__restrict__ reached,
@@ -177,13 +178,6 @@
     mark_tile_nbhd(t, dirty, z / TZ, y / TY, x >> 6);
 }
 
-__device__ __forceinline__ unsigned long long fill_up(unsigned long long seed, unsigned long long m) {
-    return (((m + seed) ^ m) & m) | seed;
-}
-__device__ __forceinline__ unsigned long long fill_runs(unsigned long long seed, unsigned long long m) {
-    unsigned long long f = fill_up(seed, m);
-    return __brevll(fill_up(__brevll(f), __brevll(m)));
-}
 
 __device__ __forceinline__ void lds_barrier() {
     __builtin_amdgcn_s_waitcnt(0xC07F);
@@ -605,7 +599,7 @@
     if (i < n) dirty[tz0 * per + i] = 1;
 }
 
-constexpr int CT = 1024, CRP = 8, CROWS_MAX = 7680;
+constexpr int CT = 1024, CRP = ivx::COARSE_CRP, CROWS_MAX = 7680;
 constexpr unsigned int ENLISTED = 0x80u;
 
 struct Blocks {
@@ -715,6 +709,10 @@
     }
 }
 
+__host__ __device__ __forceinline__ ivx::CoarseArgs coarse_args(const Tiles &t, const Blocks &bk, const unsigned long long *rowF,
+                                                               unsigned long long *rowW, const unsigned int *seed_ok) {
+    return ivx::CoarseArgs{(int)t.nty, (int)t.ntz, bk.bxs, TY, TZ, rowF, rowW, seed_ok};
+}
 template <int CONN, bool SEEDED>
 __global__ __launch_bounds__(CT) void k_flood_coarse(Tiles t, Blocks bk, const unsigned long long *__restrict__ rowF,
                                                      unsigned long long *__restrict__ rowW, SeedPack sp,
@@ -1292,9 +1290,12 @@
     while (ct < CT && ct < t.nty * t.ntz) ct *= 2;
     return ct;
 }
+struct McRide;
+static int front_launch(const Tiles &t, const Blocks &bk, const McRide &ride, const unsigned long long *rowF, unsigned long long *rowW,
+                        const SeedPack &sp, const unsigned int *seed_ok, hipStream_t st);
 template <bool FRESH>
 static int coarse_pass(const Tiles &t, const FScratch &s, char *scr, const uint64_t *cand, uint64_t *reached, const Fresh &f,
-                       int ncnt, hipStream_t st) {
+                       int ncnt, hipStream_t st, const McRide *front = nullptr) {
     const Blocks bk = coarse_blocks(t);
     uint8_t *dirty0 = (uint8_t *)(scr + s.off_dirty0), *dirty1 = (uint8_t *)(scr + s.off_dirty1);
     unsigned int *cnt = (unsigned int *)(scr + s.off_cnt), *list0 = (unsigned int *)(scr + s.off_list0);
@@ -1306,10 +1307,15 @@
                        (const unsigned long long *)reached, dirty0, dirty1, rowF, rowW, cnt, ncnt, f.sp, f.dtype, f.data, f.t0,
                        f.t1, seed_ok);
     IVX_LAUNCH_CHECK();
-    auto coarse = t.conn == 26 ? k_flood_coarse<26, FRESH> : t.conn == 18 ? k_flood_coarse<18, FRESH> : k_flood_coarse<6, FRESH>;
-    hipLaunchKernelGGL(coarse, dim3(1), dim3(ct), 0, st, t, bk, (const unsigned long long *)rowF, rowW, f.sp,
-                       (const unsigned int *)seed_ok);
-    IVX_LAUNCH_CHECK();
+    if (FRESH && front) {
+        int rc = front_launch(t, bk, *front, rowF, rowW, f.sp, seed_ok, st);
+        if (rc) return rc;
+    } else {
+        auto coarse = t.conn == 26 ? k_flood_coarse<26, FRESH> : t.conn == 18 ? k_flood_coarse<18, FRESH> : k_flood_coarse<6, FRESH>;
+        hipLaunchKernelGGL(coarse, dim3(1), dim3(ct), 0, st, t, bk, (const unsigned long long *)rowF, rowW, f.sp,
+                           (const unsigned int *)seed_ok);
+        IVX_LAUNCH_CHECK();
+    }
     hipLaunchKernelGGL(k_flood_block_apply<FRESH>, dim3(groups), dim3(256), 0, st, t, bk, (const unsigned long long *)cand,
                        (unsigned long long *)reached, (const unsigned long long *)rowW, dirty0, list0, cnt, f.sp,
                        (const unsigned int *)seed_ok);
@@ -1347,15 +1353,29 @@
     }
     return IVX_OK;
 }
+enum { RIDE_COUNT = 0, RIDE_LIST = 1, RIDE_FRONT_ONLY = 2 };
 struct McRide {
     const ivx_mc_params *p;
     void *scratch;
+    int mode = RIDE_COUNT;
+    void *list = nullptr;
+    int64_t cap = 0;
 };
+static int front_launch(const Tiles &t, const Blocks &bk, const McRide &ride, const unsigned long long *rowF, unsigned long long *rowW,
+                        const SeedPack &sp, const unsigned int *seed_ok, hipStream_t st) {
+    int rc = ivx::mc_front_launch(ride.p, ride.scratch, coarse_args(t, bk, rowF, rowW, seed_ok), sp, t.conn, st);
+    if (rc) return rc;
+    return ivx::mc_ride_scan(ride.p, ride.scratch, st);
+}
 static int launch_levels(const Tiles &t, const uint64_t *reached, const uint64_t *inside, uint8_t *mask, int v_in, int v_sel, bool all,
                          const ApplyWhen &when, hipStream_t st, const McRide *ride = nullptr) {
     const int64_t nchunks = t.dz * t.dy * t.dx / 16;
     if (!nchunks) return IVX_OK;
-    if (ride) return ivx::mc_ride_launch(ride->p, ride->scratch, reached, inside, nchunks, mask, v_in, v_sel, all, when, st);
+    if (ride && ride->mode == RIDE_COUNT)
+        return ivx::mc_ride_launch(ride->p, ride->scratch, reached, inside, nchunks, mask, v_in, v_sel, all, when, st);
+    if (ride && ride->mode == RIDE_LIST)
+        return ivx::mc_ride_list_launch(ride->p, ride->scratch, ride->list, ride->cap, reached, inside, nchunks, mask, v_in, v_sel, all,
+                                        when, st);
     const int64_t blocks = ivx::cdiv(nchunks, 1024);
     auto k = all ? k_flood_apply_levels16<true> : k_flood_apply_levels16<false>;
     hipLaunchKernelGGL(k, dim3((unsigned)(blocks < 16384 ? blocks : 16384)), dim3(256), 0, st, (const uint16_t *)reached,
@@ -1370,6 +1390,7 @@
     bool written;
     const McRide *ride = nullptr;
     bool plain = false;
+    bool front = false;
 };
 constexpr unsigned EARLY_BELOW = 96u;
 constexpr int EARLY_TRIES = 2;
@@ -1422,7 +1443,7 @@
     int ahead = fixed_ahead >= 0 ? fixed_ahead : 1;
     if (coarse_ok(t, mode)) {
         static const Fresh no_seeds = {0, nullptr, 0.0, 0.0, {{}, 0}};
-        rc = fresh ? coarse_pass<true>(t, s, scr, cand, reached, *fresh, CNT_CLEARED, st)
+        rc = fresh ? coarse_pass<true>(t, s, scr, cand, reached, *fresh, CNT_CLEARED, st, early && early->front ? early->ride : nullptr)
                    : coarse_pass<false>(t, s, scr, cand, reached, no_seeds, CNT_CLEARED, st);
         if (rc) return rc;
     } else {
@@ -1541,6 +1562,20 @@
     }();
     return fused_on && nseeds >= 1 && nseeds <= 16 && t.ntiles > 0 && !flood_mode_ccl() && coarse_ok(t, ivx::FLOOD_SYMMETRIC);
 }
+static bool front_count_ok(const Tiles &t, int64_t nseeds) {
+    return fused_start(t, nseeds) && ivx::mc_front_fits(t.nty, t.ntz);
+}
+extern "C" int ivx_flood_front_describe(const ivx_flood_plan *p, int64_t nseeds, int32_t out[4]) {
+    IVX_REQUIRE(out, IVX_EINVAL, "flood_front_describe: NULL argument");
+    Tiles t;
+    int rc = make_tiles(p, &t);
+    if (rc) return rc;
+    out[0] = front_count_ok(t, nseeds) ? 1 : 0;
+    out[1] = (int32_t)std::min<int64_t>(t.nty * t.ntz, 0x7fffffff);
+    out[2] = (int32_t)std::min<int64_t>((t.nty + 2) * (t.ntz + 2), 0x7fffffff);
+    out[3] = ivx::mc_front_lanes();
+    return IVX_OK;
+}
 static int flood_grow_impl(const ivx_flood_plan *p, int dtype, const void *data, double t0, double t1, const int64_t *seeds_xyz,
                            int64_t nseeds, uint64_t *cand, uint64_t *reached, void *scratch_, int *rounds, void *stream,
                            int look_ahead, EarlyWrite *early = nullptr) {
@@ -1762,22 +1797,33 @@
 
 static int grow_select_impl(const ivx_flood_plan *p, int dtype, const void *data, double t0, double t1, const int64_t *seeds_xyz,
                             int64_t nseeds, uint64_t *cand, uint64_t *reached, void *scratch_, int *rounds, const ivx_flood_write *write,
-                            int look_ahead, const ivx_mc_params *mc, void *mc_scratch, int *counted, void *stream) {
+                            int look_ahead, const ivx_mc_params *mc, void *mc_scratch, int *counted, void *stream, int front_flags = 0,
+                            int64_t max_tris = 0, int64_t *did = nullptr) {
     IVX_REQUIRE(write && write->kind >= IVX_FLOOD_WRITE_NONE && write->kind <= IVX_FLOOD_WRITE_APPLY_U8, IVX_EINVAL,
                 "flood_grow_select: no write description, or one of an unknown kind");
     IVX_REQUIRE(write->kind == IVX_FLOOD_WRITE_NONE || write->mask, IVX_EINVAL, "flood_grow_select: the write has no mask");
     if (counted) *counted = 0;
     EarlyWrite early = {write, false};
     const bool all = write->kind == IVX_FLOOD_WRITE_MASK_FROM_PLANES;
-    const McRide ride = {mc, mc_scratch};
-    Tiles t;
-    int rc = make_tiles(p, &t);
-    if (rc) return rc;
+    McRide ride = {mc, mc_scratch};
+    Tiles t;
+    int rc = make_tiles(p, &t);
+    if (rc) return rc;
+    if (did) did[0] = did[1] = did[2] = 0;
     if (mc && counted && (all || write->kind == IVX_FLOOD_WRITE_APPLY_LEVELS) &&
         levels_check(t, reached, write->inside_bits, write->mask, write->v_in, write->v_sel, all) == IVX_OK &&
         ivx::mc_ride_ok(mc, mc_scratch, t.dz, t.dy, t.dx)) {
         early.ride = &ride;
         ivx::mc_ride_begin(mc_scratch, write->inside_bits);
+        if ((front_flags & IVX_FLOOD_FRONT_COUNT) && front_count_ok(t, nseeds)) {
+            early.front = true;
+            ride.mode = RIDE_FRONT_ONLY;
+            if ((front_flags & IVX_FLOOD_WRITE_LIST) && max_tris > 0) {
+                if ((rc = ivx::mc_ride_list_buffer(max_tris, ivx::S(stream), &ride.list))) return rc;
+                ride.mode = RIDE_LIST;
+                ride.cap = max_tris;
+            }
+        }
     }
     rc = flood_grow_impl(p, dtype, data, t0, t1, seeds_xyz, nseeds, cand, reached, scratch_, rounds, stream, look_ahead, &early);
     if (rc) return rc;
@@ -1800,8 +1846,13 @@
         if (rc) return rc;
     }
     if (fused) {
-        if ((rc = ivx::mc_ride_scan(mc, mc_scratch, ivx::S(stream)))) return rc;
+        if (!early.front && (rc = ivx::mc_ride_scan(mc, mc_scratch, ivx::S(stream)))) return rc;
         *counted = 1;
+        if (did) did[0] = 1, did[1] = early.front ? 1 : 0;
+        if (ride.mode == RIDE_LIST) {
+            ivx::mc_ride_list_built(mc_scratch, ride.list, ride.cap);
+            if (did) did[2] = ride.cap;
+        }
     }
     return IVX_OK;
 }
@@ -1818,6 +1869,17 @@
     IVX_REQUIRE(mc && mc_scratch && counted, IVX_EINVAL, "flood_grow_select_count: null piece, scratch or result");
     return grow_select_impl(p, dtype, data, t0, t1, seeds_xyz, nseeds, cand, reached, scratch_, rounds, write, look_ahead, mc, mc_scratch,
                             counted, stream);
+}
+
+extern "C" int ivx_dev_flood_grow_select_list(const ivx_flood_plan *p, int dtype, const void *data, double t0, double t1,
+                                              const int64_t *seeds_xyz, int64_t nseeds, uint64_t *cand, uint64_t *reached,
+                                              void *scratch_, int *rounds, const ivx_flood_write *write, int look_ahead,
+                                              const ivx_mc_params *mc, void *mc_scratch, int flags, int64_t max_tris, int64_t did[3],
+                                              void *stream) {
+    IVX_REQUIRE(mc && mc_scratch && did && max_tris >= 0, IVX_EINVAL, "flood_grow_select_list: null piece, scratch or result");
+    int counted = 0;
+    return grow_select_impl(p, dtype, data, t0, t1, seeds_xyz, nseeds, cand, reached, scratch_, rounds, write, look_ahead, mc, mc_scratch,
+                            &counted, stream, flags, max_tris, did);
 }
 
 extern "C" int ivx_dev_flood_apply2(const ivx_flood_plan *p, const uint64_t *reached, uint8_t *out, int fill,
diff --git a/invesalius3_amd/csrc/k_mc.hip b/invesalius3_amd/csrc/k_mc.hip
--- a/invesalius3_amd/csrc/k_mc.hip
+++ b/invesalius3_amd/csrc/k_mc.hip
@@ -1,5 +1,6 @@
 #include <algorithm>
 
+#include "flood_coarse.h"
 #include "levels_write.h"
 #include "mc_common.h"
 
@@ -205,22 +206,31 @@
     uint4 *out;
     unsigned int in4, sel4;
 };
+struct McCountLds {
+    uint64_t c[256][5];
+    uint32_t part[4], wcnt[4];
+    uint16_t slot[256];
+    uint8_t ntri[256];
+    uint8_t hi[256];
+};
 template <bool RIDE, bool ALL>
 __device__ __forceinline__ void mc_count_body(const uint64_t *__restrict__ bits, const Geom &g, size_t nwords, uint64_t pbits,
-                                              uint16_t *__restrict__ counts, uint32_t *__restrict__ bsum, const McRideArgs &ride) {
-    __shared__ uint32_t s_part[4], s_wcnt[4];
-    __shared__ uint8_t s_ntri[256];
-    __shared__ uint64_t s_c[256][5];
-    __shared__ uint8_t s_hi[256];
-    __shared__ uint16_t s_slot[256];
+                                              uint16_t *__restrict__ counts, uint32_t *__restrict__ bsum, const McRideArgs &ride,
+                                              McCountLds &lds, uint32_t bid, uint32_t nbid) {
+    auto &s_part = lds.part;
+    auto &s_wcnt = lds.wcnt;
+    auto &s_ntri = lds.ntri;
+    auto &s_c = lds.c;
+    auto &s_hi = lds.hi;
+    auto &s_slot = lds.slot;
     const int tid = threadIdx.x, lane = tid & 63, wv = tid >> 6;
     const uint8_t ntri = MC_NTRI[tid];
-    const int64_t ride_i0 = (int64_t)blockIdx.x * 1024 + tid;
+    const int64_t ride_i0 = (int64_t)bid * 1024 + tid;
     LevelsWords lw;
     if (RIDE) levels_load<ALL>(ride.reached, ride.inside, ride.nchunks, ride_i0, lw);
     auto ride_rest = [&]() {
         if (!RIDE) return;
-        const int64_t stride = (int64_t)gridDim.x * 1024;
+        const int64_t stride = (int64_t)nbid * 1024;
         for (int64_t i0 = ride_i0 + stride; i0 < ride.nchunks; i0 += stride) {
             LevelsWords w2;
             levels_load<ALL>(ride.reached, ride.inside, ride.nchunks, i0, w2);
@@ -232,7 +242,7 @@
         if (RIDE) levels_store<ALL>(lw, ride.nchunks, ride_i0, ride.out, ride.in4, ride.sel4);
 #endif
     };
-    const size_t wid = (size_t)blockIdx.x * 256 + tid;
+    const size_t wid = (size_t)bid * 256 + tid;
     uint64_t act = 0;
     Corner8 r;
     if (wid < nwords) {
@@ -257,13 +267,13 @@
 #endif
 #if defined(IVX_RIDE_NO_WALK)
     if (RIDE) {
-        if (tid == 0) bsum[blockIdx.x] = 0;
+        if (tid == 0) bsum[bid] = 0;
         ride_rest();
         return;
     }
 #endif
     if (!nact) {
-        if (tid == 0) bsum[blockIdx.x] = 0;
+        if (tid == 0) bsum[bid] = 0;
         ride_rest();
         return;
     }
@@ -296,27 +306,52 @@
                       ((int)(hi >> 2 & 1u) << 5) | ((int)(c3 >> 63) << 6) | ((int)(hi >> 3 & 1u) << 7);
             n += s_ntri[idx];
         }
-        counts[(size_t)blockIdx.x * 256 + s_slot[tid]] = (uint16_t)n;
+        counts[(size_t)bid * 256 + s_slot[tid]] = (uint16_t)n;
     }
     uint32_t s = n;
 #pragma unroll
     for (int o = 32; o > 0; o >>= 1) s += __shfl_xor(s, o, 64);
     if (lane == 0) s_part[wv] = s;
     __syncthreads();
-    if (tid == 0) bsum[blockIdx.x] = s_part[0] + s_part[1] + s_part[2] + s_part[3];
+    if (tid == 0) bsum[bid] = s_part[0] + s_part[1] + s_part[2] + s_part[3];
     ride_rest();
 }
 __global__ __launch_bounds__(256) void k_mc_count(const uint64_t *__restrict__ bits, Geom g, size_t nwords,
                                                   uint64_t pbits, uint16_t *__restrict__ counts,
                                                   uint32_t *__restrict__ bsum) {
-    mc_count_body<false, false>(bits, g, nwords, pbits, counts, bsum, McRideArgs{});
+    __shared__ McCountLds lds;
+    mc_count_body<false, false>(bits, g, nwords, pbits, counts, bsum, McRideArgs{}, lds, blockIdx.x, gridDim.x);
 }
 template <bool ALL>
 __global__ __launch_bounds__(256) void k_mc_count_write(const uint64_t *__restrict__ bits, Geom g, size_t nwords, uint64_t pbits,
                                                         uint16_t *__restrict__ counts, uint32_t *__restrict__ bsum, McRideArgs ride,
                                                         ApplyWhen when) {
     if (apply_when_skips(when)) return;
-    mc_count_body<true, ALL>(bits, g, nwords, pbits, counts, bsum, ride);
+    __shared__ McCountLds lds;
+    mc_count_body<true, ALL>(bits, g, nwords, pbits, counts, bsum, ride, lds, blockIdx.x, gridDim.x);
+}
+constexpr int FRONT_LANES = 256;
+constexpr int FRONT_ROWS = (int)(sizeof(McCountLds) / 8) - 1;
+template <int CONN>
+__global__ __launch_bounds__(FRONT_LANES) __attribute__((amdgpu_waves_per_eu(8, 8))) void k_flood_coarse_count(CoarseArgs ca, SeedPack sp, const uint64_t *__restrict__ bits, Geom g,
+                                                                    size_t nwords, uint64_t pbits, uint16_t *__restrict__ counts,
+                                                                    uint32_t *__restrict__ bsum) {
+    __shared__ union {
+        McCountLds count;
+        unsigned long long rows[FRONT_ROWS + 1];
+    } lds;
+    if (blockIdx.x == 0) {
+#if !defined(IVX_FRONT_NO_COARSE)
+#if defined(IVX_FRONT_PRIO)
+        __builtin_amdgcn_s_setprio(3);
+#endif
+        coarse_body_lean<CONN>(ca, sp, lds.rows, reinterpret_cast<unsigned int *>(&lds.rows[FRONT_ROWS]));
+#endif
+        return;
+    }
+#if !defined(IVX_FRONT_NO_COUNT)
+    mc_count_body<false, false>(bits, g, nwords, pbits, counts, bsum, McRideArgs{}, lds.count, blockIdx.x - 1, gridDim.x - 1);
+#endif
 }
 
 __global__ __launch_bounds__(1024) void k_mc_scan(const uint32_t *__restrict__ bsum, size_t n,
@@ -429,9 +464,10 @@
     v += (uint32_t)__builtin_amdgcn_update_dpp(0, (int)v, 0x143, 0xc, 0xf, false);
     return v;
 }
-__global__ __launch_bounds__(256) void k_mc_list(const uint64_t *__restrict__ bits, Geom g, size_t nwords, uint64_t pbits,
-                                                 const uint16_t *__restrict__ counts, const uint64_t *__restrict__ boff,
-                                                 uint64_t *__restrict__ list, uint64_t max_tris) {
+template <bool RIDE, bool ALL>
+__device__ __forceinline__ void mc_list_body(const uint64_t *__restrict__ bits, const Geom &g, size_t nwords, uint64_t pbits,
+                                             const uint16_t *__restrict__ counts, const uint64_t *__restrict__ boff,
+                                             uint64_t *__restrict__ list, uint64_t max_tris, const McRideArgs &ride) {
     __shared__ uint32_t s_wave[4], s_part[2][4];
     __shared__ uint8_t s_ntri[256];
     __shared__ uint64_t s_c[4][256];
@@ -439,11 +475,32 @@
     __shared__ uint64_t s_pre[256];
     __shared__ uint16_t s_cell[MCL_CELLS];
     const int tid = threadIdx.x, lane = tid & 63, wv = tid >> 6;
+    const int64_t ride_i0 = (int64_t)blockIdx.x * 1024 + tid;
+    LevelsWords lw;
+    if (RIDE) levels_load<ALL>(ride.reached, ride.inside, ride.nchunks, ride_i0, lw);
+    auto ride_rest = [&]() {
+        if (!RIDE) return;
+        const int64_t stride = (int64_t)gridDim.x * 1024;
+        for (int64_t i0 = ride_i0 + stride; i0 < ride.nchunks; i0 += stride) {
+            LevelsWords w2;
+            levels_load<ALL>(ride.reached, ride.inside, ride.nchunks, i0, w2);
+            levels_store<ALL>(w2, ride.nchunks, i0, ride.out, ride.in4, ride.sel4);
+        }
+    };
+    auto ride_store = [&]() {
+#if !defined(IVX_LISTW_NO_STORES)
+        if (RIDE) levels_store<ALL>(lw, ride.nchunks, ride_i0, ride.out, ride.in4, ride.sel4);
+#endif
+    };
     const uint8_t ntri = MC_NTRI[tid];
     const size_t wid0 = (size_t)blockIdx.x * 256;
     const uint32_t n = wid0 + tid < nwords ? (uint32_t)counts[wid0 + tid] : 0u;
     const uint64_t pos0 = boff[blockIdx.x];
-    if (boff[blockIdx.x + 1] == pos0 || pos0 >= max_tris) return;
+    if (boff[blockIdx.x + 1] == pos0 || pos0 >= max_tris) {
+        ride_store();
+        ride_rest();
+        return;
+    }
     uint64_t a2 = 0;
     if (n) {
         uint32_t k, j, w;
@@ -467,6 +524,13 @@
     uint32_t ci = inc - pc;
     for (int q = 0; q < wv; q++) ci += s_wave[q];
     const uint32_t ncell = s_wave[0] + s_wave[1] + s_wave[2] + s_wave[3];
+    ride_store();
+#if defined(IVX_LISTW_NO_PHASE2)
+    if (RIDE) {
+        ride_rest();
+        return;
+    }
+#endif
     uint64_t P = pos0;
     int par = 0;
     for (uint32_t sb = 0; sb < ncell; sb += MCL_CELLS) {
@@ -508,10 +572,26 @@
             for (uint32_t t = 0; t < MC_MAX_TRI; t++)
                 if (t < nt && p0 + t < max_tris) list[p0 + t] = d0 | t;
             P += tot;
-            if (P >= max_tris) return;
+            if (P >= max_tris) {
+                ride_rest();
+                return;
+            }
             par ^= 1;
         }
     }
+    ride_rest();
+}
+__global__ __launch_bounds__(256) void k_mc_list(const uint64_t *__restrict__ bits, Geom g, size_t nwords, uint64_t pbits,
+                                                 const uint16_t *__restrict__ counts, const uint64_t *__restrict__ boff,
+                                                 uint64_t *__restrict__ list, uint64_t max_tris) {
+    mc_list_body<false, false>(bits, g, nwords, pbits, counts, boff, list, max_tris, McRideArgs{});
+}
+template <bool ALL>
+__global__ __launch_bounds__(256) void k_mc_list_write(const uint64_t *__restrict__ bits, Geom g, size_t nwords, uint64_t pbits,
+                                                       const uint16_t *__restrict__ counts, const uint64_t *__restrict__ boff,
+                                                       uint64_t *__restrict__ list, uint64_t max_tris, McRideArgs ride, ApplyWhen when) {
+    if (apply_when_skips(when)) return;
+    mc_list_body<true, ALL>(bits, g, nwords, pbits, counts, boff, list, max_tris, ride);
 }
 
 template <typename T, bool LEVELS>
@@ -724,6 +804,19 @@
     return IVX_OK;
 }
 
+extern "C" int ivx_mc_scratch_layout(const ivx_mc_params *p, size_t out[4]) {
+    IVX_REQUIRE(out, IVX_EINVAL, "mc_scratch_layout: NULL argument");
+    Geom g;
+    int rc = make_geom(p, &g);
+    if (rc) return rc;
+    const Scratch s = make_scratch(g, p->niso);
+    out[0] = s.off_counts;
+    out[1] = s.nwords;
+    out[2] = s.off_boff;
+    out[3] = s.nblocks;
+    return IVX_OK;
+}
+
 extern "C" int ivx_dev_mc_scratch_bytes(const ivx_mc_params *p, size_t *nbytes) {
     Geom g;
     int rc = make_geom(p, &g);
@@ -840,6 +933,48 @@
     IVX_LAUNCH_CHECK();
     return IVX_OK;
 }
+static_assert(FRONT_ROWS <= FRONT_LANES * COARSE_CRP, "mc_front_fits: the LDS bound must imply the lanes bound");
+bool ivx::mc_front_fits(int64_t nty, int64_t ntz) { return nty > 0 && ntz > 0 && (nty + 2) * (ntz + 2) <= FRONT_ROWS; }
+int ivx::mc_front_lanes() { return FRONT_LANES; }
+int ivx::mc_front_launch(const ivx_mc_params *p, void *scratch_, const CoarseArgs &ca, const SeedPack &sp, int conn, hipStream_t st) {
+    Geom g;
+    Scratch s;
+    bool empty;
+    int rc = mc_piece_layout(p, &g, &s, &empty);
+    if (rc) return rc;
+    IVX_REQUIRE(!empty && p->niso == 1 && mc_front_fits(ca.nty, ca.ntz) && (conn == 6 || conn == 18 || conn == 26), IVX_EINVAL,
+                "mc_front: an empty piece, two iso-values, a tile grid beyond the launch's bounds or no standard structuring element");
+    char *scratch = (char *)scratch_;
+    auto k = conn == 26 ? k_flood_coarse_count<26> : conn == 18 ? k_flood_coarse_count<18> : k_flood_coarse_count<6>;
+    hipLaunchKernelGGL(k, dim3((unsigned)s.nblocks + 1u), dim3(FRONT_LANES), 0, st, ca, sp, mc_bits_ptr(scratch, s, 0), g, s.nwords,
+                       pad_bits(p, 0), (uint16_t *)(scratch + s.off_counts), (uint32_t *)(scratch + s.off_bsum));
+    IVX_LAUNCH_CHECK();
+    return IVX_OK;
+}
+int ivx::mc_ride_list_buffer(int64_t max_tris, hipStream_t st, void **list) {
+    return ws_get_s(WS_MCLIST, st, (size_t)max_tris * 8 + 64, list);
+}
+int ivx::mc_ride_list_launch(const ivx_mc_params *p, void *scratch_, void *list, int64_t max_tris, const uint64_t *reached,
+                             const uint64_t *inside, int64_t nchunks, uint8_t *mask, int v_in, int v_sel, bool all, const ApplyWhen &when,
+                             hipStream_t st) {
+    Geom g;
+    Scratch s;
+    bool empty;
+    int rc = mc_piece_layout(p, &g, &s, &empty);
+    if (rc) return rc;
+    IVX_REQUIRE(!empty && p->niso == 1 && nchunks > 0 && list && max_tris >= 0, IVX_EINVAL,
+                "mc_ride_list: an empty piece or volume, two iso-values or no list");
+    char *scratch = (char *)scratch_;
+    const McRideArgs ride = {(const uint16_t *)reached, (const uint16_t *)inside, nchunks, (uint4 *)mask, 0x01010101u * (uint8_t)v_in,
+                             0x01010101u * (uint8_t)v_sel};
+    auto k = all ? k_mc_list_write<true> : k_mc_list_write<false>;
+    hipLaunchKernelGGL(k, dim3((unsigned)s.nblocks), dim3(256), 0, st, mc_bits_ptr(scratch, s, 0), g, s.nwords, pad_bits(p, 0),
+                       (const uint16_t *)(scratch + s.off_counts), (const uint64_t *)(scratch + s.off_boff), (uint64_t *)list,
+                       (uint64_t)max_tris, ride, when);
+    IVX_LAUNCH_CHECK();
+    return IVX_OK;
+}
+void ivx::mc_ride_list_built(const void *scratch, const void *list, int64_t max_tris) { mc_pieces().list_built(scratch, list, max_tris); }
 int ivx::mc_ride_scan(const ivx_mc_params *p, void *scratch, hipStream_t st) {
     Geom g;
     Scratch s;
diff --git a/invesalius3_amd/device.py b/invesalius3_amd/device.py
--- a/invesalius3_amd/device.py
+++ b/invesalius3_amd/device.py
@@ -215,6 +215,9 @@
         self._mask_defer = os.environ.get("IVX_MASK_DEFER", "1") != "0"
         self._select = os.environ.get("IVX_FLOOD_SELECT", "1") != "0"
         self._ride = RideBook(os.environ.get("IVX_MC_RIDE", "1") != "0")
+        self._ride_flags = ((L.FLOOD_FRONT_COUNT if os.environ.get("IVX_MC_RIDE_FRONT", "1") != "0" else 0)
+                            | (L.FLOOD_WRITE_LIST if os.environ.get("IVX_MC_RIDE_LIST", "1") != "0" else 0))
+        self.ride_report = (0, 0, 0)
         self._look_ahead = -1
         self._ranges = None
         self._ranges_valid = False
@@ -432,14 +435,25 @@
         write = self._flood_write(fill, select_value) if self._select else None
         piece = self._piece_to_ride(write, shared, select_value)
         if piece is not None:
-            counted = ctypes.c_int(0)
-            L.check(lib.ivx_dev_flood_grow_select_count(p, L.I16, img_ptr, ctypes.c_double(t0), ctypes.c_double(t1), L.ptr(seeds),
-                                                        c64(len(seeds)), cand.ptr, self.reached.ptr, self.flood_scratch.ptr,
-                                                        ctypes.byref(rounds), ctypes.byref(write), int(self._look_ahead),
-                                                        ctypes.byref(piece[0]), self._mc_scratch.ptr, ctypes.byref(counted), st),
-                    "region_grow")
-            if counted.value:
-                self._ride.rode(self._mbits_version)
+            did = (ctypes.c_int64 * 3)()
+            flags = self._ride_flags
+            if flags & L.FLOOD_FRONT_COUNT:
+                L.check(lib.ivx_dev_flood_grow_select_list(p, L.I16, img_ptr, ctypes.c_double(t0), ctypes.c_double(t1), L.ptr(seeds),
+                                                           c64(len(seeds)), cand.ptr, self.reached.ptr, self.flood_scratch.ptr,
+                                                           ctypes.byref(rounds), ctypes.byref(write), int(self._look_ahead),
+                                                           ctypes.byref(piece[0]), self._mc_scratch.ptr, int(flags),
+                                                           c64(self._tris.nbytes // 36), did, st), "region_grow")
+            else:
+                counted = ctypes.c_int(0)
+                L.check(lib.ivx_dev_flood_grow_select_count(p, L.I16, img_ptr, ctypes.c_double(t0), ctypes.c_double(t1), L.ptr(seeds),
+                                                            c64(len(seeds)), cand.ptr, self.reached.ptr, self.flood_scratch.ptr,
+                                                            ctypes.byref(rounds), ctypes.byref(write), int(self._look_ahead),
+                                                            ctypes.byref(piece[0]), self._mc_scratch.ptr, ctypes.byref(counted), st),
+                        "region_grow")
+                did[0] = counted.value
+            self.ride_report = (int(did[0]), int(did[1]), int(did[2]))
+            if did[0]:
+                self._ride.rode(self._mbits_version, int(did[2]))
             else:
                 self._ride.drop()
         elif write is not None:
@@ -458,7 +472,7 @@
         if (write is None or write.kind not in (L.FLOOD_WRITE_MASK_FROM_PLANES, L.FLOOD_WRITE_APPLY_LEVELS) or not shared
                 or select_value is None or int(select_value) < 127 or not self._fuse or self._prefetch is not None
                 or self._mc_scratch is None or self._tris is None or self.timer.records("mc_count")
-                or self.timer.records("mask_bytes")):
+                or self.timer.records("mc_emit") or self.timer.records("mask_bytes")):
             return None
         piece = self._ride.piece_to_ride()
         if piece is None or piece[1] != 0 or piece[0].ny != self.dy or piece[0].nx != self.dx or piece[0].nz > self.dz:
diff --git a/invesalius3_amd/mc_ride.py b/invesalius3_amd/mc_ride.py
--- a/invesalius3_amd/mc_ride.py
+++ b/invesalius3_amd/mc_ride.py
@@ -6,25 +6,31 @@
         self.enabled = bool(enabled)
         self.armed = None
         self.note = None
+        self.note_listed = 0
         self.rides = 0
         self.taken = 0
+        self.listed = 0
 
     def piece_to_ride(self):
         return self.armed if self.enabled else None
 
-    def rode(self, version: int):
+    def rode(self, version: int, listed: int = 0):
         self.note = (self.armed[0], self.armed[1], int(version))
+        self.note_listed = int(listed)
         self.armed = None
         self.rides += 1
 
     def take(self, params, z0: int, version: int) -> bool:
         n, self.note = self.note, None
+        listed, self.note_listed = self.note_listed, 0
         ok = n is not None and n[0] is params and n[1] == z0 and n[2] == int(version)
         self.taken += int(ok)
+        self.listed = listed if ok else 0
         return ok
 
     def drop(self):
         self.note = None
+        self.note_listed = 0
 
     def surface_counted(self, params, z0: int, from_plane: bool):
         self.armed = (params, z0) if (self.enabled and from_plane) else None
```
